# ChenyuWang-Monica/REED

Measured on AMD Instinct MI355X. Metric: SiT-XL/2 ImageNet-256 train images/sec, higher is better.
Workload: dtype bf16

## Files before the change

include/reed_hip.h:

```cpp
#ifndef REED_HIP_H
#define REED_HIP_H
#include <stdint.h>
#ifdef __cplusplus
extern "C" {
#endif

const char* reed_last_error(void);
int reed_version(void);
int reed_half_kind(void);

int reed_gemm(int layout, int epilogue, const void* P, int64_t ldp, const void* Q, int64_t ldq,
              int M, int N, int K, void* C, int64_t ldc, void* C2, int64_t ldc2, const void* R,
              int64_t ldr, const void* bias, const void* gate, int64_t ldgate, int rows_per_gate,
              float* dbias, int accumulate, int split_k, int64_t slab_stride, void* stream);

int reed_wgrad_group(int n, const void* const* dy, const void* const* x, float* const* dw, float* const* dbias,
                     const int* n_out, const int* k_in, int tokens, int accumulate, void* stream);
int reed_wgrad_group_deal(int n, const int* n_out, const int* k_in, const int* has_bias, int cus, unsigned* items);

int reed_set_cu_reserve(int n);
int reed_planning_cus(void);
int reed_set_concurrent_comm(int on);

int reed_gemm_force_tile(int tile);

int64_t reed_colsum_ws_floats(int M, int N);
int reed_colsum_bf16(const void* x, int64_t ld, float* ws, float* out, int M, int N, int accumulate,
                     void* stream);

int reed_reduce_slabs(const float* slabs, int64_t stride, int nslabs, float* out, int64_t n,
                      int accumulate, void* stream);

int reed_ln_modulate_fwd(const float* x, const void* shift, const void* scale, int64_t ldmod,
                         void* h, float* mean, float* rstd, int M, int D, int T, float eps,
                         void* stream);
int reed_ln_modulate_bwd(const void* dh, const float* x, const float* mean, const float* rstd,
                         const void* scale, int64_t ldmod, float* dx, float* part, int M, int D,
                         int T, void* stream);

int reed_ln_modulate_bwd_gate(const void* dh, const float* x, const float* mean, const float* rstd,
                              const void* scale, int64_t ldmod, float* dx, float* part, const void* y,
                              const void* gate, int64_t ldgate, void* dy, float* part_g, float* part_dy,
                              int M, int D, int T, void* stream);

int reed_gate_bwd(const float* dx, const void* y, const void* gate, int64_t ldgate, void* dy,
                  float* part, float* part_dy, int M, int D, int T, void* stream);
int reed_transpose_bf16(const void* src, void* dst, int R, int C, void* stream);
int reed_rowsum_f32(const float* part, int R, float* ws, float* out, int N, int accumulate, void* stream);

int reed_reduce_mod_parts(const float* const* parts, const int64_t* strides, const int64_t* offs,
                          int nparts, void* dmod, int64_t lddmod, int B, int D, int chunks,
                          void* stream);

int reed_attention_fwd(const void* qkv, void* o, float* lse, int B, int T, int H, int hd,
                       void* stream);
int reed_attention_bwd(const void* qkv, const void* o, const void* d_o, const float* lse,
                       void* dqkv, int B, int T, int H, int hd, void* stream);
int64_t reed_attention_bwd_ws_floats(int B, int T, int H);
int reed_attention_bwd_ws(const void* qkv, const void* o, const void* d_o, const float* lse, void* dqkv, float* ws,
                          int B, int T, int H, int hd, void* stream);
int reed_attention_bwd_dp(const void* qkv, const void* d_o, const float* lse, const float* dpart, void* dqkv, float* ws,
                          int B, int T, int H, int hd, void* stream);

int reed_qk_norm_fwd(const void* qkv, const float* qw, const float* qb, const float* kw, const float* kb,
                     void* out, float* stats, int M, int H, int hd, float eps, void* stream);
int64_t reed_qk_norm_bwd_part_floats(int M, int H, int hd);
int reed_qk_norm_bwd(const void* dn, const void* qkv, const float* stats, const float* qw, const float* kw,
                     void* dpre, float* part, int M, int H, int hd, void* stream);

int reed_patch_embed_fwd(const float* x, const void* w, const void* bias, const float* pos,
                         float* tokens, int B, int C, int HW, int P, int D, void* stream);
int reed_patchify_bf16(const float* x, void* out, int B, int C, int HW, int P, int order, void* stream);
int64_t reed_smallk_wgrad_ws_floats(int Dw, int KS);
int reed_smallk_wgrad(const void* wide, int wide_is_f32, const void* small, float* ws, float* out,
                      float* colsum_wide, float* colsum_small, int M, int Dw, int KS, int layout,
                      int accumulate, void* stream);
int reed_timestep_sinusoid(const float* t, void* out, int B, int dim, float max_period, void* stream);
int reed_label_cond(const int64_t* labels, const uint8_t* drop, int num_classes, int table_rows, const float* table,
                    const void* t_emb, int64_t* labels_out, float* c, void* silu_c, int* err_flag, int B, int D,
                    void* stream);
int reed_label_cond_bwd(const float* dsilu_c, const float* c, const int64_t* labels_eff, void* dt_emb,
                        float* dtable, int B, int D, void* stream);
int reed_final_layer_fwd(const float* x, const void* shift, const void* scale, int64_t ldmod,
                         const void* w, const void* bias, float* out, float* mean, float* rstd,
                         int B, int T, int D, int C, int P, float eps, void* stream);
int reed_final_layer_bwd_rows(const float* dout, const float* x, const float* mean, const float* rstd,
                              const void* shift, const void* scale, int64_t ldmod, const void* w,
                              void* hbuf, void* dlin, void* dh, int B, int T, int D, int C, int P,
                              void* stream);
int reed_token_mean_fwd(const float* x, void* out, int B, int T, int D, void* stream);
int reed_token_mean_bwd(const void* dmean, float* dx, int B, int T, int D, void* stream);

int reed_sample_posterior(const float* moments, const float* eps, float* out, int B, int64_t half,
                          float scale, float bias, void* stream);
int reed_interpolant(const float* x, const float* noise, const float* t, float* xt, float* target,
                     int B, int64_t per, int path_type, void* stream);
int reed_mse_fwd(const float* out, const float* target, float* loss, int B, int64_t per, void* stream);
int reed_mse_bwd(const float* out, const float* target, const float* gscale, float* dout, int B,
                 int64_t per, void* stream);
int reed_cosine_fwd(const void* zt, const float* z, float* rowdot, float* loss, int B, int T, int Z,
                    void* stream);
int reed_cosine_bwd(const void* zt, const float* z, const float* gscale, void* dzt, int B, int T,
                    int Z, void* stream);

int reed_grad_sqnorm(const float* g, int64_t n, float* partial, int nblocks, void* stream);
int reed_clip_finalize(const float* partial, int nblocks, float max_norm, float* norm_clip, void* stream);
int reed_clip_finalize_scaled(const float* partial, int nblocks, float max_norm, float* norm_clip, float* scaler_state,
                              float growth_factor, float backoff_factor, float growth_interval, void* stream);
int reed_adamw_ema(float* p, const float* g, float* m, float* v, float* ema, void* shadow,
                   int64_t n_train, int64_t n_total, const float* norm_clip, const float* scaler_state, float lr,
                   float beta1, float beta2, float eps, float weight_decay, float bc1, float bc2, float ema_decay,
                   void* stream);
int reed_cast_bf16(const float* src, void* dst, int64_t n, void* stream);

int reed_sampler_update(const double* x_cur, const float* model_out, const double* d_prev,
                        double* d_store, double* x_next, int64_t n_elems, int cfg, double cfg_scale,
                        double dt, double w0, double w1, void* stream);
int reed_sde_update(const double* x_cur, const float* model_out, const double* eps, double* x_next,
                    int64_t n_elems, int cfg, double cfg_scale, double t_cur, double dt,
                    int path_type, int last_step, void* stream);
int reed_sampler_input(const double* x, float* out, int64_t n_elems, int dup, void* stream);

int reed_comm_unique_id(void* out128);
int reed_comm_init(const void* id128, int rank, int world, void** comm_out);
int reed_comm_allreduce_avg(void* comm, float* buf, int64_t count, void* compute_stream);
int reed_comm_allreduce_avg_rsag(void* comm, float* buf, int64_t count, void* compute_stream);
int reed_comm_sync(void* comm, void* compute_stream);
int reed_comm_broadcast(void* comm, float* buf, int64_t count, int root, void* compute_stream);
int reed_comm_allgather(void* comm, const void* send, void* recv, int64_t bytes, void* compute_stream);
int reed_comm_sync_gather(void* comm, void* compute_stream);
int reed_comm_destroy(void* comm);

int reed_clip_im2col(const float* img, void* out, int B, int S, int P, int Kp, void* stream);
int reed_clip_tokens(const void* patches, const float* cls, const float* pos, void* out, int B, int T, int D,
                     void* stream);
int reed_ln_affine_bf16(const void* x, const float* w, const float* b, void* out, int M, int D, float eps,
                        void* stream);

// ... 27 lines not shown
```

reed_amd/csrc/attention.hip:

```cpp
#include <stdlib.h>

#include <type_traits>
#include <utility>

#include "../../include/reed_hip.h"
#include "common.hpp"

#ifndef REED_ATTN_LD_AUX
#define REED_ATTN_LD_AUX 0
#endif
namespace {

constexpr int ROWB = 144;
constexpr int TILE_B = 256 * ROWB;
constexpr int ROWF = 160;
constexpr int TILE_F = 256 * ROWF;
constexpr float LOG2E = 1.4426950408889634f;
constexpr float LN2 = 0.6931471805599453f;

template <int HD>
struct Cfg {
  static constexpr int KS = (HD + 31) / 32;
  static constexpr int DT = (HD + 15) / 16;
  static constexpr int NCH = HD / 8;
};

template <int HD, int RB = ROWB>
__device__ __forceinline__ void load_tile(char* lds, const bf16* src, long row_stride, int rows_valid,
                                          int tid, int nthreads) {
  constexpr int NCH = Cfg<HD>::NCH;
  constexpr int PER = (256 * NCH + 511) / 512;
  uint4 v[PER];
  const int last = rows_valid - 1;
#pragma unroll
  for (int k = 0; k < PER; ++k) {
    int idx = tid + k * 512;
    int row = idx / NCH, c = idx - row * NCH;
    int rc = min(row, last);
    if (rc < 0) rc = 0;
    int cc = idx < 256 * NCH ? c : 0;
    v[k] = *(const uint4*)(src + (long)rc * row_stride + cc * 8);
  }
#pragma unroll
  for (int k = 0; k < PER; ++k) {
    int idx = tid + k * 512;
    int row = idx / NCH, c = idx - row * NCH;
    if (idx < 256 * NCH) {
      const unsigned msk = row < rows_valid ? 0xFFFFFFFFu : 0u;
      uint4 w = v[k];
      w.x &= msk; w.y &= msk; w.z &= msk; w.w &= msk;
      *(uint4*)(lds + row * RB + c * 16) = w;
    }
  }
  if (RB > HD * 2 + 8 && tid < 256) {
#pragma unroll
    for (int c = Cfg<HD>::NCH; c < RB / 16; ++c) *(uint4*)(lds + tid * RB + c * 16) = make_uint4(0, 0, 0, 0);
  }
}

__device__ __forceinline__ bf16x8 frag_rows(const char* tile, int row0, int ks, int lane) {
  return *(const bf16x8*)(tile + (row0 + (lane & 15)) * ROWB + (ks * 32 + 8 * (lane >> 4)) * 2);
}
template <bool WRAP>
__device__ __forceinline__ bf16x8 frag_rows_f(const char* tile, int row0, int ks, int lane) {
  const int g = WRAP ? ((lane >> 4) & 1) : (lane >> 4);
  return *(const bf16x8*)(tile + (row0 + (lane & 15)) * ROWF + (ks * 32 + 8 * g) * 2);
}
__device__ __forceinline__ bf16x8 frag_trT_f(const char* tile, int rbase, int d0, int lane) {
  int i = lane & 15, g = lane >> 4, q = i >> 2, p = i & 3;
  const char* a0 = tile + (rbase + 4 * g + q) * ROWF + (d0 + 4 * p) * 2;
  bf16x4 lo = REED_DS_READ_TR16_B64((bf16x4 __attribute__((address_space(3)))*)a0);
  bf16x4 hi = REED_DS_READ_TR16_B64((bf16x4 __attribute__((address_space(3)))*)(a0 + 16 * ROWF));
  return __builtin_shufflevector(lo, hi, 0, 1, 2, 3, 4, 5, 6, 7);
}
__device__ __forceinline__ bf16x8 frag_trT(const char* tile, int rbase, int d0, int lane) {
  int i = lane & 15, g = lane >> 4, q = i >> 2, p = i & 3;
  const char* a0 = tile + (rbase + 4 * g + q) * ROWB + (d0 + 4 * p) * 2;
  bf16x4 lo = REED_DS_READ_TR16_B64((bf16x4 __attribute__((address_space(3)))*)a0);
  bf16x4 hi = REED_DS_READ_TR16_B64((bf16x4 __attribute__((address_space(3)))*)(a0 + 16 * ROWB));
  return __builtin_shufflevector(lo, hi, 0, 1, 2, 3, 4, 5, 6, 7);
}
template <int HD>
__device__ __forceinline__ bf16x8 load_frag_global(const bf16* rowptr, bool row_ok, int ks, int lane) {
  bf16x8 z;
#pragma unroll
  for (int j = 0; j < 8; ++j) z[j] = (bf16)0.f;
  int col = ks * 32 + 8 * (lane >> 4);
  if (row_ok && col < HD) z = *(const bf16x8*)(rowptr + col);
// ... 833 lines not shown
#pragma unroll
      for (int kt = 0; kt < 16; ++kt) {
#pragma unroll
        for (int r = 0; r < 4; ++r) {
          float p = __builtin_fmaf(st[qt][kt][r], sc2, -mneg);
          if (!(DBGK && (dbg & 2))) p = __builtin_amdgcn_exp2f(p);
          st[qt][kt][r] = p;
          if (!ONES) sum += p;
        }
        if (kt & 1) pb[qt][kt >> 1] = pack2(st[qt][kt - 1], st[qt][kt]);
      }
      if (!ONES) {
        sum += __shfl_xor(sum, 16, 64);
        sum += __shfl_xor(sum, 32, 64);
      }
      mrow[qt] = mneg;
      lrow[qt] = sum;
      __builtin_amdgcn_sched_barrier(0);
    }
    ATTN_STAMP(3);
    asm volatile("s_waitcnt vmcnt(12)" ::: "memory");
    __builtin_amdgcn_sched_barrier(0);
    ATTN_STAMP(4);
    if (ONES && lane < 32) *(bf16*)(Vw + lane * ROWF + HD * 2) = (bf16)1.0f;
    ATTN_BARRIER();
    ATTN_STAMP(5);
    char* const k2rows = Kb + par * TILE_F + wave * 32 * ROWF;
    const __amdgpu_buffer_rsrc_t k2rs = mk_rsrc(plus(base_of(it + 2 * G), D), win);
    constexpr bool KSPREAD = PVX && REED_ATTN_KSPREAD;
    if constexpr (!KSPREAD) {
#pragma unroll
      for (int j = 0; j < 5; ++j) issue_piece(k2rows, k2rs, j);
    }
    __builtin_amdgcn_sched_barrier(0);
    f32x4 ot[2][DT];
    {
      const unsigned vb = lds_addr(Vt + (4 * g + (i >> 2)) * ROWF + (i & 3) * 8);
      if (DBGK && (dbg & 4)) {
#pragma unroll
        for (int dt = 0; dt < DT; ++dt) ot[0][dt] = ot[1][dt] = f32x4{1.f, 1.f, 1.f, 1.f};
      } else if (FULL && !PVX) {
        pvu_all<ROWF, 8, DT>(vb, pb, ot);
      } else if (FULL) {
        pvx_all<ROWF, DT, !ONES>(vb, st, mrow, sc2, lrow, DBGK && (dbg & 2), ot, [&](auto s_c) {
          constexpr int S = decltype(s_c)::value;
          if constexpr (KSPREAD && S < 5) issue_piece(k2rows, k2rs, S);
        });
        if (!ONES) {
#pragma unroll
          for (int qt = 0; qt < 2; ++qt) {
            lrow[qt] += __shfl_xor(lrow[qt], 16, 64);
            lrow[qt] += __shfl_xor(lrow[qt], 32, 64);
          }
        }
      } else {
#pragma unroll
        for (int qt = 0; qt < 2; ++qt)
#pragma unroll
          for (int dt = 0; dt < DT; ++dt) ot[qt][dt] = zero4();
        pv_all<ROWF, DT>(Vt + (4 * g + (i >> 2)) * ROWF + (i & 3) * 8, (T + 31) >> 5, pb, ot);
      }
    }
    ATTN_STAMP(6);
    asm volatile("s_waitcnt vmcnt(22)" ::: "memory");
    __builtin_amdgcn_sched_barrier(0);
    ATTN_STAMP(7);
    ATTN_BARRIER();
    ATTN_STAMP(8);
    stage_item(ot, mrow, lrow);
    __builtin_amdgcn_sched_barrier(0);
    store_item(it);
  }
  asm volatile("s_waitcnt vmcnt(0)" ::: "memory");
  if (DBGK && (dbg & 32) && lse && lane0 == 0) {
    unsigned long long* dst = (unsigned long long*)lse + ((long)blockIdx.x * 8 + wave) * 10;
#pragma unroll
    for (int k = 0; k < 10; ++k) dst[k] = tacc[k];
  }
#undef ATTN_STAMP
}

template <int HD, bool KSP = true, bool QSP = true>
__global__ __launch_bounds__(512, 2) void attn_fwd256v_kernel(const bf16* __restrict__ qkv, bf16* __restrict__ o,
                                                             float* __restrict__ lse, int H, int nitems) {
  extern __shared__ __attribute__((aligned(16))) char smem[];
  constexpr int T = 256;
  constexpr int KS = Cfg<HD>::KS, DT = Cfg<HD>::DT, NCH = Cfg<HD>::NCH;
  constexpr bool ONES = (HD == 72);
  static_assert(HD == 64 || HD == 72, "attn_fwd256v_kernel: head_dim 64 or 72");
  const int tid = threadIdx.x;
  const int lane0 = tid & 63;
  const int wave = __builtin_amdgcn_readfirstlane(tid >> 6);
  const int D = H * HD;
  const long tok = 3l * D;
  const int tokb = (int)(tok * 2);
  char* const Kw = smem + wave * 32 * ROWF;
  char* const Vt = smem + TILE_F;
  char* const Qw = smem + 3 * TILE_F + wave * 32 * ROWF;
  const int q0 = wave * 32;
  const float sc2 = rsqrtf((float)HD) * LOG2E;
  int voff[5];
#pragma unroll
  for (int j = 0; j < 5; ++j) voff[j] = dma_voff<HD, ROWF>((wave * 5 + j) * 64 + lane0, tokb);
  const long win = tile_window<HD>(T, tokb);
  auto piece = [&](char* wave_rows, __amdgpu_buffer_rsrc_t rs, int j) {
    __builtin_amdgcn_raw_ptr_buffer_load_lds(rs, (lds_ptr_t)(wave_rows + j * 1024), 16, voff[j], 0, 0, REED_ATTN_LD_AUX);
  };
  auto issue = [&](char* wave_rows, const bf16* base) {
    const __amdgpu_buffer_rsrc_t rs = mk_rsrc(base, win);
#pragma unroll
    for (int j = 0; j < 5; ++j) piece(wave_rows, rs, j);
  };
  auto base_of = [&](int item) -> const bf16* {
    if (item >= nitems) return nullptr;
    const int b = item / H, h = item - b * H;
    return qkv + (long)b * T * tok + h * HD;
  };
  auto plus = [](const bf16* p_, long n) -> const bf16* { return p_ ? p_ + n : nullptr; };
  const int G = gridDim.x;
  constexpr int RST = ROWB;
  constexpr int NQ = 32 * NCH;
  float lsev[2] = {0.f, 0.f};
  f32x4 st[2][16];

  int it = xcd_contiguous(blockIdx.x, G);
  {
    const bf16* b0 = base_of(it);
    issue(Qw, b0);
    issue(Kw, plus(b0, D));
    issue(Vt + wave * 32 * ROWF, plus(b0, 2 * D));
    const __amdgpu_buffer_rsrc_t none = mk_rsrc(nullptr, 0);
#pragma unroll
    for (int k = 0; k < 8; ++k) __builtin_amdgcn_raw_buffer_store_b32((unsigned)(k + lane0), none, DMA_OOB - 256 * k, 0, 0);
    asm volatile("s_waitcnt vmcnt(13)" ::: "memory");
    ATTN_BARRIER();
  }
  int par = 0, pit = -1;
  for (; it < nitems; it += G, par ^= 1) {
    int lane = lane0;
    asm volatile("" : "+v"(lane));
    const int i = lane & 15, g = lane >> 4;
    char* const Vcur = Vt + par * TILE_F;
    char* const Vprev_w = Vt + (par ^ 1) * TILE_F + wave * 32 * ROWF;
    asm volatile("s_waitcnt vmcnt(17)" ::: "memory");
    __builtin_amdgcn_sched_barrier(0);
    bf16x8 qf[2][KS];
    {
      const unsigned qa = lds_addr(Qw + i * ROWF + 16 * g);
#pragma unroll
      for (int qt = 0; qt < 2; ++qt)
#pragma unroll
        for (int ks = 0; ks < KS; ++ks) {
          const bool wrap = HD % 32 != 0 && ks == KS - 1;
          const unsigned a = qa + qt * 16 * ROWF + ks * 64 - ((wrap && g >= 2) ? 32 : 0);
          qf[qt][ks] = lds_read128_asm(a);
        }
      ATTN_LDS_WAIT();
      if (HD % 32 != 0 && g >= 2) { qf[0][KS - 1] = zero_frag(); qf[1][KS - 1] = zero_frag(); }
    }
    const __amdgpu_buffer_rsrc_t rsQ = mk_rsrc(base_of(it + G), win);
    if constexpr (!QSP) {
#pragma unroll
      for (int j = 0; j < 5; ++j) piece(Qw, rsQ, j);
    }
    __builtin_amdgcn_sched_barrier(0);
    {
      const int pb_ = pit < 0 ? 0 : pit / H, ph = pit < 0 ? 0 : pit - pb_ * H;
      const __amdgpu_buffer_rsrc_t rsO = mk_rsrc(pit < 0 ? nullptr : o + (long)pb_ * T * D + ph * HD, tile_window<HD>(T, D * 2));
      const __amdgpu_buffer_rsrc_t rsL = mk_rsrc((lse && pit >= 0) ? lse + ((long)pb_ * H + ph) * T : nullptr, (long)T * 4);
      const __amdgpu_buffer_rsrc_t rsV = mk_rsrc(plus(base_of(it + G), 2 * D), win);
      u32x4 pc = {0u, 0u, 0u, 0u};
      const unsigned ka = lds_addr(smem + i * ROWF + 16 * g);
      sk_all<HD, ROWF>(ka, ka - (g >= 2 ? 32 : 0), qf, st, [&](auto kt_c) {
        constexpr int KT = decltype(kt_c)::value;
        if constexpr (KT < 10 && (KT & 1) == 0) {
          constexpr int k = KT / 2;
          const int qi = min(lane + 64 * k, NQ - 1);
          const int rr = qi / NCH, c = qi - rr * NCH;
          pc = __builtin_bit_cast(u32x4, lds_read128_asm(lds_addr(Vprev_w + rr * RST + c * 16)));
        } else if constexpr (KT < 10) {
          constexpr int k = KT / 2;
          piece(Vprev_w, rsV, k);
          const int qi = lane + 64 * k;
          const int rr = qi / NCH, c = qi - rr * NCH;
          __builtin_amdgcn_raw_buffer_store_b128(pc, rsO, qi < NQ ? (q0 + rr) * (D * 2) + c * 16 : DMA_OOB, 0, 0);
        } else if constexpr (KT < 12) {
          constexpr int qt = KT - 10;
          __builtin_amdgcn_raw_buffer_store_b32(__builtin_bit_cast(unsigned, lsev[qt]), rsL,
                                                g == 0 ? (q0 + 16 * qt + i) * 4 : DMA_OOB, 0, 0);
        }
        if constexpr (QSP && KT >= 11) piece(Qw, rsQ, KT - 11);
      });
    }
    float mrow[2], lrow[2];
#pragma unroll
    for (int qt = 0; qt < 2; ++qt) {
      float mx = -INFINITY;
#pragma unroll
      for (int kt = 0; kt < 16; ++kt)
#pragma unroll
        for (int r = 0; r < 4; ++r) mx = fmaxf(mx, st[qt][kt][r]);
      mx = fmaxf(mx, __shfl_xor(mx, 16, 64));
      mx = fmaxf(mx, __shfl_xor(mx, 32, 64));
      mrow[qt] = mx * sc2;
      lrow[qt] = 0.f;
    }
    asm volatile("s_waitcnt vmcnt(25)" ::: "memory");
    __builtin_amdgcn_sched_barrier(0);
    if (ONES && lane < 32) *(bf16*)(Vcur + (wave * 32 + lane) * ROWF + HD * 2) = (bf16)1.0f;
    ATTN_BARRIER();
    const __amdgpu_buffer_rsrc_t rsK = mk_rsrc(plus(base_of(it + G), D), win);
    if constexpr (!KSP) {
#pragma unroll
      for (int j = 0; j < 5; ++j) piece(Kw, rsK, j);
    }
    __builtin_amdgcn_sched_barrier(0);
    f32x4 ot[2][DT];
    {
      const unsigned vb = lds_addr(Vcur + (4 * g + (i >> 2)) * ROWF + (i & 3) * 8);
      pvx_all<ROWF, DT, !ONES>(vb, st, mrow, sc2, lrow, false, ot, [&](auto s_c) {
        constexpr int S = decltype(s_c)::value;
        if constexpr (KSP && S < 5) piece(Kw, rsK, S);
      });
      if (!ONES) {
#pragma unroll
        for (int qt = 0; qt < 2; ++qt) {
          lrow[qt] += __shfl_xor(lrow[qt], 16, 64);
          lrow[qt] += __shfl_xor(lrow[qt], 32, 64);
        }
      }
    }
    asm volatile("s_waitcnt vmcnt(0)" ::: "memory");
    __builtin_amdgcn_sched_barrier(0);
    ATTN_BARRIER();
    {
      char* const Vw = Vcur + wave * 32 * ROWF;
#pragma unroll
      for (int qt = 0; qt < 2; ++qt) {
        float l = lrow[qt];
        if (ONES) l = __shfl(ot[qt][DT - 1][0], 32 + i, 64);
        const float inv = __builtin_amdgcn_rcpf(l);
#pragma unroll
        for (int dt = 0; dt < DT; ++dt) {
          const int d = 16 * dt + 4 * g;
          const u32x2 v = {pk2(ot[qt][dt][0] * inv, ot[qt][dt][1] * inv), pk2(ot[qt][dt][2] * inv, ot[qt][dt][3] * inv)};
          if (16 * dt + 16 <= HD || d < HD) *(u32x2*)(Vw + (16 * qt + i) * RST + d * 2) = v;
        }
        lsev[qt] = mrow[qt] * LN2 + __logf(l);
      }
    }
    __builtin_amdgcn_sched_barrier(0);
    pit = it;
  }
  if (pit >= 0) {
    int lane = lane0;
    asm volatile("" : "+v"(lane));
    const int i = lane & 15, g = lane >> 4;
    const char* const Vw = Vt + (par ^ 1) * TILE_F + wave * 32 * ROWF;
    const int pb_ = pit / H, ph = pit - pb_ * H;
    const __amdgpu_buffer_rsrc_t rsO = mk_rsrc(o + (long)pb_ * T * D + ph * HD, tile_window<HD>(T, D * 2));
    const __amdgpu_buffer_rsrc_t rsL = mk_rsrc(lse ? lse + ((long)pb_ * H + ph) * T : nullptr, (long)T * 4);
    u32x4 pcs[5];
#pragma unroll
    for (int k = 0; k < 5; ++k) {
      const int qi = min(lane + 64 * k, NQ - 1);
      const int rr = qi / NCH, c = qi - rr * NCH;
      pcs[k] = __builtin_bit_cast(u32x4, lds_read128_asm(lds_addr(Vw + rr * RST + c * 16)));
    }
    ATTN_LDS_WAIT();
#pragma unroll
    for (int k = 0; k < 5; ++k) {
      const int qi = lane + 64 * k;
      const int rr = qi / NCH, c = qi - rr * NCH;
      __builtin_amdgcn_raw_buffer_store_b128(pcs[k], rsO, qi < NQ ? (q0 + rr) * (D * 2) + c * 16 : DMA_OOB, 0, 0);
    }
#pragma unroll
    for (int qt = 0; qt < 2; ++qt)
      __builtin_amdgcn_raw_buffer_store_b32(__builtin_bit_cast(unsigned, lsev[qt]), rsL, g == 0 ? (q0 + 16 * qt + i) * 4 : DMA_OOB, 0, 0);
  }
  asm volatile("s_waitcnt vmcnt(0)" ::: "memory");
}

template <int HD>
__global__ __launch_bounds__(512, 2) void attn_bwd_ks_kernel(const bf16* __restrict__ qkv, const bf16* __restrict__ o,
                                                             const bf16* __restrict__ d_o, const float* __restrict__ lse,
                                                             bf16* __restrict__ dqkv, int B, int T, int H) {
  extern __shared__ __attribute__((aligned(16))) char smem[];
  constexpr int KS = Cfg<HD>::KS, DT = Cfg<HD>::DT, NCH = Cfg<HD>::NCH;
  constexpr int DTA = (DT + 1) / 2;
  const int tid = threadIdx.x, lane = tid & 63;
  const int wave = __builtin_amdgcn_readfirstlane(tid >> 6);
  const int i = lane & 15, g = lane >> 4;
  const int D = H * HD;
  const int bh = xcd_contiguous(blockIdx.x, gridDim.x);
  const int b = bh / H, h = bh % H;
  const long tok = 3l * D;
  const bf16* base = qkv + (long)b * T * tok + h * HD;
  bf16* dbase = dqkv + (long)b * T * tok + h * HD;
  const bf16* gbase = d_o + (long)b * T * D + h * HD;
  char* Qt = smem;
  char* Kt = smem + TILE_B;
  char* St = smem + 2 * TILE_B;
  char* Gt = smem + 3 * TILE_B;
  float* lse2 = (float*)(smem + 4 * TILE_B + 256);
  float* dlt = lse2 + 256;
  if (tid < 16) *(uint4*)(smem + 4 * TILE_B + tid * 16) = make_uint4(0, 0, 0, 0);
  const float scale = rsqrtf((float)HD);
  const float sc2 = scale * LOG2E;
  const int r0 = wave * 32;

  auto issue_tile = [&](char* t, const bf16* s, int sb) {
    const __amdgpu_buffer_rsrc_t rs = mk_rsrc(s, tile_window<HD>(T, sb));
#pragma unroll
    for (int j = 0; j < 5; ++j) {
      const int I = wave + 8 * j;
      const int vo = dma_voff<HD, ROWB>(I * 64 + lane, sb);
      if (I < 36) __builtin_amdgcn_raw_ptr_buffer_load_lds(rs, (lds_ptr_t)(t + I * 1024), 16, vo, 0, 0, REED_ATTN_LD_AUX);
    }
  };
  issue_tile(Kt, base + D, (int)(tok * 2));
  issue_tile(Qt, base, (int)(tok * 2));
  issue_tile(Gt, gbase, D * 2);
  bf16x8 kf[2][KS], vf[2][KS];
  {
    bf16x8 gf[2][KS], of[2][KS];
    float lq[2];
#pragma unroll
    for (int t2 = 0; t2 < 2; ++t2) {
      const int row = r0 + 16 * t2 + i;
      const bool ok = row < T;
#pragma unroll
      for (int ks = 0; ks < KS; ++ks) {
        vf[t2][ks] = load_frag_global<HD>(base + 2 * D + (long)row * tok, ok, ks, lane);
        gf[t2][ks] = load_frag_global<HD>(gbase + (long)row * D, ok, ks, lane);
        of[t2][ks] = load_frag_global<HD>(o + ((long)b * T + row) * D + h * HD, ok, ks, lane);
// ... 1049 lines not shown
            bf16x8 gtf = frag_trT(Gc, qq0, 16 * dt, lane);
            bf16x8 qtf = frag_trT(Qc, qq0, 16 * dt, lane);
#pragma unroll
            for (int ct = 0; ct < 2; ++ct) {
              dv[ct][dt] = MFMA(gtf, pb[ct], dv[ct][dt]);
              dk[ct][dt] = MFMA(qtf, dsb[ct], dk[ct][dt]);
            }
          }
        }
      }
      __syncthreads();
      {
        const int qtile = wave >> 1;
        const int dt0 = (wave & 1) ? DTA : 0;
        f32x4 dq[DTA];
#pragma unroll
        for (int k = 0; k < DTA; ++k) dq[k] = zero4();
#pragma unroll 1
        for (int ks = 0; ks < nkb; ++ks) {
          const bf16x8 dsf = frag_trT(St, 32 * ks, 16 * qtile, lane);
#pragma unroll
          for (int k = 0; k < DTA; ++k) {
            if (dt0 + k < DT) {
              const bf16x8 ktf = frag_trT(Kt, 32 * ks, 16 * (dt0 + k), lane);
              dq[k] = MFMA(ktf, dsf, dq[k]);
            }
          }
        }
        const int q = ch * 64 + 16 * qtile + i;
#pragma unroll
        for (int k = 0; k < DTA; ++k) {
          const int d = 16 * (dt0 + k) + 4 * g;
          if (dt0 + k < DT && d < HD && q < T) *(f32x4*)(dqb + (long)q * D + d) = dq[k] * scale;
        }
      }
    }
#pragma unroll
    for (int ct = 0; ct < 2; ++ct) {
      const int key = k0 + r0 + 16 * ct + i;
#pragma unroll
      for (int dt = 0; dt < DT; ++dt) {
        const int d = 16 * dt + 4 * g;
        if (d < HD && kvalid[ct]) {
          bf16x4 a, c;
#pragma unroll
          for (int r = 0; r < 4; ++r) { a[r] = f2bf(dk[ct][dt][r] * scale); c[r] = f2bf(dv[ct][dt][r]); }
          *(bf16x4*)(dbase + (long)key * tok + D + d) = a;
          *(bf16x4*)(dbase + (long)key * tok + 2 * D + d) = c;
        }
      }
    }
  }
}

__global__ __launch_bounds__(256) void attn_dq_reduce_kernel(const float* __restrict__ dqp, bf16* __restrict__ dqkv, long n4, long slice,
                                                             int D, int nkt) {
  const long j = (long)blockIdx.x * 256 + threadIdx.x;
  if (j >= n4) return;
  f32x4 acc = *(const f32x4*)(dqp + 4 * j);
  for (int kt = 1; kt < nkt; ++kt) acc += *(const f32x4*)(dqp + kt * slice + 4 * j);
  const long e = 4 * j, tokn = e / D;
  const int c = (int)(e - tokn * D);
  bf16x4 v;
#pragma unroll
  for (int r = 0; r < 4; ++r) v[r] = f2bf(acc[r]);
  *(bf16x4*)(dqkv + tokn * 3 * D + c) = v;
}

template <typename K>
int set_lds(K kernel, int bytes) {
  hipError_t e = hipFuncSetAttribute((const void*)kernel, hipFuncAttributeMaxDynamicSharedMemorySize, bytes);
  if (e != hipSuccess) { reed_set_error("hipFuncSetAttribute(LDS=%d): %s", bytes, hipGetErrorString(e)); return (int)e; }
  return 0;
}

}
int reed_concurrent_comm();
int reed_num_cus();
namespace {
int num_cus() { return reed_num_cus(); }

}

extern "C" int reed_attention_fwd(const void* qkv, void* o, float* lse, int B, int T, int H, int hd,
                                  void* stream) {
  REED_CHECK_ARG(qkv && o, "attention_fwd: null pointer");
  REED_CHECK_ARG(hd == 64 || hd == 72 || hd == 80, "attention: head_dim %d unsupported (64, 72 or 80)", hd);
  REED_CHECK_ARG(hd != 80 || T <= 256, "attention: head_dim 80 (the I-JEPA ViT-H tower) is built for T <= 256 only (T=%d)", T);
  REED_CHECK_ARG(B > 0 && T > 0 && H > 0, "attention: bad dims B=%d T=%d H=%d", B, T, H);
  if (T <= 256) {
    const int lds = 4 * TILE_F, nitems = B * H;
    int ncu = num_cus();
    ncu -= ncu % 8;
    const dim3 grid(nitems < ncu ? nitems : ncu);
#ifdef REED_ATTN_DIAG
    static const int fdbg = getenv("REED_ATTN_FWD_DBG") ? atoi(getenv("REED_ATTN_FWD_DBG")) : 0;
#else
    constexpr int fdbg = 0;
#endif
    if (REED_ATTN_FWD_VDB_DEFAULT && T == 256 && (hd == 64 || hd == 72) && !fdbg) {
      if (hd == 64) {
        static int once = set_lds(attn_fwd256v_kernel<64>, lds);
        if (once) return once;
        REED_KLAUNCH((attn_fwd256v_kernel<64>), grid, dim3(512), lds, (hipStream_t)stream, (const bf16*)qkv, (bf16*)o, lse, H, nitems);
      } else {
        static int once = set_lds(attn_fwd256v_kernel<72>, lds);
        if (once) return once;
        REED_KLAUNCH((attn_fwd256v_kernel<72>), grid, dim3(512), lds, (hipStream_t)stream, (const bf16*)qkv, (bf16*)o, lse, H, nitems);
      }
      REED_LAUNCH_CHECK();
      return REED_OK;
    }
#define LAUNCH_FWD256P(HD, FULL, DBGK)                                                                                 \
    do {                                                                                                               \
      static int once = set_lds(attn_fwd256p_kernel<HD, FULL, DBGK>, lds);                                             \
      if (once) return once;                                                                                           \
      REED_KLAUNCH((attn_fwd256p_kernel<HD, FULL, DBGK>), grid, dim3(512), lds, (hipStream_t)stream,                    \
                   (const bf16*)qkv, (bf16*)o, lse, T, H, nitems, fdbg);                                               \
    } while (0)
#ifdef REED_ATTN_DIAG
    if (fdbg && hd == 72 && T == 256) LAUNCH_FWD256P(72, true, true);
    else
#endif
    if (hd == 64) { if (T == 256) LAUNCH_FWD256P(64, true, false); else LAUNCH_FWD256P(64, false, false); }
    else if (hd == 72) { if (T == 256) LAUNCH_FWD256P(72, true, false); else LAUNCH_FWD256P(72, false, false); }
    else { if (T == 256) LAUNCH_FWD256P(80, true, false); else LAUNCH_FWD256P(80, false, false); }
#undef LAUNCH_FWD256P
    REED_LAUNCH_CHECK();
    return REED_OK;
  }
  const int lds = 2 * TILE_F;
  dim3 grid(B * H, (T + 255) / 256);
  const int tail = T % 256;
  if (hd == 64 && T > 512 && T <= 4096 + 16 && tail >= 1 && tail <= 16) {
    grid.y = T / 256;
    static int once = set_lds(attn_fwd_kernel<64, true>, lds);
    if (once) return once;
    REED_KLAUNCH((attn_fwd_kernel<64, true>), grid, dim3(512), lds, (hipStream_t)stream, (const bf16*)qkv, (bf16*)o, lse, B, T, H);
    REED_LAUNCH_CHECK();
    return REED_OK;
  }
  if (hd == 64 && T > 256 && T <= 512 && tail >= 1 && tail <= 16) {
    grid.y = T / 256;
    const int nwaves = B * H * tail;
    REED_KLAUNCH(attn_fwd_rows_kernel, dim3(cdiv(nwaves, 4)), dim3(256), 0, (hipStream_t)stream, (const bf16*)qkv, (bf16*)o, lse, T, H,
                 T - tail, tail, nwaves);
    REED_LAUNCH_CHECK();
  }
  if (hd == 64) {
    static int once = set_lds(attn_fwd_kernel<64>, lds);
    if (once) return once;
    REED_KLAUNCH(attn_fwd_kernel<64>, grid, dim3(512), lds, (hipStream_t)stream, (const bf16*)qkv, (bf16*)o, lse, B, T, H);
  } else {
    static int once = set_lds(attn_fwd_kernel<72>, lds);
    if (once) return once;
    REED_KLAUNCH(attn_fwd_kernel<72>, grid, dim3(512), lds, (hipStream_t)stream, (const bf16*)qkv, (bf16*)o, lse, B, T, H);
  }
  REED_LAUNCH_CHECK();
  return REED_OK;
}

extern "C" int reed_attention_bwd(const void* qkv, const void* o, const void* d_o, const float* lse,
                                  void* dqkv, int B, int T, int H, int hd, void* stream) {
  REED_CHECK_ARG(qkv && o && d_o && lse && dqkv, "attention_bwd: null pointer");
  REED_CHECK_ARG(hd == 64 || hd == 72, "attention: head_dim %d unsupported (64 or 72)", hd);
  REED_CHECK_ARG(T > 0 && T <= 256, "attention_bwd: T=%d unsupported without a workspace (T <= 256; 256 < T <= 4096 runs through "
                 "reed_attention_bwd_ws / reed_attention_bwd_dp)", T);
  const int lds = 4 * TILE_B + 256 + 2048;
  dim3 grid(B * H);
  if (hd == 64) {
    static int once = set_lds(attn_bwd_ks_kernel<64>, lds);
    if (once) return once;
    REED_KLAUNCH((attn_bwd_ks_kernel<64>), grid, dim3(512), lds, (hipStream_t)stream, (const bf16*)qkv, (const bf16*)o,
                 (const bf16*)d_o, lse, (bf16*)dqkv, B, T, H);
  } else {
    static int once = set_lds(attn_bwd_ks_kernel<72>, lds);
    if (once) return once;
    REED_KLAUNCH((attn_bwd_ks_kernel<72>), grid, dim3(512), lds, (hipStream_t)stream, (const bf16*)qkv, (const bf16*)o,
                 (const bf16*)d_o, lse, (bf16*)dqkv, B, T, H);
  }
  REED_LAUNCH_CHECK();
  return REED_OK;
}


extern "C" int64_t reed_attention_bwd_ws_floats(int B, int T, int H) {
  const int64_t n = (int64_t)B * T * H;
  return T <= 256 ? n : n * (1 + (int64_t)((T + 255) / 256) * 72);
}

static int attention_bwd_persistent(const void* qkv, const void* o, const void* d_o, const float* lse, void* dqkv, float* ws,
                                    const float* dpart, int B, int T, int H, int hd, void* stream) {
  REED_CHECK_ARG(qkv && (o || dpart) && d_o && lse && dqkv && ws, "attention_bwd: null pointer");
  REED_CHECK_ARG(hd == 64 || hd == 72, "attention: head_dim %d unsupported (64 or 72)", hd);
  REED_CHECK_ARG(B > 0 && H > 0 && T > 0 && T <= 4096 && (T <= 256 || T % 16 == 0),
                 "attention_bwd: B=%d H=%d T=%d unsupported (T <= 256, or 256 < T <= 4096 with T a multiple of 16)", B, H, T);
  const int lds = 4 * TILE_B + 256 + 2048;
  const int nitems = B * H;
  const long nseg = (long)B * T * H;
  int ncu = num_cus();
  ncu -= ncu % 8;
  const int gmult = reed_concurrent_comm() ? 4 : 1;
  const long gwant = (long)ncu * gmult;
  const dim3 pgrid((unsigned)(nitems < gwant ? nitems : gwant));
  hipStream_t s = (hipStream_t)stream;
#ifdef REED_ATTN_DIAG
  static const int dbg = getenv("REED_ATTN_KSP_DBG") ? atoi(getenv("REED_ATTN_KSP_DBG")) : 0;
#else
  constexpr int dbg = 0;
#endif
#define REED_DELTA(HD)                                                                                                    \
  do {                                                                                                                    \
    if (dpart)                                                                                                            \
      REED_KLAUNCH(attn_delta_combine_kernel, dim3(cdiv(nseg, 256)), dim3(256), 0, s, dpart, ws, (long)B * T, T, H, (HD) == 64 ? 1 : 2); \
    else                                                                                                                  \
      REED_KLAUNCH(attn_delta_kernel<HD>, dim3(cdiv(nseg, 256)), dim3(256), 0, s, (const bf16*)o, (const bf16*)d_o, ws, nseg, T, H); \
  } while (0)
#define REED_BWD_KSP(HD)                                                                                                  \
  do {                                                                                                                    \
    static int once = set_lds(attn_bwd_ksp_kernel<HD>, lds);                                                              \
    if (once) return once;                                                                                                \
    REED_DELTA(HD);                                                                                                       \
    REED_LAUNCH_CHECK();                                                                                                  \
    REED_KLAUNCH(attn_bwd_ksp_kernel<HD>, pgrid, dim3(512), lds, s, (const bf16*)qkv, (const bf16*)d_o, lse, (const float*)ws, \
                 (bf16*)dqkv, T, H, nitems, dbg);                                                                              \
  } while (0)
  if (T > 256) {
    const int nkt = (T + 255) / 256, litems = B * H * nkt;
    const dim3 lgrid((unsigned)(litems < gwant ? litems : gwant));
    const long slice = nseg * hd;
    float* dqp = ws + nseg;
#define REED_BWD_LONG(HD)                                                                                                 \
  do {                                                                                                                    \
    static int once = set_lds(attn_bwd_long_kernel<HD>, LONG_LDS);                                                        \
    if (once) return once;                                                                                                \
    REED_DELTA(HD);                                                                                                       \
    REED_LAUNCH_CHECK();                                                                                                  \
    REED_KLAUNCH(attn_bwd_long_kernel<HD>, lgrid, dim3(512), LONG_LDS, s, (const bf16*)qkv, (const bf16*)d_o, lse,         \
                 (const float*)ws, dqp, (bf16*)dqkv, slice, T, H, nkt, litems);                                            \
  } while (0)
    if (hd == 64) REED_BWD_LONG(64);
    else REED_BWD_LONG(72);
// ... 54 lines not shown
```

reed_amd/csrc/attention_f32.hip:

```cpp
#include "../../include/reed_hip.h"
#include "common.hpp"

#ifndef REED_FP32
#error "attention_f32.hip belongs to the fp32-operand build (-DREED_FP32) only"
#endif

namespace {

constexpr int KT = 32;

template <int HD>
__device__ __forceinline__ void stage_rows(float* tile, const float* qkv, int which, long b, int h, int H, int T, int r0,
                                           int tid) {
  constexpr int NV = HD / 4;
  for (int i = tid; i < KT * NV; i += 256) {
    const int r = i / NV, c = i % NV;
    const int row = r0 + r;
    f32x4 v = {0.f, 0.f, 0.f, 0.f};
    if (row < T) v = *(const f32x4*)(qkv + (((b * T + row) * 3 + which) * H + h) * HD + 4 * c);
    *(f32x4*)(tile + r * HD + 4 * c) = v;
  }
}
template <int HD>
__device__ __forceinline__ void stage_rows_o(float* tile, const float* x, long b, int h, int H, int T, int r0, int tid) {
// ... 126 lines not shown
    __syncthreads();
    const int kn = min(KT, T - k0);
#pragma unroll 1
    for (int j = 0; j < kn; ++j) {
      const float p = expf(dot_row<HD>(qv, sk + j * HD) - ls);
      const float ds = p * (dot_row<HD>(dov, sv + j * HD) - delta);
      axpy_row<HD>(dq, ds, sk + j * HD);
    }
  }
  if (live) {
    float* gp = dqkv + (((b * T + q) * 3 + 0) * H + h) * HD;
#pragma unroll
    for (int c = 0; c < HD / 4; ++c)
      *(f32x4*)(gp + 4 * c) = f32x4{dq[4 * c] * scale, dq[4 * c + 1] * scale, dq[4 * c + 2] * scale, dq[4 * c + 3] * scale};
  }
}

template <int HD>
__global__ __launch_bounds__(256) void attn_f32_bwd_dkv_kernel(const float* __restrict__ qkv, const float* __restrict__ o,
                                                               const float* __restrict__ d_o, const float* __restrict__ lse,
                                                               float* __restrict__ dqkv, int T, int H) {
  __shared__ __attribute__((aligned(16))) float sq[KT * HD], sdo[KT * HD];
  __shared__ float sls[KT], sdl[KT];
  const int tid = threadIdx.x;
  const long b = blockIdx.x / H;
  const int h = blockIdx.x % H;
  const int kr = blockIdx.y * 256 + tid;
  const bool live = kr < T;
  const int kc = live ? kr : 0;
  const float scale = rsqrtf((float)HD);
  float kv[HD], vv[HD], dk[HD], dv[HD];
  {
    const float* kp = qkv + (((b * T + kc) * 3 + 1) * H + h) * HD;
    const float* vp = qkv + (((b * T + kc) * 3 + 2) * H + h) * HD;
#pragma unroll
    for (int c = 0; c < HD / 4; ++c) {
      const f32x4 a = *(const f32x4*)(kp + 4 * c), v = *(const f32x4*)(vp + 4 * c);
#pragma unroll
      for (int e = 0; e < 4; ++e) {
        kv[4 * c + e] = a[e] * scale;
        vv[4 * c + e] = v[e];
        dk[4 * c + e] = 0.f;
        dv[4 * c + e] = 0.f;
      }
    }
  }
  for (int q0 = 0; q0 < T; q0 += KT) {
    __syncthreads();
    stage_rows<HD>(sq, qkv, 0, b, h, H, T, q0, tid);
    stage_rows_o<HD>(sdo, d_o, b, h, H, T, q0, tid);
    if (tid < KT) {
      const int row = q0 + tid;
      float dl = 0.f, ls = INFINITY;
      if (row < T) {
        const float* op = o + ((b * T + row) * H + h) * HD;
        const float* gp = d_o + ((b * T + row) * H + h) * HD;
        for (int e = 0; e < HD; ++e) dl = fmaf(gp[e], op[e], dl);
        ls = lse[(b * H + h) * T + row];
      }
      sls[tid] = ls;
      sdl[tid] = dl;
    }
    __syncthreads();
    const int qn = min(KT, T - q0);
#pragma unroll 1
    for (int i = 0; i < qn; ++i) {
      const float p = expf(dot_row<HD>(kv, sq + i * HD) - sls[i]);
      const float ds = p * (dot_row<HD>(vv, sdo + i * HD) - sdl[i]);
      axpy_row<HD>(dv, p, sdo + i * HD);
      axpy_row<HD>(dk, ds, sq + i * HD);
    }
  }
  if (live) {
    float* gk = dqkv + (((b * T + kr) * 3 + 1) * H + h) * HD;
    float* gv = dqkv + (((b * T + kr) * 3 + 2) * H + h) * HD;
#pragma unroll
    for (int c = 0; c < HD / 4; ++c) {
      *(f32x4*)(gk + 4 * c) = f32x4{dk[4 * c] * scale, dk[4 * c + 1] * scale, dk[4 * c + 2] * scale, dk[4 * c + 3] * scale};
      *(f32x4*)(gv + 4 * c) = f32x4{dv[4 * c], dv[4 * c + 1], dv[4 * c + 2], dv[4 * c + 3]};
    }
  }
}

}

extern "C" int reed_attention_fwd(const void* qkv, void* o, float* lse, int B, int T, int H, int hd, void* stream) {
  REED_CHECK_ARG(qkv && o, "attention_fwd: null pointer");
  REED_CHECK_ARG(hd == 64 || hd == 72, "attention (fp32 build): head_dim %d unsupported (64 or 72)", hd);
  REED_CHECK_ARG(B > 0 && T > 0 && H > 0, "attention: bad dims B=%d T=%d H=%d", B, T, H);
  const dim3 grid(B * H, (T + 255) / 256);
  if (hd == 64) REED_KLAUNCH(attn_f32_fwd_kernel<64>, grid, dim3(256), 0, (hipStream_t)stream, (const float*)qkv, (float*)o, lse, T, H);
  else REED_KLAUNCH(attn_f32_fwd_kernel<72>, grid, dim3(256), 0, (hipStream_t)stream, (const float*)qkv, (float*)o, lse, T, H);
  REED_LAUNCH_CHECK();
  return REED_OK;
}

extern "C" int reed_attention_bwd(const void* qkv, const void* o, const void* d_o, const float* lse, void* dqkv, int B, int T,
                                  int H, int hd, void* stream) {
  REED_CHECK_ARG(qkv && o && d_o && lse && dqkv, "attention_bwd: null pointer");
  REED_CHECK_ARG(hd == 64 || hd == 72, "attention (fp32 build): head_dim %d unsupported (64 or 72)", hd);
  REED_CHECK_ARG(B > 0 && T > 0 && H > 0, "attention: bad dims B=%d T=%d H=%d", B, T, H);
  const dim3 grid(B * H, (T + 255) / 256);
  hipStream_t s = (hipStream_t)stream;
#define REED_BWD_F32(HD)                                                                                                 \
  do {                                                                                                                   \
    REED_KLAUNCH(attn_f32_bwd_dq_kernel<HD>, grid, dim3(256), 0, s, (const float*)qkv, (const float*)o, (const float*)d_o, \
                 lse, (float*)dqkv, T, H);                                                                               \
    REED_LAUNCH_CHECK();                                                                                                 \
    REED_KLAUNCH(attn_f32_bwd_dkv_kernel<HD>, grid, dim3(256), 0, s, (const float*)qkv, (const float*)o,                  \
                 (const float*)d_o, lse, (float*)dqkv, T, H);                                                            \
  } while (0)
  if (hd == 64) REED_BWD_F32(64);
  else REED_BWD_F32(72);
#undef REED_BWD_F32
  REED_LAUNCH_CHECK();
  return REED_OK;
}

extern "C" int64_t reed_attention_bwd_ws_floats(int, int, int) { return 0; }
extern "C" int reed_attention_bwd_ws(const void* qkv, const void* o, const void* d_o, const float* lse, void* dqkv, float*, int B,
                                     int T, int H, int hd, void* stream) {
  return reed_attention_bwd(qkv, o, d_o, lse, dqkv, B, T, H, hd, stream);
}

extern "C" int reed_attention_bwd_dp(const void*, const void*, const float*, const float*, void*, float*, int, int, int, int, void*) {
  reed_set_error("reed_attention_bwd_dp: not built for fp32 operands (use reed_attention_bwd_ws)");
  return REED_ERR_UNSUPPORTED;
}
```

reed_amd/csrc/gemm.hip:

```cpp
#include <stdlib.h>

#include "gemm_common.hpp"

int reed_gemm256_launch(int layout, int epi, GemmArgs a, int splits, hipStream_t stream);
int reed_gemm_tn_launch(int tile, GemmArgs a, int splits, hipStream_t stream);
bool reed_gemm256_preferred(int layout, int epi, const GemmArgs& a, int splits);
bool reed_gemm144_eligible(int layout, int epi, const GemmArgs& a, int splits);
bool reed_gemm144_preferred(int layout, int epi, const GemmArgs& a, int splits);
int reed_gemm144_launch(int layout, int epi, GemmArgs a, hipStream_t stream);
bool reed_gemm288_eligible(int layout, int epi, const GemmArgs& a, int splits);
bool reed_gemm288_preferred(int layout, int epi, const GemmArgs& a, int splits);
int reed_gemm288_launch(int epi, GemmArgs a, hipStream_t stream);
bool reed_gemm256w_eligible(int layout, int epi, const GemmArgs& a, int splits);
int reed_gemm256w_launch(int layout, int epi, GemmArgs a, hipStream_t stream);
int reed_num_cus();
double reed_gemm256_rate();
bool reed_gemm_skinny_eligible(int layout, int epi, const GemmArgs& a, int splits);
int reed_gemm_skinny_launch(int epi, GemmArgs a, hipStream_t stream);

namespace {
using namespace gemm_detail;

constexpr int BM = 128, BN = 128, BK = 64;
constexpr int TILE_BYTES = 16384;
// ... 105 lines not shown
    if constexpr (LAY != LAY_NT) REED_LDS_WAIT();
#pragma unroll
    for (int ks = 0; ks < 2; ++ks) {
#pragma unroll
      for (int i = 0; i < 4; ++i)
#pragma unroll
        for (int j = 0; j < 4; ++j)
          acc[i][j] = REED_MFMA_16x16x32(qf[ks][j], pf[ks][i], acc[i][j]);
      if constexpr (LAY == LAY_TN) {
        if (do_dbias) {
#pragma unroll
          for (int i = 0; i < 4; ++i)
            accb[i] = REED_MFMA_16x16x32(ones, pf[ks][i], accb[i]);
        }
      }
    }
    __syncthreads();
  }

  tile_epilogue<EPI, 4>(a, acc, m0, wm * 64, n0 + wn * 64, lane, z, smem + wave * EPI_STAGE_BYTES);
  if constexpr (LAY == LAY_TN) {
    if (do_dbias && (lane >> 4) == 0) {
#pragma unroll
      for (int i = 0; i < 4; ++i) {
        const int m = m0 + wm * 64 + i * 16 + (lane & 15);
        if (m < a.M) {
          if (gridDim.y > 1) a.dbias[(long)z * a.slab_stride + m] = accb[i][0];
          else if (a.accumulate) a.dbias[m] += accb[i][0];
          else a.dbias[m] = accb[i][0];
        }
      }
    }
  }
}

template <int LAY, int EPI>
int launch(const GemmArgs& a, int splits, hipStream_t stream) {
  static bool attr_set = false;
  if (!attr_set) {
    (void)hipFuncSetAttribute((const void*)gemm_kernel<LAY, EPI>,
                              hipFuncAttributeMaxDynamicSharedMemorySize, 2 * STAGE_BYTES);
    attr_set = true;
  }
  const int ntm = cdiv(a.M, BM), ntn = a.N / BN;
  dim3 grid(ntm * ntn, splits, 1);
  REED_KLAUNCH((gemm_kernel<LAY, EPI>), grid, dim3(256), 2 * STAGE_BYTES, stream, a);
  REED_LAUNCH_CHECK();
  return REED_OK;
}

template <int LAY>
int dispatch_epi(int epi, const GemmArgs& a, int splits, hipStream_t s) {
  switch (epi) {
    case EPI_BF16: return launch<LAY, EPI_BF16>(a, splits, s);
    case EPI_GELU: return launch<LAY, EPI_GELU>(a, splits, s);
    case EPI_SILU: return launch<LAY, EPI_SILU>(a, splits, s);
    case EPI_GATE_RES: return launch<LAY, EPI_GATE_RES>(a, splits, s);
    case EPI_DGELU: return launch<LAY, EPI_DGELU>(a, splits, s);
    case EPI_DSILU: return launch<LAY, EPI_DSILU>(a, splits, s);
    case EPI_GELU_G: return launch<LAY, EPI_GELU_G>(a, splits, s);
    case EPI_SILU_G: return launch<LAY, EPI_SILU_G>(a, splits, s);
    case EPI_MUL: return launch<LAY, EPI_MUL>(a, splits, s);
    case EPI_F32: return launch<LAY, EPI_F32>(a, splits, s);
    case EPI_ADDF32_RB: return launch<LAY, EPI_ADDF32_RB>(a, splits, s);
    case EPI_ATOMIC_F32: return launch<LAY, EPI_ATOMIC_F32>(a, splits, s);
    case EPI_QGELU: return launch<LAY, EPI_QGELU>(a, splits, s);
    case EPI_GELU_ERF: return launch<LAY, EPI_GELU_ERF>(a, splits, s);
    case EPI_RES_BF16: return launch<LAY, EPI_RES_BF16>(a, splits, s);
    case EPI_LS_RES:
      if constexpr (LAY == LAY_NT) return launch<LAY, EPI_LS_RES>(a, splits, s);
      break;
  }
  reed_set_error("reed_gemm: unknown epilogue %d", epi);
  return REED_ERR_ARG;
}

}

static const bool g_colsplit = getenv("REED_GEMM_COLSPLIT") && atoi(getenv("REED_GEMM_COLSPLIT")) != 0;
static int g_force_tile = 0;
extern "C" int reed_gemm_force_tile(int tile) { g_force_tile = tile; return 0; }
int reed_gemm_forced_tile() { return g_force_tile; }

int reed_gemm_launch(int layout, int epi, GemmArgs a, int splits, hipStream_t stream) {
  REED_CHECK_ARG(a.M > 0 && a.N > 0 && a.K > 0, "reed_gemm: empty problem M=%d N=%d K=%d", a.M, a.N, a.K);
  const int want = epi;
  if (epi == EPI_BF16_DOT) {
    REED_CHECK_ARG((layout == LAY_NN || layout == LAY_NT) && a.R && a.C2 && (a.rows_per_gate == 64 || a.rows_per_gate == 72) &&
                       a.N % a.rows_per_gate == 0 && a.N % 64 == 0 && splits <= 1,
                   "reed_gemm(epilogue 13): NN or NT, R and C2 given, rows_per_gate = head_dim 64 or 72 dividing N");
    epi = EPI_BF16;
  }
#define REED_ONLY_PLAIN()                                                                             \
  do {                                                                                                \
    if (want == EPI_BF16_DOT) {                                                                       \
      reed_set_error("reed_gemm(epilogue 13): this shape runs on a kernel without it (use epilogue 0)"); \
      return REED_ERR_UNSUPPORTED;                                                                    \
    }                                                                                                 \
  } while (0)
  const bool can144 = reed_gemm144_eligible(layout, epi, a, splits);
  REED_CHECK_ARG(a.N % BN == 0 || can144, "reed_gemm: N=%d must be a multiple of %d (or, NT / NN with a bf16-output epilogue, of 144)", a.N, BN);
  REED_CHECK_ARG(a.ldp % 8 == 0 && a.ldq % 8 == 0, "reed_gemm: leading dims must be multiples of 8 elements");
  REED_CHECK_ARG(a.ldc >= 0 && a.ldc < (1 << 20) && a.ldc2 >= 0 && a.ldc2 < (1 << 20) && a.ldr >= 0 && a.ldr < (1 << 20) &&
                     a.ldc % 8 == 0 && a.ldc2 % 8 == 0 && a.ldr % 8 == 0,
                 "reed_gemm: output/residual leading dims must be multiples of 8 below 2^20 (32-bit tile offsets)");
  REED_CHECK_ARG(((uintptr_t)a.P % 16) == 0 && ((uintptr_t)a.Q % 16) == 0 && ((uintptr_t)a.C % 16) == 0,
                 "reed_gemm: operands must be 16-byte aligned");
  const int tn_tile = layout == LAY_TN_TALL ? 1 : layout == LAY_TN_WIDE ? 2 : 0;
  if (tn_tile) {
    REED_CHECK_ARG(epi == EPI_F32, "reed_gemm(TN 256x128 / 128x256): fp32 (weight-gradient) epilogue only");
    layout = LAY_TN;
  }
  if (layout == LAY_TN) {
    REED_CHECK_ARG(a.M % BM == 0, "reed_gemm(TN): M=%d must be a multiple of %d", a.M, BM);
  } else {
    REED_CHECK_ARG(a.K % BK == 0, "reed_gemm(NT/NN): K=%d must be a multiple of %d", a.K, BK);
  }
  if (splits < 1) splits = 1;
  int ksteps = cdiv(a.K, BK);
  int per = cdiv(ksteps, splits);
  splits = cdiv(ksteps, per);
  a.ksplit_len = per * BK;
  if (splits > 1) {
    REED_CHECK_ARG(epi == EPI_ATOMIC_F32 || (epi == EPI_F32 && a.slab_stride > 0),
                   "reed_gemm: split-K needs the atomic or slab fp32 epilogue");
  }
  if (tn_tile) return reed_gemm_tn_launch(tn_tile, a, splits, stream);
  {
    const bool epi_rows_free = epi == EPI_BF16 || epi == EPI_GELU || epi == EPI_SILU || epi == EPI_QGELU || epi == EPI_GELU_ERF ||
                               epi == EPI_RES_BF16 || epi == EPI_LS_RES || epi == EPI_DGELU || epi == EPI_DSILU ||
                               epi == EPI_GELU_G || epi == EPI_SILU_G || epi == EPI_MUL;
    const int r = a.M % 256, mfull = a.M - r;
    if (g_force_tile == 0 && want != EPI_BF16_DOT && epi_rows_free && splits <= 1 && (layout == LAY_NT || layout == LAY_NN) &&
        r > 0 && r <= 128 && mfull >= 2048) {
      const int ncu = reed_num_cus(), ntn = cdiv(a.N, 256), rows = mfull / 256;
      if (cdiv((long)rows * ntn, ncu) < cdiv((long)(rows + 1) * ntn, ncu)) {
        const int cb = epi == EPI_LS_RES ? 4 : 2, rb = epi == EPI_LS_RES ? 4 : 2;
        GemmArgs m = a, t = a;
        m.M = mfull;
        t.M = r;
        t.P = a.P + (long)mfull * a.ldp;
        if (a.C) t.C = (char*)a.C + (long)mfull * a.ldc * cb;
        if (a.C2) t.C2 = (char*)a.C2 + (long)mfull * a.ldc2 * 2;
        if (a.R) t.R = (const char*)a.R + (long)mfull * a.ldr * rb;
        const int rc = reed_gemm_launch(layout, epi, m, splits, stream);
        if (rc != REED_OK) return rc;
        if (reed_gemm_skinny_eligible(layout, epi, t, splits)) return reed_gemm_skinny_launch(epi, t, stream);
        return reed_gemm_launch(layout, epi, t, splits, stream);
      }
    }
  }
  {
    const bool epi_cols_free = epi == EPI_BF16 || epi == EPI_GELU || epi == EPI_SILU || epi == EPI_QGELU || epi == EPI_GELU_ERF ||
                               epi == EPI_RES_BF16 || epi == EPI_GATE_RES || epi == EPI_DGELU || epi == EPI_DSILU ||
                               epi == EPI_GELU_G || epi == EPI_SILU_G || epi == EPI_MUL;
    if (((g_force_tile == 0 && g_colsplit) || g_force_tile == 259) && want != EPI_BF16_DOT && epi_cols_free && splits <= 1 &&
        (layout == LAY_NT || layout == LAY_NN) && a.N % 256 == 0 && a.K >= 256) {
      const int ncu = reed_num_cus();
      const long tm = cdiv(a.M, 256), tn = a.N / 256;
      const long full = tm * tn / ncu, rem = tm * tn % ncu;
      if (full >= 1 && rem > 0 && (full * ncu) % tm == 0) {
        const long tn1 = full * ncu / tm;
        GemmArgs h = a, t = a;
        h.N = (int)(tn1 * 256);
        t.N = a.N - h.N;
        if (reed_gemm256w_eligible(layout, epi, h, splits)) {
          const double r256 = 4.0 / reed_gemm256_rate();
// ... 65 lines not shown
```

reed_amd/csrc/gemm256w.hip:

```cpp
#include <math.h>
#include <stdlib.h>
#include <string.h>

#include <algorithm>
#include <vector>
#include <type_traits>

#include "gemm_common.hpp"

int reed_num_cus();
int reed_gemm_forced_tile();
int reed_concurrent_comm();

#if defined(REED_CLK_PROBE) || defined(REED_CLK_PHASE)
__device__ unsigned long long reed_clk_buf[8 * 8192];
extern "C" int reed_clk_probe_read(unsigned long long* out, int n) {
  return (int)hipMemcpyFromSymbol(out, HIP_SYMBOL(reed_clk_buf), sizeof(unsigned long long) * n);
}
#endif
#ifndef REED_EPI_PF
#define REED_EPI_PF 4
#endif
#ifndef REED_TN_RING
#define REED_TN_RING 1
#endif
#ifndef REED_TN_Q_NT
#define REED_TN_Q_NT 0
#endif
#ifndef REED_DB_DEAL
#define REED_DB_DEAL 0
#endif
namespace {
using namespace gemm_detail;

constexpr int WBM = 256, WBN = 256, WBK = 64;
constexpr int HTW = 16384;
constexpr int LDS_W = 8 * HTW + 4 * EPI_STAGE_BYTES;
constexpr int LDS_TN = 8 * HTW;
__device__ __forceinline__ constexpr int wslotA(int h, int cur) { return (h * 2 + cur) * HTW; }
__device__ __forceinline__ constexpr int wslotB(int h, int cur) { return (4 + h * 2 + cur) * HTW; }

__device__ __forceinline__ int wvoff_row(int tid, long ld) {
  const int r = tid >> 3, cp = tid & 7;
  return (int)(((long)r * ld + (cp ^ ((r >> 1) & 7)) * 8) * 2);
}
__device__ __forceinline__ int wvoff_tr(int tid, long ld) {
  const int r = tid >> 4, chp = tid & 15;
  return (int)(((long)r * ld + (chp ^ tr_sw(r)) * 8) * 2);
}

template <int OFF>
__device__ __forceinline__ bf16x8 wtr2u(unsigned a0, unsigned a1) {
  bf16x4 lo, hi;
  asm volatile("ds_read_b64_tr_b16 %0, %1 offset:%2" : "=v"(lo) : "v"(a0), "i"(OFF));
  asm volatile("ds_read_b64_tr_b16 %0, %1 offset:%2" : "=v"(hi) : "v"(a1), "i"(OFF));
  return __builtin_shufflevector(lo, hi, 0, 1, 2, 3, 4, 5, 6, 7);
}
template <int OFF>
__device__ __forceinline__ bf16x8 wtr2(const char* a0, const char* a1) {
  bf16x4 lo = ds_read_tr16_off<OFF>(a0);
  bf16x4 hi = ds_read_tr16_off<OFF>(a1);
  return __builtin_shufflevector(lo, hi, 0, 1, 2, 3, 4, 5, 6, 7);
}

typedef int w_i32x4 __attribute__((ext_vector_type(4)));
__device__ __forceinline__ void w_store_acc(const f32x4& q, w_i32x4 rs, int voff) {
  asm volatile("buffer_store_dwordx4 %0, %1, %2, 0 offen" ::"a"(q), "v"(voff), "s"(rs) : "memory");
}
template <int LAY, int EPI, int MODE, int PM = 0, int DIRECT = 0>
__device__ __forceinline__ void gemm256w_body(const GemmArgs& a, char* smem, const int tm, const int tn,
                                              const int prev_mode = -1, const int nx_mode = -1, const int nx_tm = 0,
                                              const int nx_tn = 0) {
  const bool first = prev_mode < 0;
  static_assert(MODE <= 3 || (MODE >= 6 && MODE <= 8 && LAY == LAY_TN && PM == 0), "three-unit / bias-only items: weight gradients only");
  constexpr bool RN = MODE <= 3 && (MODE & 1) != 0, RM = MODE <= 3 && (MODE & 2) != 0;
  constexpr int NA = RN ? 4 : 8;
  constexpr int NB = RM ? 4 : 8;
  constexpr int NCH = NA * NB / 4;
  constexpr int NF = NA + NB;
  constexpr int NAH = MODE == 8 ? 4 : MODE == 6 ? 3 : (MODE == 7 || RM) ? 1 : 2;
  constexpr int NBH = MODE == 7 ? 3 : MODE == 8 ? 0 : (MODE == 6 || RN) ? 1 : 2;
  constexpr int ND = 4 * (NAH + NBH);
  constexpr bool A_TR = LAY == LAY_TN, B_TR = LAY != LAY_NT;
  const int tid = threadIdx.x, lane = tid & 63;
  const int wave = __builtin_amdgcn_readfirstlane(tid >> 6);
  const bool brole = MODE == 8 || ((MODE == 6 || MODE == 7) && wave == 3);
  const int aHalf = (MODE == 6 || MODE == 8) ? wave : (MODE == 0 || MODE == 1) ? (wave >> 1) : 0;
  const int aQuart = MODE == 1 ? (wave & 1) : MODE == 3 ? (wave >> 1) : 0;
  const int bHalf = MODE == 7 ? wave : MODE == 0 ? (wave & 1) : MODE == 2 ? (wave >> 1) : 0;
  const int bQuart = (MODE == 2 || MODE == 3) ? (wave & 1) : 0;
// ... 542 lines not shown
      const bool rv = m0 + ml < a.M;
      const int ro = (ml + lr) * ldc4 + (n0 + ncol + lc) * 4;
#pragma unroll
      for (int j = 0; j < NB; ++j) {
        const bool ok = rv && n0 + ncol + 16 * j < a.N;
        w_store_acc(acc[i][j], rs, ok ? ro + 64 * j : EPI_OOB);
      }
    }
    return;
  }
  char* stage = smem + 8 * HTW + wave * EPI_STAGE_BYTES;
#pragma unroll
  for (int h = 0; h < NB / 4; ++h) {
    f32x4 part[NA][4];
#pragma unroll
    for (int i = 0; i < NA; ++i)
#pragma unroll
      for (int j = 0; j < 4; ++j) part[i][j] = acc[i][h * 4 + j];
    tile_epilogue<EPI, NA, REED_EPI_PF>(a, part, m0, mrow, n0 + ncol + h * 64, lane, 0, stage);
  }
  if constexpr (LAY == LAY_TN && !(PM == 0 && REED_TN_RING)) {
    if (do_dbias && (lane >> 4) == 0) {
#pragma unroll
      for (int i = 0; i < NA; ++i) {
        const int m = m0 + mrow + i * 16 + (lane & 15);
        if (m < a.M && (db_par < 0 || (db_par < 2 ? (i & 1) == db_par : (i >> 1) == db_par - 2))) {
          if (a.accumulate) a.dbias[m] += accb[i][0];
          else a.dbias[m] = accb[i][0];
        }
      }
    }
  }
#undef W_CI
#undef W_CJ
#undef WMMA4
#undef WPHASE
#undef WBARRIER
#undef WLGKM0
#undef WKTILE
#undef WKTILE_
#undef WSTAMP
}

template <int LAY, int EPI>
__global__ __launch_bounds__(256, 1) void gemm256w_kernel(GemmArgs a) {
  extern __shared__ __attribute__((aligned(16))) char smem[];
  const int ntm = (a.M + WBM - 1) / WBM, ntn = (a.N + WBN - 1) / WBN;
  int tm, tn;
  {
    const int nwg = ntm * ntn;
    int bid = blockIdx.x;
    {
      int xcd = bid & 7, q = nwg >> 3, r = nwg & 7;
      bid = (xcd < r ? xcd * (q + 1) : r * (q + 1) + (xcd - r) * q) + (bid >> 3);
    }
    const int GM = a.tile_gm;
    const int per_group = GM * ntn;
    const int group = bid / per_group, first_m = group * GM;
    const int gs = min(ntm - first_m, GM);
    tm = first_m + (bid % per_group) % gs;
    tn = (bid % per_group) / gs;
  }
#ifdef REED_CLK_PROBE
  const unsigned long long en0 = __builtin_amdgcn_s_memrealtime();
  __builtin_amdgcn_s_waitcnt(0xC07F);
#endif
  if (a.N - tn * WBN <= 128) gemm256w_body<LAY, EPI, 1>(a, smem, tm, tn);
  else gemm256w_body<LAY, EPI, 0>(a, smem, tm, tn);
#ifdef REED_CLK_PROBE
  {
    asm volatile("s_waitcnt vmcnt(0)" ::: "memory");
    const unsigned long long en1 = __builtin_amdgcn_s_memrealtime();
    __builtin_amdgcn_s_waitcnt(0xC07F);
    const int pidx = tm * ntn + tn;
    if (threadIdx.x == 0 && pidx < 8192) {
      const unsigned hw = __builtin_amdgcn_s_getreg((31 << 11) | 4), xcc = __builtin_amdgcn_s_getreg((31 << 11) | 20);
      reed_clk_buf[8 * pidx + 6] = en0;
      reed_clk_buf[8 * pidx + 7] = (en1 << 16) | ((xcc & 0xF) << 8) | ((hw >> 8) & 0xFF);
    }
  }
#endif
}

__device__ __forceinline__ void w_tile_of(int b, int ntm, int ntn, int GM, int& tm, int& tn) {
  const int per_group = GM * ntn;
  const int group = b / per_group, first_m = group * GM;
  const int gs = min(ntm - first_m, GM);
  tm = first_m + (b % per_group) % gs;
  tn = (b % per_group) / gs;
}
template <int LAY, int EPI>
__global__ __launch_bounds__(256, 1) void gemm256wp_kernel(GemmArgs a) {
  extern __shared__ __attribute__((aligned(16))) char smem[];
  const int ntm = (a.M + WBM - 1) / WBM, ntn = (a.N + WBN - 1) / WBN;
  const int nwg = ntm * ntn;
  const int xcd = blockIdx.x & 7, s = blockIdx.x >> 3, wpx = gridDim.x >> 3;
  const int q = nwg >> 3, r = nwg & 7;
  const int run0 = xcd < r ? xcd * (q + 1) : r * (q + 1) + (xcd - r) * q, runlen = q + (xcd < r ? 1 : 0);
  int p = s;
  if (p >= runlen) return;
  int tm, tn;
  w_tile_of(run0 + p, ntm, ntn, a.tile_gm, tm, tn);
  int pmode = -1;
  for (;;) {
    const int pn = p + wpx;
    int nmode = -1, tmn = 0, tnn = 0;
    if (pn < runlen) {
      w_tile_of(run0 + pn, ntm, ntn, a.tile_gm, tmn, tnn);
      nmode = (a.N - tnn * WBN <= 128) ? 1 : 0;
    }
#ifdef REED_CLK_PROBE
    const unsigned long long en0 = __builtin_amdgcn_s_memrealtime();
    __builtin_amdgcn_s_waitcnt(0xC07F);
#endif
    const int cmode = (a.N - tn * WBN <= 128) ? 1 : 0;
    if (cmode) gemm256w_body<LAY, EPI, 1, 1>(a, smem, tm, tn, pmode, nmode, tmn, tnn);
    else gemm256w_body<LAY, EPI, 0, 1>(a, smem, tm, tn, pmode, nmode, tmn, tnn);
#ifdef REED_CLK_PROBE
    {
      const unsigned long long en1 = __builtin_amdgcn_s_memrealtime();
      __builtin_amdgcn_s_waitcnt(0xC07F);
      const int pidx = tm * ntn + tn;
      if (threadIdx.x == 0 && pidx < 8192) {
        const unsigned hw = __builtin_amdgcn_s_getreg((31 << 11) | 4), xcc = __builtin_amdgcn_s_getreg((31 << 11) | 20);
        reed_clk_buf[8 * pidx + 6] = en0;
        reed_clk_buf[8 * pidx + 7] = (en1 << 16) | ((xcc & 0xF) << 8) | ((hw >> 8) & 0xFF);
      }
    }
#endif
    if (nmode < 0) break;
    p = pn;
    tm = tmn;
    tn = tnn;
    pmode = cmode;
  }
}

struct TnGroupW {
  GemmArgs a[4];
  int n;
  int wpx;
  unsigned item[256];
};
template <int ACC>
__global__ __launch_bounds__(256, 1) void gemm256w_tn_group_kernel(TnGroupW g) {
  extern __shared__ __attribute__((aligned(16))) char smem[];
  const unsigned it = g.item[(blockIdx.x & 7) * g.wpx + (blockIdx.x >> 3)];
  if (it == 0xFFFFFFFFu) return;
  const int p = it & 3, mode = (it >> 2) & 15, mu = (it >> 6) & 255, nu = (it >> 14) & 255;
  const int vm = ((it >> 22) & 3) + 1, vn = ((it >> 24) & 3) + 1;
  GemmArgs a = g.a[p];
  if (((it >> 26) & 1) == 0) a.dbias = nullptr;
#ifdef REED_CLK_PROBE
  a.act_variant = 2000 + (int)blockIdx.x;
#endif
  if (mode == 0) {
    gemm256w_body<LAY_TN, EPI_F32, 0, 0, 1 - ACC>(a, smem, mu >> 1, nu >> 1);
  } else if (mode == 6) {
    a.M = min(a.M, (mu + vm) * 128);
    gemm256w_body<LAY_TN, EPI_F32, 6, 0, 1 - ACC>(a, smem, mu, nu);
  } else if (mode == 7) {
    a.N = min(a.N, (nu + vn) * 128);
    gemm256w_body<LAY_TN, EPI_F32, 7, 0, 1 - ACC>(a, smem, mu, nu);
  } else {
    a.M = min(a.M, (mu + vm) * 128);
    gemm256w_body<LAY_TN, EPI_F32, 8, 0, 1 - ACC>(a, smem, mu, 0);
  }
}

int w_tile_group_rows(const GemmArgs& a) {
#ifdef REED_TILE_GM_ENV
  if (const char* e = getenv("REED_TILE_GM")) return atoi(e) > 0 ? atoi(e) : 4;
#endif
  if (cdiv(a.M, WBM) < 192) return 4;
  const int ntn = cdiv(a.N, WBN);
  return ntn <= 6 ? 2 : ntn >= 16 ? 5 : 4;
}

constexpr double RAG_COST = 0.58;
double w_static_max_load(int ntm, int ntn, bool rag, int GM, int wpx) {
  const int nwg = ntm * ntn, q = nwg >> 3, r = nwg & 7;
  double worst = 0;
  for (int xcd = 0; xcd < 8; ++xcd) {
    const int run0 = xcd < r ? xcd * (q + 1) : r * (q + 1) + (xcd - r) * q, runlen = q + (xcd < r ? 1 : 0);
    for (int s = 0; s < wpx && s < runlen; ++s) {
      double load = 0;
      for (int p = s; p < runlen; p += wpx) {
        const int b = run0 + p, per_group = GM * ntn, group = b / per_group, first_m = group * GM;
        const int gs = std::min(ntm - first_m, GM), tn = (b % per_group) / gs;
        load += (rag && tn == ntn - 1) ? RAG_COST : 1.0;
      }
      worst = std::max(worst, load);
    }
  }
  return worst;
}

template <int LAY, int EPI>
int launch256wp(const GemmArgs& a, hipStream_t stream, bool* used) {
  const int forced = reed_gemm_forced_tile();
  const int mode = forced == 257 ? 0 : forced == 258 ? 2 : reed_concurrent_comm() ? 0 : 1;
  *used = false;
  const int nt = cdiv(a.K, WBK), ntm = cdiv(a.M, WBM), ntn = cdiv(a.N, WBN);
  const int wpx = reed_num_cus() / 8;
  if (mode == 0 || (nt & 1) || nt < 4 || wpx < 1 || (a.K % WBK) != 0) return REED_OK;
  const bool rag = (a.N % WBN) != 0;
  const int GM = w_tile_group_rows(a);
  const double total = (double)ntm * ((ntn - (rag ? 1 : 0)) + (rag ? RAG_COST : 0.0));
  const double ideal = total / (8.0 * wpx);
  if (mode == 1 && ideal < 3.0) return REED_OK;
  if (mode == 1) {
    static thread_local struct { int ntm, ntn, gm, wpx, ok; } memo[8];
    static thread_local int memo_n = 0;
    int ok = -1;
    for (int i = 0; i < memo_n; ++i)
      if (memo[i].ntm == ntm && memo[i].ntn == (rag ? -ntn : ntn) && memo[i].gm == GM && memo[i].wpx == wpx) ok = memo[i].ok;
    if (ok < 0) {
      const double worst = w_static_max_load(ntm, ntn, rag, GM, wpx);
      const double greedy = ideal + (rag ? 0.45 : 0.0);
      ok = worst > greedy + 0.05 ? 0 : 1;
      memo[memo_n % 8] = {ntm, rag ? -ntn : ntn, GM, wpx, ok};
      if (memo_n < 8) ++memo_n;
    }
    if (!ok) return REED_OK;
  }
  static bool attr_set = false;
  if (!attr_set) {
    hipError_t e = hipFuncSetAttribute((const void*)gemm256wp_kernel<LAY, EPI>, hipFuncAttributeMaxDynamicSharedMemorySize,
                                       LDS_W);
    if (e != hipSuccess) { reed_set_error("gemm256wp: cannot reserve LDS: %s", hipGetErrorString(e)); return (int)e; }
    attr_set = true;
  }
  GemmArgs b = a;
  b.tile_gm = GM;
  REED_KLAUNCH((gemm256wp_kernel<LAY, EPI>), dim3(8 * wpx), dim3(256), LDS_W, stream, b);
  REED_LAUNCH_CHECK();
  *used = true;
  return REED_OK;
}

template <int LAY, int EPI>
int launch256w(const GemmArgs& a, hipStream_t stream) {
  {
    bool used = false;
    const int rc = launch256wp<LAY, EPI>(a, stream, &used);
    if (rc != REED_OK || used) return rc;
  }
  static bool attr_set = false;
  if (!attr_set) {
    hipError_t e = hipFuncSetAttribute((const void*)gemm256w_kernel<LAY, EPI>, hipFuncAttributeMaxDynamicSharedMemorySize,
                                       LDS_W);
    if (e != hipSuccess) { reed_set_error("gemm256w: cannot reserve LDS: %s", hipGetErrorString(e)); return (int)e; }
    attr_set = true;
  }
  dim3 grid(cdiv(a.M, WBM) * cdiv(a.N, WBN), 1, 1);
  GemmArgs b = a;
  b.tile_gm = w_tile_group_rows(a);
  REED_KLAUNCH((gemm256w_kernel<LAY, EPI>), grid, dim3(256), LDS_W, stream, b);
  REED_LAUNCH_CHECK();
  return REED_OK;
}

template <int LAY>
int dispatch256w(int epi, const GemmArgs& a, hipStream_t s) {
  if constexpr (LAY == LAY_NT) {
    switch (epi) {
      case EPI_BF16: return launch256w<LAY, EPI_BF16>(a, s);
      case EPI_GELU: return launch256w<LAY, EPI_GELU>(a, s);
      case EPI_SILU: return launch256w<LAY, EPI_SILU>(a, s);
      case EPI_GELU_G: return launch256w<LAY, EPI_GELU_G>(a, s);
      case EPI_SILU_G: return launch256w<LAY, EPI_SILU_G>(a, s);
      case EPI_GATE_RES: return launch256w<LAY, EPI_GATE_RES>(a, s);
      case EPI_RES_BF16: return launch256w<LAY, EPI_RES_BF16>(a, s);
      case EPI_LS_RES: return launch256w<LAY, EPI_LS_RES>(a, s);
      case EPI_QGELU: return launch256w<LAY, EPI_QGELU>(a, s);
      case EPI_GELU_ERF: return launch256w<LAY, EPI_GELU_ERF>(a, s);
      case EPI_BF16_DOT: return launch256w<LAY, EPI_BF16_DOT>(a, s);
      case EPI_DGELU: return launch256w<LAY, EPI_DGELU>(a, s);
      case EPI_MUL: return launch256w<LAY, EPI_MUL>(a, s);
    }
  } else {
    switch (epi) {
      case EPI_BF16: return launch256w<LAY, EPI_BF16>(a, s);
      case EPI_BF16_DOT: return launch256w<LAY, EPI_BF16_DOT>(a, s);
      case EPI_DGELU: return launch256w<LAY, EPI_DGELU>(a, s);
      case EPI_DSILU: return launch256w<LAY, EPI_DSILU>(a, s);
      case EPI_MUL: return launch256w<LAY, EPI_MUL>(a, s);
    }
  }
  reed_set_error("reed_gemm(256w): epilogue %d not built for this layout", epi);
  return REED_ERR_UNSUPPORTED;
}

}

bool reed_gemm256w_eligible(int layout, int epi, const GemmArgs& a, int splits) {
  const bool epi_ok = layout == LAY_NT ? (epi == EPI_BF16 || epi == EPI_GELU || epi == EPI_SILU || epi == EPI_GATE_RES ||
                                          epi == EPI_GELU_G || epi == EPI_SILU_G || epi == EPI_RES_BF16 || epi == EPI_LS_RES ||
                                          epi == EPI_BF16_DOT || epi == EPI_DGELU || epi == EPI_MUL)
                                       : (epi == EPI_BF16 || epi == EPI_BF16_DOT || epi == EPI_DGELU || epi == EPI_DSILU || epi == EPI_MUL);
  return (layout == LAY_NT || layout == LAY_NN) && splits <= 1 && a.K % WBK == 0 && a.K >= 2 * WBK && a.N % 128 == 0 && epi_ok;
}

int reed_gemm256w_launch(int layout, int epi, GemmArgs a, hipStream_t stream) {
  if (layout == LAY_NT) return dispatch256w<LAY_NT>(epi, a, stream);
  return dispatch256w<LAY_NN>(epi, a, stream);
}

int reed_gemm_forced_tile();

static int w4_deal(int n, const int* M, const int* N, const int* has_db, int ncu, unsigned* item) {
  if (n < 1 || n > 4 || ncu < 8 || (ncu & 7) != 0 || ncu > 256) return 0;
  const int wpx = ncu / 8;
  auto pack = [](int p, int mode, int mu, int nu, int vm, int vn, int db) {
    return (unsigned)(p | mode << 2 | mu << 6 | nu << 14 | (vm - 1) << 22 | (vn - 1) << 24 | db << 26);
  };
  int count = 0, bias_only = 0;
  double equiv = 0.0;
  for (int i = 0; i < n; ++i) {
    if (M[i] <= 0 || N[i] <= 0 || M[i] % 128 || N[i] % 128 || M[i] / 128 > 255 || N[i] / 128 > 255) return 0;
    const int Mu = M[i] / 128, Nu = N[i] / 128, fm = Mu / 2, fn = Nu / 2, rm = Mu & 1, rn = Nu & 1;
    count += fm * fn + (rn ? cdiv(Mu, 3) : 0) + (rm ? cdiv(2 * fn, 3) : 0);
    if (has_db[i] && !rn) bias_only += cdiv(2 * fm, 4);
    equiv += 0.25 * Mu * Nu;
  }
  constexpr double minfill = 0.7;
  if (count > ncu || equiv < minfill * ncu) return 0;
  const bool use_bias_only = count + bias_only <= ncu;
  std::vector<unsigned> seq;
  for (int i = 0; i < n; ++i) {
    const int Mu = M[i] / 128, Nu = N[i] / 128, fm = Mu / 2, fn = Nu / 2, rm = Mu & 1, rn = Nu & 1;
    const bool colmajor = fm < fn;
    const int db = has_db[i] ? 1 : 0;
    std::vector<std::pair<double, unsigned>> its;
    for (int u = 0; u < (colmajor ? fn : fm); ++u)
      for (int v = 0; v < (colmajor ? fm : fn); ++v) {
        const int tm = colmajor ? v : u, tn = colmajor ? u : v;
        its.push_back({u + 0.5, pack(i, 0, 2 * tm, 2 * tn, 2, 2, (db && !rn && !use_bias_only && tn == 0) ? 1 : 0)});
      }
    if (rn)
      for (int c = 0; 3 * c < Mu; ++c)
        its.push_back({colmajor ? fn + 0.51 : (3 * c + 1.5) / 2.0, pack(i, 6, 3 * c, 2 * fn, std::min(3, Mu - 3 * c), 1, db)});
    if (rm)
      for (int c = 0; 3 * c < 2 * fn; ++c)
        its.push_back({colmajor ? (3 * c + 1.5) / 2.0 : fm + 0.51,
                       pack(i, 7, 2 * fm, 3 * c, 1, std::min(3, 2 * fn - 3 * c), (db && !rn && c == 0) ? 1 : 0)});
    if (db && !rn && use_bias_only)
      for (int c = 0; 4 * c < 2 * fm; ++c)
        its.push_back({(colmajor ? fn : fm) + 1.0, pack(i, 8, 4 * c, 0, std::min(4, 2 * fm - 4 * c), 1, 1)});
    std::stable_sort(its.begin(), its.end(),
                     [](const std::pair<double, unsigned>& x, const std::pair<double, unsigned>& y) { return x.first < y.first; });
    for (auto& e : its) seq.push_back(e.second);
  }
  const int T = (int)seq.size();
  if (T > ncu) return 0;
  for (int q = 0; q < 256; ++q) item[q] = 0xFFFFFFFFu;
  for (int x = 0; x < 8; ++x) {
    const int b = (int)((long)x * T / 8), e = (int)((long)(x + 1) * T / 8);
    for (int q = b; q < e; ++q) item[x * wpx + (q - b)] = seq[q];
  }
  return T;
}

extern "C" int reed_wgrad_group_deal(int n, const int* n_out, const int* k_in, const int* has_bias, int cus, unsigned* items) {
  if (!n_out || !k_in || !has_bias || !items) return 0;
  return w4_deal(n, n_out, k_in, has_bias, cus, items);
}

int reed_gemm256w_tn_group_launch(int n, const GemmArgs* probs, hipStream_t stream, int* launched) {
  *launched = 0;
  static const int w4mode = getenv("REED_WGRAD_W4") ? atoi(getenv("REED_WGRAD_W4")) : -1;
  if (w4mode == 0 || reed_gemm_forced_tile() == 128) return REED_OK;
  if (reed_concurrent_comm() && w4mode != 1) return REED_OK;
  if (n < 1 || n > 4) return REED_OK;
  const int ncu = reed_num_cus();
  TnGroupW g;
  memset(&g, 0, sizeof(g));
  int M[4], N[4], db[4];
  for (int i = 0; i < n; ++i) {
    const GemmArgs& a = probs[i];
    if (a.K < 2 * WBK || a.slab_stride != 0 || a.K != probs[0].K) return REED_OK;
    M[i] = a.M; N[i] = a.N; db[i] = a.dbias != nullptr;
    g.a[i] = a;
  }
  if (w4_deal(n, M, N, db, ncu, g.item) == 0) return REED_OK;
  g.n = n;
  g.wpx = ncu / 8;
  static bool attr_set = false;
  if (!attr_set) {
    hipError_t e = hipFuncSetAttribute((const void*)gemm256w_tn_group_kernel<0>, hipFuncAttributeMaxDynamicSharedMemorySize, LDS_TN);
    if (e == hipSuccess) e = hipFuncSetAttribute((const void*)gemm256w_tn_group_kernel<1>, hipFuncAttributeMaxDynamicSharedMemorySize, LDS_TN);
    if (e != hipSuccess) { reed_set_error("gemm256w: cannot reserve LDS: %s", hipGetErrorString(e)); return (int)e; }
    attr_set = true;
// ... 10 lines not shown
```

reed_amd/csrc/gemm_f32.hip:

```cpp
#include <stdlib.h>
#include <string.h>

#include <type_traits>
#include <utility>

#include "../../include/reed_hip.h"
#include "gemm.h"

#ifndef REED_FP32
#error "gemm_f32.hip belongs to the fp32-operand build (-DREED_FP32) only"
#endif

int reed_num_cus();

namespace {

constexpr int BK = 16;
typedef __attribute__((ext_vector_type(16))) float f32x16;

template <int W>
struct Geo {
  static constexpr int BT = 64 * W, NT = 64 * W * W, LDT = BT + 32, TILE_FLOATS = BK * LDT, PP = BT * 4 / NT;
};

// ... 185 lines not shown
        if (C) C[(long)m * a.ldc + n] = v;
        C2[(long)m * a.ldc2 + n] = act_fwd(epi, a.act_variant, v);
        break;
      case EPI_GATE_RES: {
        if (C2) C2[(long)m * a.ldc2 + n] = v;
        const float g = a.gate[(long)(m / a.rows_per_gate) * a.ldgate + n];
        C[(long)m * a.ldc + n] = Rf[(long)m * a.ldr + n] + g * v;
      } break;
      case EPI_LS_RES: C[(long)m * a.ldc + n] = Rf[(long)m * a.ldr + n] + a.gate[n] * v; break;
      case EPI_GELU_G: case EPI_SILU_G: {
        float av, gv;
        if (epi == EPI_GELU_G) gelu_tanh_both(v, av, gv);
        else silu_both(v, av, gv);
        if (C) C[(long)m * a.ldc + n] = gv;
        C2[(long)m * a.ldc2 + n] = av;
      } break;
      case EPI_MUL: C[(long)m * a.ldc + n] = v * Rf[(long)m * a.ldr + n]; break;
      case EPI_DGELU: C[(long)m * a.ldc + n] = v * gelu_tanh_grad_f(Rf[(long)m * a.ldr + n]); break;
      case EPI_DSILU: C[(long)m * a.ldc + n] = v * silu_grad_f(Rf[(long)m * a.ldr + n]); break;
      case EPI_RES_BF16: C[(long)m * a.ldc + n] = v + Rf[(long)m * a.ldr + n]; break;
      case EPI_F32: {
        float* cp = C + (long)z * a.slab_stride + (long)m * a.ldc + n;
        *cp = a.accumulate ? *cp + v : v;
      } break;
      case EPI_ADDF32_RB: C[(long)m * a.ldc + n] += v; break;
      case EPI_ATOMIC_F32: atomicAdd(C + (long)m * a.ldc + n, v); break;
    }
  };
  static_for<2>([&](auto I) { static_for<2>([&](auto J) { static_for<16>([&](auto Rr) { elem(I, J, Rr); }); }); });
  if (do_dbias && tid < BM) {
    const int m = m0 + tid;
    if (m < a.M) {
      if (gridDim.y > 1) a.dbias[(long)z * a.slab_stride + m] = bsum;
      else if (a.accumulate) a.dbias[m] += bsum;
      else a.dbias[m] = bsum;
    }
  }
}

template <int LAY, int W>
int launch_w(const GemmArgs& a, int epi, int splits, hipStream_t stream, ConvGeo cg = ConvGeo{0, 0, 0, 0, 0}) {
  constexpr int lds = 2 * 2 * Geo<W>::TILE_FLOATS * (int)sizeof(float);
  static bool attr_set = false;
  if (!attr_set) {
    hipError_t e = hipFuncSetAttribute((const void*)gemm_f32_kernel<LAY, W>, hipFuncAttributeMaxDynamicSharedMemorySize, lds);
    if (e != hipSuccess) { reed_set_error("gemm_f32: cannot reserve LDS: %s", hipGetErrorString(e)); return (int)e; }
    attr_set = true;
  }
  dim3 grid(cdiv(a.M, Geo<W>::BT) * cdiv(a.N, Geo<W>::BT), splits, 1);
  REED_KLAUNCH((gemm_f32_kernel<LAY, W>), grid, dim3(Geo<W>::NT), lds, stream, a, epi, cg);
  REED_LAUNCH_CHECK();
  return REED_OK;
}

template <int LAY>
int launch(const GemmArgs& a, int epi, int splits, hipStream_t stream) {
  return launch_w<LAY, 2>(a, epi, splits, stream);
}

}

static int g_force_tile = 0, g_cu_reserve = 0, g_concurrent_comm = 0;
extern "C" int reed_gemm_force_tile(int tile) { g_force_tile = tile; return 0; }
extern "C" int reed_set_cu_reserve(int n) { g_cu_reserve = n > 0 ? n : 0; return 0; }
extern "C" int reed_set_concurrent_comm(int on) { g_concurrent_comm = on ? 1 : 0; return 0; }
int reed_num_cus() {
  static int n = 0;
  if (!n) {
    int dev = 0;
    hipDeviceProp_t p;
    if (hipGetDevice(&dev) == hipSuccess && hipGetDeviceProperties(&p, dev) == hipSuccess) n = p.multiProcessorCount;
    if (n <= 0) n = 256;
  }
  return n - g_cu_reserve > 32 ? n - g_cu_reserve : 32;
}
extern "C" int reed_planning_cus(void) { return reed_num_cus(); }

int reed_gemm_tn_group_launch(int, const GemmArgs*, hipStream_t) {
  reed_set_error("reed_wgrad_group: not built for fp32 operands (one reed_gemm(TN) per weight instead)");
  return REED_ERR_UNSUPPORTED;
}

extern "C" int reed_wgrad_group_deal(int, const int*, const int*, const int*, int, unsigned*) { return 0; }

static int conv3x3_f32(const char* what, const void* act, const void* w, const float* bias, float* out, int64_t ldc, int B, int Hi,
                       int Wi, int C, int N, int upsample, int down, int accumulate, void* stream) {
  REED_CHECK_ARG(act && w && out && B > 0 && Hi > down && Wi > down && C > 0 && N > 0, "%s: empty problem", what);
  REED_CHECK_ARG(upsample == 0 || upsample == 1, "%s: upsample must be 0 or 1 (nearest x2)", what);
  REED_CHECK_ARG(C % 4 == 0 && N % 4 == 0 && ldc >= N, "%s(fp32): C=%d and N=%d must be multiples of 4, ldc >= N", what, C, N);
  const long M = down ? (long)B * (Hi >> 1) * (Wi >> 1) : (long)B * (Hi << upsample) * (Wi << upsample);
  REED_CHECK_ARG(M < (1l << 31) - 256 && (long)B * Hi * Wi < (1l << 31), "%s: too many positions for one call", what);
  REED_CHECK_ARG(((uintptr_t)act % 16) == 0 && ((uintptr_t)w % 16) == 0 && (!bias || (uintptr_t)bias % 16 == 0),
                 "%s: operands must be 16-byte aligned", what);
  GemmArgs a;
  memset(&a, 0, sizeof(a));
  a.P = (const float*)act;
  a.Q = (const float*)w;
  a.ldp = 9 * C;
  a.ldq = 9 * C;
  a.M = (int)M;
  a.N = N;
  a.K = 9 * C;
  a.C = out;
  a.ldc = ldc;
  a.bias = bias;
  a.accumulate = accumulate;
  a.rows_per_gate = 1;
  a.ksplit_len = a.K;
  return launch_w<LAY_NT, 2>(a, EPI_F32, 1, (hipStream_t)stream, ConvGeo{C, Hi, Wi, upsample, down});
}

extern "C" int reed_conv3x3(const void* act, const void* w, const float* bias, float* out, int64_t ldc, int B, int Hi, int Wi, int C,
                            int N, int upsample, int accumulate, void* stream) {
  return conv3x3_f32("reed_conv3x3", act, w, bias, out, ldc, B, Hi, Wi, C, N, upsample, 0, accumulate, stream);
}

extern "C" int reed_conv3x3_down(const void* act, const void* w, const float* bias, float* out, int64_t ldc, int B, int Hi, int Wi,
                                 int C, int N, int accumulate, void* stream) {
  REED_CHECK_ARG(Hi > 1 && Wi > 1, "reed_conv3x3_down: Hi=%d, Wi=%d must be at least 2", Hi, Wi);
  return conv3x3_f32("reed_conv3x3_down", act, w, bias, out, ldc, B, Hi, Wi, C, N, 0, 1, accumulate, stream);
}

int reed_gemm_launch(int layout, int epi, GemmArgs a, int splits, hipStream_t stream) {
  REED_CHECK_ARG(a.M > 0 && a.N > 0 && a.K > 0, "reed_gemm: empty problem M=%d N=%d K=%d", a.M, a.N, a.K);
  REED_CHECK_ARG(a.ldp % 4 == 0 && a.ldq % 4 == 0 && a.N % 4 == 0, "reed_gemm(fp32): leading dims and N must be multiples of 4 elements");
  REED_CHECK_ARG(((uintptr_t)a.P % 16) == 0 && ((uintptr_t)a.Q % 16) == 0, "reed_gemm: operands must be 16-byte aligned");
  if (layout == LAY_TN_TALL || layout == LAY_TN_WIDE) layout = LAY_TN;
  if (layout == LAY_TN) REED_CHECK_ARG(a.M % 4 == 0, "reed_gemm(TN, fp32): M=%d must be a multiple of 4", a.M);
  else REED_CHECK_ARG(a.K % 4 == 0, "reed_gemm(NT/NN, fp32): K=%d must be a multiple of 4", a.K);
  switch (epi) {
    case EPI_BF16: case EPI_GELU: case EPI_SILU: case EPI_GATE_RES: case EPI_DGELU: case EPI_DSILU: case EPI_F32:
    case EPI_ADDF32_RB: case EPI_ATOMIC_F32: case EPI_QGELU: case EPI_RES_BF16: case EPI_LS_RES:
    case EPI_GELU_G: case EPI_SILU_G: case EPI_MUL: break;
    default: reed_set_error("reed_gemm: unknown epilogue %d", epi); return REED_ERR_ARG;
  }
  if (splits < 1) splits = 1;
  const int ksteps = cdiv(a.K, 64);
  const int per = cdiv(ksteps, splits);
  splits = cdiv(ksteps, per);
  a.ksplit_len = per * 64;
  if (splits > 1)
    REED_CHECK_ARG(epi == EPI_ATOMIC_F32 || (epi == EPI_F32 && a.slab_stride > 0),
                   "reed_gemm: split-K needs the atomic or slab fp32 epilogue");
  switch (layout) {
    case LAY_NT: return launch<LAY_NT>(a, epi, splits, stream);
    case LAY_NN: return launch<LAY_NN>(a, epi, splits, stream);
    case LAY_TN: return launch<LAY_TN>(a, epi, splits, stream);
  }
  reed_set_error("reed_gemm: unknown layout %d", layout);
  return REED_ERR_ARG;
}
```

reed_amd/csrc/norm.hip:

```cpp
#include "../../include/reed_hip.h"
#include "common.hpp"

namespace {

constexpr int MAXV = 5;

__device__ __forceinline__ f32x4 ld_bf4(const bf16* p) {
  bf16x4 v = *(const bf16x4*)p;
  return f32x4{bf2f(v[0]), bf2f(v[1]), bf2f(v[2]), bf2f(v[3])};
}
__device__ __forceinline__ void st_bf4(bf16* p, f32x4 v) {
  bf16x4 o;
#pragma unroll
  for (int j = 0; j < 4; ++j) o[j] = f2bf(v[j]);
  *(bf16x4*)p = o;
}

template <bool NT>
__global__ __launch_bounds__(256) void ln_mod_fwd_kernel(const float* __restrict__ x, const bf16* __restrict__ shift,
                                                         const bf16* __restrict__ scale, long ldmod,
                                                         bf16* __restrict__ h, float* __restrict__ mean,
                                                         float* __restrict__ rstd, int M, int D, int T, float eps) {
  const int row = blockIdx.x * 4 + (threadIdx.x >> 6);
  if (row >= M) return;
  const int lane = threadIdx.x & 63, nv = D >> 2;
  const float* xr = x + (long)row * D;
  f32x4 v[MAXV];
  float s = 0.f;
#pragma unroll
  for (int k = 0; k < MAXV; ++k) {
    int idx = lane + 64 * k;
    const bool ok = idx < nv;
    if constexpr (NT) v[k] = __builtin_nontemporal_load((const f32x4*)(xr + (ok ? idx : 0) * 4));
    else v[k] = *(const f32x4*)(xr + (ok ? idx : 0) * 4);
    const float m = ok ? 1.f : 0.f;
    v[k] *= m;
    s += v[k][0] + v[k][1] + v[k][2] + v[k][3];
  }
  bf16* hr = h + (long)row * D;
  if (scale == nullptr) {
#pragma unroll
    for (int k = 0; k < MAXV; ++k) {
      int idx = lane + 64 * k;
      if (idx < nv) st_bf4(hr + idx * 4, v[k]);
    }
    return;
  }
  const float mu = wave_sum(s) / D;
  float q = 0.f;
#pragma unroll
  for (int k = 0; k < MAXV; ++k) {
    int idx = lane + 64 * k;
    if (idx < nv) {
#pragma unroll
      for (int j = 0; j < 4; ++j) { float d = v[k][j] - mu; q += d * d; }
    }
  }
  const float r = rsqrtf(wave_sum(q) / D + eps);
  if (lane == 0 && mean) { mean[row] = mu; rstd[row] = r; }
  const bf16* sc = scale + (long)(row / T) * ldmod;
  const bf16* sh = shift + (long)(row / T) * ldmod;
  f32x4 av[MAXV], bv[MAXV];
#pragma unroll
  for (int k = 0; k < MAXV; ++k) {
    int idx = lane + 64 * k;
    int ic = idx < nv ? idx : 0;
    av[k] = ld_bf4(sc + ic * 4);
    bv[k] = ld_bf4(sh + ic * 4);
  }
#pragma unroll
  for (int k = 0; k < MAXV; ++k) {
    int idx = lane + 64 * k;
    if (idx < nv) {
      f32x4 o;
#pragma unroll
      for (int j = 0; j < 4; ++j) o[j] = (v[k][j] - mu) * r * bfround(1.f + av[k][j]) + bv[k][j];
      st_bf4(hr + idx * 4, o);
    }
  }
}

template <bool GATE>
__global__ __launch_bounds__(256) void ln_mod_bwd_kernel(const bf16* __restrict__ dh, const float* __restrict__ x,
                                                         const float* __restrict__ mean, const float* __restrict__ rstd,
                                                         const bf16* __restrict__ scale, long ldmod,
                                                         float* __restrict__ dx, float* __restrict__ part,
                                                         const bf16* __restrict__ y, const bf16* __restrict__ gate,
                                                         long ldgate, bf16* __restrict__ dy, float* __restrict__ part_g,
                                                         float* __restrict__ part_dy, int M, int D, int T) {
  extern __shared__ __attribute__((aligned(16))) float red[];
  const int wave = threadIdx.x >> 6, lane = threadIdx.x & 63, nv = D >> 2;
  const int row0 = blockIdx.x * 16 + wave * 4;
  const long smp = (blockIdx.x * 16) / T;
  const bf16* sc = scale + smp * ldmod;
  f32x4 s1[MAXV], ps[MAXV], pq[MAXV];
  f32x4 gv[GATE ? MAXV : 1], pg[GATE ? MAXV : 1], pd[GATE ? MAXV : 1];
#pragma unroll
  for (int k = 0; k < MAXV; ++k) {
    int idx = lane + 64 * k;
    ps[k] = f32x4{0, 0, 0, 0};
    pq[k] = f32x4{0, 0, 0, 0};
    if (GATE) { pg[k] = f32x4{0, 0, 0, 0}; pd[k] = f32x4{0, 0, 0, 0}; }
    if (idx < nv) {
      f32x4 a = ld_bf4(sc + idx * 4);
#pragma unroll
      for (int j = 0; j < 4; ++j) s1[k][j] = bfround(1.f + a[j]);
// ... 97 lines not shown

typedef unsigned int u32x2_t __attribute__((ext_vector_type(2)));
typedef unsigned int u32x4_t __attribute__((ext_vector_type(4)));
__device__ __forceinline__ __amdgpu_buffer_rsrc_t row_rsrc(const void* p, unsigned bytes) {
  return __builtin_amdgcn_make_buffer_rsrc(const_cast<void*>(p), 0, p ? bytes : 0u, 0x00020000);
}
template <int NF, int TS>
struct HalfRow {
  static constexpr int NE = 4 * NF + TS, NV = NF + TS;
  int vo[NV > 0 ? NV : 1];
  __device__ __forceinline__ HalfRow(int hf, int lane) {
    const int half0 = hf * 64 * NE;
#pragma unroll
    for (int k = 0; k < NF; ++k) vo[k] = half0 + (lane + 64 * k) * 4;
#pragma unroll
    for (int t = 0; t < TS; ++t) vo[NF + t] = half0 + 256 * NF + 64 * t + lane;
  }
  template <int AUX = 0>
  __device__ __forceinline__ void ld_f32(__amdgpu_buffer_rsrc_t rs, int soff, float (&v)[NE]) const {
#pragma unroll
    for (int k = 0; k < NF; ++k) {
      f32x4 t = __builtin_bit_cast(f32x4, __builtin_amdgcn_raw_buffer_load_b128(rs, vo[k] * 4, soff, AUX));
#pragma unroll
      for (int j = 0; j < 4; ++j) v[4 * k + j] = t[j];
    }
#pragma unroll
    for (int t = 0; t < TS; ++t)
      v[4 * NF + t] = __builtin_bit_cast(float, __builtin_amdgcn_raw_buffer_load_b32(rs, vo[NF + t] * 4, soff, AUX));
  }
  template <int AUX = 0>
  __device__ __forceinline__ void st_f32(__amdgpu_buffer_rsrc_t rs, int soff, const float (&v)[NE]) const {
#pragma unroll
    for (int k = 0; k < NF; ++k)
      __builtin_amdgcn_raw_buffer_store_b128(
          __builtin_bit_cast(u32x4_t, f32x4{v[4 * k], v[4 * k + 1], v[4 * k + 2], v[4 * k + 3]}), rs, vo[k] * 4, soff, AUX);
#pragma unroll
    for (int t = 0; t < TS; ++t)
      __builtin_amdgcn_raw_buffer_store_b32(__builtin_bit_cast(unsigned, v[4 * NF + t]), rs, vo[NF + t] * 4, soff, AUX);
  }
#ifdef REED_FP32
  template <int AUX = 0>
  __device__ __forceinline__ void ld_bf(__amdgpu_buffer_rsrc_t rs, int soff, float (&v)[NE]) const { ld_f32<AUX>(rs, soff, v); }
  template <int AUX = 0>
  __device__ __forceinline__ void st_bf(__amdgpu_buffer_rsrc_t rs, int soff, const float (&v)[NE]) const { st_f32<AUX>(rs, soff, v); }
#else
  template <int AUX = 0>
  __device__ __forceinline__ void ld_bf(__amdgpu_buffer_rsrc_t rs, int soff, float (&v)[NE]) const {
#pragma unroll
    for (int k = 0; k < NF; ++k) {
      const bf16x4 t = __builtin_bit_cast(bf16x4, __builtin_amdgcn_raw_buffer_load_b64(rs, vo[k] * 2, soff, AUX));
#pragma unroll
      for (int j = 0; j < 4; ++j) v[4 * k + j] = bf2f(t[j]);
    }
#pragma unroll
    for (int t = 0; t < TS; ++t)
      v[4 * NF + t] = bf2f(__builtin_bit_cast(bf16, (unsigned short)__builtin_amdgcn_raw_buffer_load_b16(rs, vo[NF + t] * 2, soff, AUX)));
  }
  template <int AUX = 0>
  __device__ __forceinline__ void st_bf(__amdgpu_buffer_rsrc_t rs, int soff, const float (&v)[NE]) const {
#pragma unroll
    for (int k = 0; k < NF; ++k) {
      bf16x4 o;
#pragma unroll
      for (int j = 0; j < 4; ++j) o[j] = f2bf(v[4 * k + j]);
      __builtin_amdgcn_raw_buffer_store_b64(__builtin_bit_cast(u32x2_t, o), rs, vo[k] * 2, soff, AUX);
    }
#pragma unroll
    for (int t = 0; t < TS; ++t)
      __builtin_amdgcn_raw_buffer_store_b16(__builtin_bit_cast(unsigned short, f2bf(v[4 * NF + t])), rs, vo[NF + t] * 2, soff, AUX);
  }
#endif
  __device__ __forceinline__ void st_lds(float* p, const float (&v)[NE]) const {
#pragma unroll
    for (int k = 0; k < NF; ++k) *(f32x4*)(p + vo[k]) = f32x4{v[4 * k], v[4 * k + 1], v[4 * k + 2], v[4 * k + 3]};
#pragma unroll
    for (int t = 0; t < TS; ++t) p[vo[NF + t]] = v[4 * NF + t];
  }
};

#ifndef REED_LNB_NT
#define REED_LNB_NT 1
#endif
constexpr int LNB_AUX = REED_LNB_NT ? 2 : 0;
template <bool GATE, int NF, int TS>
__global__ __launch_bounds__(512, 4) void ln_mod_bwd2_kernel(
    const bf16* __restrict__ dh, const float* __restrict__ x, const float* __restrict__ mean,
    const float* __restrict__ rstd, const bf16* __restrict__ scale, long ldmod, float* __restrict__ dx,
    float* __restrict__ part, const bf16* __restrict__ y, const bf16* __restrict__ gate, long ldgate,
    bf16* __restrict__ dy, float* __restrict__ part_g, float* __restrict__ part_dy, int M, int T) {
  using HR = HalfRow<NF, TS>;
  constexpr int NE = HR::NE, D = 128 * NE, HB = sizeof(bf16);
  extern __shared__ __attribute__((aligned(16))) float red[];
  const int lane = threadIdx.x & 63;
  const int wave = __builtin_amdgcn_readfirstlane(threadIdx.x >> 6);
  const int rg = wave >> 1, hf = wave & 1;
  const HR hr(hf, lane);
  float* rsum = red + 8 * D;
  const long blk0 = (long)blockIdx.x * 16;
  const long smp = blk0 / T;
  const __amdgpu_buffer_rsrc_t rsX = row_rsrc(x + blk0 * D, 16 * D * 4), rsDX = row_rsrc(dx + blk0 * D, 16 * D * 4),
                               rsDH = row_rsrc(dh + blk0 * D, 16 * D * HB),
                               rsY = row_rsrc(GATE ? y + blk0 * D : nullptr, 16 * D * HB),
                               rsDY = row_rsrc(GATE ? dy + blk0 * D : nullptr, 16 * D * HB);
  float s1[NE], gv[GATE ? NE : 1], ps[NE], pq[NE], pg[GATE ? NE : 1], pd[GATE ? NE : 1];
  hr.ld_bf(row_rsrc(scale + smp * ldmod, D * HB), 0, s1);
#pragma unroll
  for (int e = 0; e < NE; ++e) {
    s1[e] = bfround(1.f + s1[e]);
    ps[e] = 0.f;
    pq[e] = 0.f;
    if (GATE) { pg[e] = 0.f; pd[e] = 0.f; }
  }
  if constexpr (GATE) hr.ld_bf(row_rsrc(gate + smp * ldgate, D * HB), 0, gv);
#pragma unroll 1
  for (int rr = 0; rr < 4; ++rr) {
    const int lr = rg * 4 + rr;
    const float mu = mean[blk0 + lr], r = rstd[blk0 + lr];
    float xh[NE], gy[NE], o[NE], yin[GATE ? NE : 1];
    hr.template ld_f32<LNB_AUX>(rsX, lr * D * 4, xh);
    hr.ld_bf(rsDH, lr * D * HB, gy);
    hr.template ld_f32<LNB_AUX>(rsDX, lr * D * 4, o);
    if constexpr (GATE) hr.template ld_bf<LNB_AUX>(rsY, lr * D * HB, yin);
    float a1 = 0.f, a2 = 0.f;
#pragma unroll
    for (int e = 0; e < NE; ++e) {
      const float g = gy[e];
      const float xv = (xh[e] - mu) * r;
      xh[e] = xv;
      gy[e] = g * s1[e];
      a1 += gy[e];
      a2 += gy[e] * xv;
      ps[e] += g;
      pq[e] += g * xv;
    }
    a1 = wave_sum(a1);
    a2 = wave_sum(a2);
    if (lane == 0) *(float2*)(rsum + (lr * 2 + hf) * 2) = make_float2(a1, a2);
    __syncthreads();
    {
      const f32x4 t = *(const f32x4*)(rsum + lr * 4);
      a1 = (t[0] + t[2]) / D;
      a2 = (t[1] + t[3]) / D;
    }
#pragma unroll
    for (int e = 0; e < NE; ++e) o[e] += r * (gy[e] - a1 - xh[e] * a2);
    hr.template st_f32<LNB_AUX>(rsDX, lr * D * 4, o);
    if constexpr (GATE) {
#pragma unroll
      for (int e = 0; e < NE; ++e) {
        const float dg = bfround(o[e]);
        o[e] = dg * gv[e];
        pg[e] += bfround(dg * yin[e]);
        pd[e] += bfround(o[e]);
      }
      hr.st_bf(rsDY, lr * D * HB, o);
    }
  }
  hr.st_lds(red + (rg * 2 + 0) * D, ps);
  hr.st_lds(red + (rg * 2 + 1) * D, pq);
  __syncthreads();
  float* out = part + (long)blockIdx.x * 2 * D;
  for (int i = threadIdx.x; i < 2 * D; i += 512) out[i] = red[i] + red[2 * D + i] + red[4 * D + i] + red[6 * D + i];
  if constexpr (GATE) {
    __syncthreads();
    hr.st_lds(red + (rg * 2 + 0) * D, pg);
    hr.st_lds(red + (rg * 2 + 1) * D, pd);
    __syncthreads();
    float* og = part_g + (long)blockIdx.x * D;
    for (int i = threadIdx.x; i < D; i += 512) og[i] = red[i] + red[2 * D + i] + red[4 * D + i] + red[6 * D + i];
    if (part_dy) {
      float* od = part_dy + (long)blockIdx.x * D;
      for (int i = threadIdx.x; i < D; i += 512) od[i] = red[D + i] + red[3 * D + i] + red[5 * D + i] + red[7 * D + i];
    }
  }
}

template <bool GATE>
bool launch_ln_mod_bwd2(hipStream_t stream, const bf16* dh, const float* x, const float* mean, const float* rstd,
                        const bf16* scale, long ldmod, float* dx, float* part, const bf16* y, const bf16* gate,
                        long ldgate, bf16* dy, float* part_g, float* part_dy, int M, int D, int T) {
#define REED_LNB2(NF_, TS_)                                                                                          \
  if (D == 128 * (4 * NF_ + TS_)) {                                                                                   \
    REED_KLAUNCH((ln_mod_bwd2_kernel<GATE, NF_, TS_>), dim3(M / 16), dim3(512), (8 * D + 64) * sizeof(float),  \
                       stream, dh, x, mean, rstd, scale, ldmod, dx, part, y, gate, ldgate, dy, part_g, part_dy, M, T); \
    return true;                                                                                                      \
  }
  REED_LNB2(0, 1) REED_LNB2(0, 2) REED_LNB2(0, 3) REED_LNB2(1, 0) REED_LNB2(1, 2) REED_LNB2(2, 0) REED_LNB2(2, 1)
#undef REED_LNB2
  return false;
}

__global__ __launch_bounds__(256) void gate_bwd_kernel(const float* __restrict__ dx, const bf16* __restrict__ y,
                                                       const bf16* __restrict__ gate, long ldgate,
                                                       bf16* __restrict__ dy, float* __restrict__ part,
                                                       float* __restrict__ part_dy, int M, int D, int T) {
  extern __shared__ __attribute__((aligned(16))) float red[];
  const int wave = threadIdx.x >> 6, lane = threadIdx.x & 63, nv = D >> 2;
  const int row0 = blockIdx.x * 16 + wave * 4;
  const bf16* gp = gate + (long)((blockIdx.x * 16) / T) * ldgate;
  f32x4 gv[MAXV], pg[MAXV], pd[MAXV];
#pragma unroll
  for (int k = 0; k < MAXV; ++k) {
    int idx = lane + 64 * k;
    pg[k] = f32x4{0, 0, 0, 0};
    pd[k] = f32x4{0, 0, 0, 0};
    if (idx < nv) gv[k] = ld_bf4(gp + idx * 4);
  }
  for (int rr = 0; rr < 4; ++rr) {
    const int row = row0 + rr;
    if (row >= M) break;
    f32x4 din[MAXV], yin[MAXV];
#pragma unroll
    for (int k = 0; k < MAXV; ++k) {
      int idx = lane + 64 * k;
      int ic = idx < nv ? idx : 0;
      din[k] = *(const f32x4*)(dx + (long)row * D + ic * 4);
      yin[k] = ld_bf4(y + (long)row * D + ic * 4);
    }
#pragma unroll
    for (int k = 0; k < MAXV; ++k) {
      int idx = lane + 64 * k;
      if (idx < nv) {
        f32x4 d = din[k];
        f32x4 yv = yin[k], o;
#pragma unroll
        for (int j = 0; j < 4; ++j) {
          float dg = bfround(d[j]);
          o[j] = dg * gv[k][j];
          pg[k][j] += bfround(dg * yv[j]);
          pd[k][j] += bfround(o[j]);
        }
        st_bf4(dy + (long)row * D + idx * 4, o);
      }
    }
  }
#pragma unroll
  for (int k = 0; k < MAXV; ++k) {
    int idx = lane + 64 * k;
    if (idx < nv) *(f32x4*)(red + wave * D + idx * 4) = pg[k];
  }
  __syncthreads();
  float* out = part + (long)blockIdx.x * D;
  for (int i = threadIdx.x; i < D; i += 256) out[i] = red[i] + red[D + i] + red[2 * D + i] + red[3 * D + i];
  if (part_dy) {
    __syncthreads();
#pragma unroll
    for (int k = 0; k < MAXV; ++k) {
      int idx = lane + 64 * k;
      if (idx < nv) *(f32x4*)(red + wave * D + idx * 4) = pd[k];
    }
    __syncthreads();
    float* o2 = part_dy + (long)blockIdx.x * D;
    for (int i = threadIdx.x; i < D; i += 256) o2[i] = red[i] + red[D + i] + red[2 * D + i] + red[3 * D + i];
  }
}

__global__ __launch_bounds__(256) void transpose_bf16_kernel(const bf16* __restrict__ src, bf16* __restrict__ dst, int R,
                                                             int C) {
  __shared__ bf16 t[64][66];
  const int r0 = blockIdx.y * 64, c0 = blockIdx.x * 64;
  const int tx = threadIdx.x & 63, ty = threadIdx.x >> 6;
  for (int i = ty; i < 64; i += 4)
    if (r0 + i < R && c0 + tx < C) t[i][tx] = src[(long)(r0 + i) * C + c0 + tx];
  __syncthreads();
  for (int i = ty; i < 64; i += 4)
    if (c0 + i < C && r0 + tx < R) dst[(long)(c0 + i) * R + r0 + tx] = t[tx][i];
}
// ... 68 lines not shown
  for (; c < chunks; ++c) s += *(const f32x4*)(p + (long)c * st);
  bf16x4 o;
#pragma unroll
  for (int e = 0; e < 4; ++e) o[e] = f2bf(s[e]);
  *(bf16x4*)(dmod + (long)b * ld + pl.off[j] + d) = o;
}

__global__ __launch_bounds__(256) void token_mean_fwd_kernel(const float* __restrict__ x, bf16* __restrict__ out,
                                                             int T, int D) {
  const int b = blockIdx.y, d = blockIdx.x * 256 + threadIdx.x;
  if (d >= D) return;
  const float* p = x + (long)b * T * D + d;
  float s = 0.f;
  for (int t = 0; t < T; ++t) s += p[(long)t * D];
  out[(long)b * D + d] = f2bf(s / T);
}
__global__ __launch_bounds__(256) void token_mean_bwd_kernel(const bf16* __restrict__ dmean, float* __restrict__ dx,
                                                             int T, int D) {
  const int b = blockIdx.y, d = blockIdx.x * 256 + threadIdx.x;
  if (d >= D) return;
  const float g = bf2f(dmean[(long)b * D + d]) / T;
  float* p = dx + (long)b * T * D + d;
  for (int t = 0; t < T; ++t) p[(long)t * D] += g;
}

__global__ __launch_bounds__(256) void cast_bf16_kernel(const float* __restrict__ s, bf16* __restrict__ d, long n4,
                                                        long n) {
  long i = (long)blockIdx.x * 256 + threadIdx.x;
  const long stride = (long)gridDim.x * 256;
  for (; i < n4; i += stride) st_bf4(d + i * 4, *(const f32x4*)(s + i * 4));
  if (blockIdx.x == 0 && threadIdx.x < (n & 3)) {
    long k = (n4 << 2) + threadIdx.x;
    d[k] = f2bf(s[k]);
  }
}

__global__ __launch_bounds__(256) void colsum_partial_kernel(const bf16* __restrict__ x, long ld, float* __restrict__ part,
                                                             int M, int N) {
  const int col = (blockIdx.x * 256 + threadIdx.x) * 4;
  if (col >= N) return;
  const int r0 = blockIdx.y * 256;
  f32x4 s = {0, 0, 0, 0};
  const bf16* base = x + (long)r0 * ld + col;
  if (r0 + 256 <= M) {
#pragma unroll 1
    for (int rr = 0; rr < 256; rr += 8) {
      f32x4 v[8];
#pragma unroll
      for (int k = 0; k < 8; ++k) v[k] = ld_bf4(base + (long)(rr + k) * ld);
#pragma unroll
      for (int k = 0; k < 8; ++k) s += v[k];
    }
  } else {
    for (int r = r0; r < M; ++r) s += ld_bf4(x + (long)r * ld + col);
  }
  *(f32x4*)(part + (long)blockIdx.y * N + col) = s;
}
__global__ __launch_bounds__(256) void colsum_reduce_kernel(const float* __restrict__ part, int nsl, float* __restrict__ out,
                                                            int N, int accumulate) {
  __shared__ float red[4][64];
  const int col = blockIdx.x * 64 + (threadIdx.x & 63), grp = threadIdx.x >> 6;
  float s = 0.f;
  if (col < N)
    for (int z = grp; z < nsl; z += 4) s += part[(long)z * N + col];
  red[grp][threadIdx.x & 63] = s;
  __syncthreads();
  if (grp == 0 && col < N) {
    float t = (red[0][threadIdx.x] + red[1][threadIdx.x]) + (red[2][threadIdx.x] + red[3][threadIdx.x]);
    out[col] = accumulate ? out[col] + t : t;
  }
}

__global__ __launch_bounds__(256) void reduce_slabs_kernel(const float* __restrict__ slabs, long stride, int ns,
                                                           float* __restrict__ out, long n, int accumulate) {
  long i = (long)blockIdx.x * 256 + threadIdx.x;
  if (i >= n) return;
  float s = accumulate ? out[i] : 0.f;
  for (int z = 0; z < ns; ++z) s += slabs[(long)z * stride + i];
  out[i] = s;
}

}

extern "C" int reed_ln_modulate_fwd(const float* x, const void* shift, const void* scale, int64_t ldmod,
                                    void* h, float* mean, float* rstd, int M, int D, int T, float eps,
                                    void* stream) {
  REED_CHECK_ARG(x && h, "ln_modulate_fwd: null pointer");
  REED_CHECK_ARG(D % 4 == 0 && D <= 256 * MAXV, "ln_modulate: D=%d unsupported (multiple of 4, <= %d)", D, 256 * MAXV);
  REED_CHECK_ARG(M > 0 && T > 0, "ln_modulate: bad M=%d T=%d", M, T);
  REED_CHECK_ARG((scale == nullptr) == (shift == nullptr), "ln_modulate: shift and scale must both be given or both NULL");
  if ((long)M * D * 4 >= (256l << 20))
    REED_KLAUNCH(ln_mod_fwd_kernel<true>, dim3(cdiv(M, 4)), dim3(256), 0, (hipStream_t)stream, x, (const bf16*)shift,
                 (const bf16*)scale, (long)ldmod, (bf16*)h, mean, rstd, M, D, T, eps);
  else
    REED_KLAUNCH(ln_mod_fwd_kernel<false>, dim3(cdiv(M, 4)), dim3(256), 0, (hipStream_t)stream, x, (const bf16*)shift,
                 (const bf16*)scale, (long)ldmod, (bf16*)h, mean, rstd, M, D, T, eps);
  REED_LAUNCH_CHECK();
  return REED_OK;
}

extern "C" int reed_ln_modulate_bwd(const void* dh, const float* x, const float* mean, const float* rstd,
                                    const void* scale, int64_t ldmod, float* dx, float* part, int M, int D,
                                    int T, void* stream) {
  REED_CHECK_ARG(dh && x && mean && rstd && scale && dx && part, "ln_modulate_bwd: null pointer");
  REED_CHECK_ARG(D % 4 == 0 && D <= 256 * MAXV, "ln_modulate: D=%d unsupported", D);
  REED_CHECK_ARG(T % 16 == 0 && M % 16 == 0, "ln_modulate_bwd: T=%d, M=%d must be multiples of 16", T, M);
  if (launch_ln_mod_bwd2<false>((hipStream_t)stream, (const bf16*)dh, x, mean, rstd, (const bf16*)scale, (long)ldmod, dx,
                                part, nullptr, nullptr, 0l, nullptr, nullptr, nullptr, M, D, T)) {
    REED_LAUNCH_CHECK();
    return REED_OK;
  }
    REED_KLAUNCH(ln_mod_bwd_kernel<false>, dim3(M / 16), dim3(256), 8 * D * sizeof(float), (hipStream_t)stream,
                 (const bf16*)dh, x, mean, rstd, (const bf16*)scale, (long)ldmod, dx, part, (const bf16*)nullptr,
                 (const bf16*)nullptr, 0l, (bf16*)nullptr, (float*)nullptr, (float*)nullptr, M, D, T);
  REED_LAUNCH_CHECK();
  return REED_OK;
}

extern "C" int reed_ln_modulate_bwd_gate(const void* dh, const float* x, const float* mean, const float* rstd,
                                         const void* scale, int64_t ldmod, float* dx, float* part, const void* y,
                                         const void* gate, int64_t ldgate, void* dy, float* part_g, float* part_dy,
                                         int M, int D, int T, void* stream) {
  REED_CHECK_ARG(dh && x && mean && rstd && scale && dx && part, "ln_modulate_bwd_gate: null pointer");
  REED_CHECK_ARG(y && gate && dy && part_g, "ln_modulate_bwd_gate: null gate operand");
  REED_CHECK_ARG(D % 4 == 0 && D <= 256 * MAXV, "ln_modulate: D=%d unsupported", D);
  REED_CHECK_ARG(T % 16 == 0 && M % 16 == 0, "ln_modulate_bwd_gate: T=%d, M=%d must be multiples of 16", T, M);
  if (launch_ln_mod_bwd2<true>((hipStream_t)stream, (const bf16*)dh, x, mean, rstd, (const bf16*)scale, (long)ldmod, dx,
                               part, (const bf16*)y, (const bf16*)gate, (long)ldgate, (bf16*)dy, part_g, part_dy, M, D, T)) {
    REED_LAUNCH_CHECK();
    return REED_OK;
  }
    REED_KLAUNCH(ln_mod_bwd_kernel<true>, dim3(M / 16), dim3(256), 8 * D * sizeof(float), (hipStream_t)stream,
                 (const bf16*)dh, x, mean, rstd, (const bf16*)scale, (long)ldmod, dx, part, (const bf16*)y,
                 (const bf16*)gate, (long)ldgate, (bf16*)dy, part_g, part_dy, M, D, T);
  REED_LAUNCH_CHECK();
  return REED_OK;
}

extern "C" int reed_transpose_bf16(const void* src, void* dst, int R, int C, void* stream) {
  REED_CHECK_ARG(src && dst && R > 0 && C > 0, "transpose_bf16: bad args");
  if (R % 64 == 0 && C % 64 == 0 && ((uintptr_t)src % 8) == 0 && ((uintptr_t)dst % 8) == 0)
    REED_KLAUNCH(transpose_bf16_v4_kernel, dim3(C / 64, R / 64), dim3(256), 0, (hipStream_t)stream, (const bf16*)src, (bf16*)dst, R, C);
  else
    REED_KLAUNCH(transpose_bf16_kernel, dim3(cdiv(C, 64), cdiv(R, 64)), dim3(256), 0, (hipStream_t)stream,
                 (const bf16*)src, (bf16*)dst, R, C);
  REED_LAUNCH_CHECK();
  return REED_OK;
}

__global__ __launch_bounds__(256) void rowsum_stage1_kernel(const float* __restrict__ part, int R, float* __restrict__ part2,
                                                            int N) {
  const int col = blockIdx.x * 256 + threadIdx.x;
  if (col >= N) return;
  const int r0 = blockIdx.y * 64, r1 = min(R, r0 + 64);
  float s = 0.f;
  int r = r0;
  for (; r + 8 <= r1; r += 8) {
    float v[8];
#pragma unroll
    for (int k = 0; k < 8; ++k) v[k] = part[(long)(r + k) * N + col];
#pragma unroll
    for (int k = 0; k < 8; ++k) s += v[k];
  }
  for (; r < r1; ++r) s += part[(long)r * N + col];
  part2[(long)blockIdx.y * N + col] = s;
}

extern "C" int reed_rowsum_f32(const float* part, int R, float* ws, float* out, int N, int accumulate, void* stream) {
  REED_CHECK_ARG(part && out && R > 0 && N > 0, "rowsum_f32: bad args");
  if (R > 256 && ws) {
    const int R2 = cdiv(R, 64);
    REED_KLAUNCH(rowsum_stage1_kernel, dim3(cdiv(N, 256), R2), dim3(256), 0, (hipStream_t)stream, part, R, ws, N);
    REED_KLAUNCH(rowsum_f32_kernel, dim3(cdiv(N, 64)), dim3(256), 0, (hipStream_t)stream, ws, R2, out, N, accumulate);
  } else {
    REED_KLAUNCH(rowsum_f32_kernel, dim3(cdiv(N, 64)), dim3(256), 0, (hipStream_t)stream, part, R, out, N, accumulate);
  }
  REED_LAUNCH_CHECK();
  return REED_OK;
}

extern "C" int reed_gate_bwd(const float* dx, const void* y, const void* gate, int64_t ldgate, void* dy,
                             float* part, float* part_dy, int M, int D, int T, void* stream) {
  REED_CHECK_ARG(dx && y && gate && dy && part, "gate_bwd: null pointer");
  REED_CHECK_ARG(D % 4 == 0 && D <= 256 * MAXV, "gate_bwd: D=%d unsupported", D);
  REED_CHECK_ARG(T % 16 == 0 && M % 16 == 0, "gate_bwd: T=%d, M=%d must be multiples of 16", T, M);
  REED_KLAUNCH(gate_bwd_kernel, dim3(M / 16), dim3(256), 4 * D * sizeof(float), (hipStream_t)stream, dx,
                     (const bf16*)y, (const bf16*)gate, (long)ldgate, (bf16*)dy, part, part_dy, M, D, T);
  REED_LAUNCH_CHECK();
  return REED_OK;
}

extern "C" int reed_reduce_mod_parts(const float* const* parts, const int64_t* strides, const int64_t* offs,
                                     int nparts, void* dmod, int64_t lddmod, int B, int D, int chunks,
                                     void* stream) {
  REED_CHECK_ARG(nparts >= 1 && nparts <= 8, "reduce_mod_parts: nparts=%d out of range", nparts);
  PartList pl;
  pl.n = nparts;
  for (int i = 0; i < nparts; ++i) { pl.ptr[i] = parts[i]; pl.stride[i] = strides[i]; pl.off[i] = offs[i]; }
  bool four = (D % 4) == 0 && (lddmod % 4) == 0 && ((uintptr_t)dmod % 8) == 0;
  for (int i = 0; i < nparts; ++i) four = four && (strides[i] % 4) == 0 && (offs[i] % 4) == 0 && ((uintptr_t)parts[i] % 16) == 0;
  if (four)
    REED_KLAUNCH(reduce_mod_parts4_kernel, dim3(cdiv(D, 256), B, nparts), dim3(64), 0, (hipStream_t)stream, pl,
                 (bf16*)dmod, (long)lddmod, D, chunks);
  else
    REED_KLAUNCH(reduce_mod_parts_kernel, dim3(cdiv(D, 256), B, nparts), dim3(256), 0, (hipStream_t)stream, pl,
                 (bf16*)dmod, (long)lddmod, D, chunks);
  REED_LAUNCH_CHECK();
  return REED_OK;
}

extern "C" int reed_token_mean_fwd(const float* x, void* out, int B, int T, int D, void* stream) {
  REED_KLAUNCH(token_mean_fwd_kernel, dim3(cdiv(D, 256), B), dim3(256), 0, (hipStream_t)stream, x, (bf16*)out, T, D);
  REED_LAUNCH_CHECK();
  return REED_OK;
}
extern "C" int reed_token_mean_bwd(const void* dmean, float* dx, int B, int T, int D, void* stream) {
  REED_KLAUNCH(token_mean_bwd_kernel, dim3(cdiv(D, 256), B), dim3(256), 0, (hipStream_t)stream,
                     (const bf16*)dmean, dx, T, D);
  REED_LAUNCH_CHECK();
// ... 36 lines not shown
```

reed_amd/engine.py:

```python
import contextlib
import os
import types

import torch

from . import ops
from .ops import (NT, NN, TN, EPI_BF16, EPI_GELU, EPI_SILU, EPI_GATE_RES, EPI_DGELU, EPI_DSILU, EPI_F32, EPI_ADDF32_RB,
                  EPI_GELU_G, EPI_SILU_G, EPI_MUL)


class Engine:
    DGRAD_NT_MIN_TOKENS = 12289
    SAVE_ACT_GRAD_MIN_TOKENS = 12288
    WGRAD_STREAM_MAX_TOKENS = 0

    def __init__(self, model):
        self.m = model
        self.L = model._layout
        self.A = model._arena
        if self.A.master.device.type != "cuda":
            raise RuntimeError("reed_amd.SiT: parameters are on %s; move the model to an AMD GPU (model.cuda()). "
                               "The hot path has no CPU fallback." % self.A.master.device)
        self.D = model.hidden_size
        self.H = model.num_heads
        self.hd = self.D // self.H
        self.Hm = int(self.D * model.mlp_ratio)
        self.T = model.num_patches
        self.P = model.patch_size
        self.C = model.in_channels
        self.depth = model.depth
        self.NO = self.P * self.P * self.C
        self._dims_ok = set()
        split = model.encoder_depth_text is not None and model.encoder_depth_text != model.encoder_depth
        self.split = split
        self.tap_depth = [model.encoder_depth if (zt == "i" or not split) else model.encoder_depth_text
                          for zt in model.z_types]
        self.reducer = None
        self._dot_delta = {}
        self._ws = None
        self._named = None
        self._sentinel = None
        self._ws_side = None
        self._shadow_t = None
        self.dgrad_nt = None
        self.split_ada_wgrad = None
        self._side = None
        self.wgrad_stream = {"0": False, "1": True}.get(os.environ.get("REED_WGRAD_STREAM", "auto"))
        self.wgrad_stream_max_tokens = self.WGRAD_STREAM_MAX_TOKENS
        self.grad_live = False
        self.table_rows = model.num_classes + (1 if model.class_dropout_prob > 0 else 0)
        self._hb = 2
        self.save_act_grad = None
        self.fused_delta = True
        self._err = None

    def _check_dims(self, prec):
        if prec in self._dims_ok:
            return
        q = 4 if prec == "fp32" else 128
        what = "4 (fp32 operands)" if prec == "fp32" else "128 for the MFMA GEMM tiles"
        for n, v in (("hidden_size", self.D), ("mlp hidden", self.Hm), ("projector_dim", self.m.projector_dim)):
            if v % q:
                raise ValueError(f"{n}={v} must be a multiple of {what}")
        for z in self.m.z_dims:
            if z % q:
                raise ValueError(f"z_dim={z} must be a multiple of {what}")
        self._dims_ok.add(prec)

    def check_errors(self):
        if self._err is not None and int(self._err.item()) != 0:
            self._err.zero_()
            raise IndexError(f"reed_amd.SiT: a class label outside [0, {self.table_rows}) was passed to the model "
                             f"(num_classes={self.m.num_classes}, class_dropout_prob={self.m.class_dropout_prob}); "
                             "the affected forwards used row 0 instead")

    def W(self, name):
        return self._shadow.data_ptr() + self._hb * self.L.off(name)

    def Wf(self, name):
        return self.A.master.data_ptr() + 4 * self.L.off(name)

    def G(self, name):
        return self.A.grad.data_ptr() + 4 * self.L.off(name)

    def ws(self, nfloats, dev):
        if self._ws is None or self._ws.numel() < nfloats:
            self._ws = torch.empty(int(nfloats), dtype=torch.float32, device=dev)
        return self._ws

    def ws_side(self, nfloats, dev):
        if self._ws_side is None or self._ws_side.numel() < nfloats:
            self._ws_side = torch.empty(int(nfloats), dtype=torch.float32, device=dev)
        return self._ws_side

    def forward(self, x, t, y, inference, need_grad, drop):
        prec = getattr(self.m, "precision", "bf16")
        prev = ops.use(prec)
        try:
            return self._forward(x, t, y, inference, need_grad, drop, prec)
        finally:
            ops.use(prev)

    def _forward(self, x, t, y, inference, need_grad, drop, prec):
        m, L = self.m, self.L
        ops.require_cuda(x, "x")
        dev = x.device
        B, C, HW = x.shape[0], x.shape[1], x.shape[-1]
        D, H, hd, Hm, T, P = self.D, self.H, self.hd, self.Hm, self.T, self.P
        if C != self.C or HW != m.input_size or x.shape[-2] != HW:
            raise ValueError(f"input {tuple(x.shape)} does not match (N,{self.C},{m.input_size},{m.input_size})")
        M = B * T
        self._check_dims(prec)
        self._shadow = self.A.ensure_shadow(prec)
        hdt = ops.half_dtype(prec)
        hb = self._hb = hdt.itemsize
        pend = self.A.pending
        if "all" in pend:
            self.A.wait_all()
        elif pend:
            self.A.wait("embed")
        x = x.contiguous().float()
        t = t.contiguous().float()
        y = y.contiguous().long()

        def bf(*s):
            return torch.empty(s, dtype=hdt, device=dev)

        def f32(*s):
            return torch.empty(s, dtype=torch.float32, device=dev)

        sag = self.save_act_grad if self.save_act_grad is not None else M > self.SAVE_ACT_GRAD_MIN_TOKENS
        self._sag = sag
        tp = types.SimpleNamespace(B=B, blocks=[], proj={}, x=x, prec=prec, act_grad=sag) if need_grad else None
        epi_silu = EPI_SILU_G if need_grad and sag else EPI_SILU
        epi_gelu = EPI_GELU_G if need_grad and sag else EPI_GELU
        tok = f32(M, D)
        ops.patch_embed_fwd(x, self.W("x_embedder.proj.weight"), self.W("x_embedder.proj.bias"), self.Wf("pos_embed"),
                            tok, B, C, HW, P, D)
        sin = bf(B, 256)
        ops.timestep_sinusoid(t, sin, B)
        t1p = bf(B, D) if need_grad else None
        t1 = bf(B, D)
        ops.gemm(NT, epi_silu, sin, self.W("t_embedder.mlp.0.weight"), B, D, 256, t1p, 256, 256, D, C2=t1, ldc2=D,
                 bias=self.W("t_embedder.mlp.0.bias"))
        temb = bf(B, D)
        ops.gemm(NT, EPI_BF16, t1, self.W("t_embedder.mlp.2.weight"), B, D, D, temb, D, D, D,
                 bias=self.W("t_embedder.mlp.2.bias"))
        drop_u8 = None
        if drop is not None:
            drop_u8 = drop.to(device=dev, dtype=torch.uint8).contiguous()
        labels_eff = torch.empty(B, dtype=torch.int64, device=dev)
        c = f32(B, D)
        silu_c = bf(B, D)
        if self._err is None:
            self._err = torch.zeros(1, dtype=torch.int32, device=dev)
        ops.label_cond(y, drop_u8, m.num_classes, self.Wf("y_embedder.embedding_table.weight"), temb, labels_eff, c,
                       silu_c, B, D, table_rows=self.table_rows, err=self._err)
        Nall = L.ada_rows
        mod = bf(B, Nall)
        sp = self._shadow.data_ptr()
        mp = mod.data_ptr()
        kh = min(L.ADA_HEAD_BLOCKS, self.depth) if "ada_tail" in pend else 0
        n_head = kh * 6 * D if kh else Nall
        if pend:
            self.A.wait("ada_head")
        ops.gemm(NT, EPI_BF16, silu_c, sp + hb * L.ada_w_off, B, n_head, D, mod, D, D, Nall, bias=sp + hb * L.ada_b_off)
        if need_grad:
            tp.sin, tp.t1p, tp.t1, tp.labels_eff, tp.c, tp.silu_c, tp.mod = sin, t1p, t1, labels_eff, c, silu_c, mod

        if not need_grad:
            xa, xb = tok, f32(M, D)
            h, qkv, o, u = bf(M, D), bf(M, 3 * D), bf(M, D), bf(M, Hm)
        xcur = tok
        zs_by_proj = {}
        for i in range(self.depth):
            b = f"blocks.{i}."
            mb = mp + hb * (i * 6 * D)
            if kh and i == kh:
                self.A.wait("ada_tail")
                ops.gemm(NT, EPI_BF16, silu_c, sp + hb * (L.ada_w_off + n_head * D), B, Nall - n_head, D, mp + hb * n_head,
                         D, D, Nall, bias=sp + hb * (L.ada_b_off + n_head))
                kh = 0
            if pend:
                self.A.wait(f"block{i}")
            if need_grad:
                h, qkv, o, u = bf(M, D), bf(M, 3 * D), bf(M, D), bf(M, Hm)
                h2, a1, y1, y2 = bf(M, D), bf(M, Hm), bf(M, D), bf(M, D)
                mean1, rstd1, mean2, rstd2 = f32(M), f32(M), f32(M), f32(M)
                lse = f32(B, H, T)
                xmid, xout = f32(M, D), f32(M, D)
            else:
                h2, a1, y1, y2 = h, None, None, None
                mean1 = rstd1 = mean2 = rstd2 = lse = None
                xmid = xb if xcur is xa else xa
                xout = xcur
            ops.ln_modulate_fwd(xcur, mb, mb + hb * D, Nall, h, mean1, rstd1, M, D, T)
            ops.gemm(NT, EPI_BF16, h, self.W(b + "attn.qkv.weight"), M, 3 * D, D, qkv, D, D, 3 * D,
                     bias=self.W(b + "attn.qkv.bias"))
            qkv_a, qstats = qkv, None
            if m.qk_norm:
                qkv_a = bf(M, 3 * D)
                qstats = f32(M, 2, H, 2) if need_grad else None
                ops.qk_norm_fwd(qkv, self.Wf(b + "attn.q_norm.weight"), self.Wf(b + "attn.q_norm.bias"),
                                self.Wf(b + "attn.k_norm.weight"), self.Wf(b + "attn.k_norm.bias"), qkv_a, qstats, M, H, hd)
            ops.attention_fwd(qkv_a, o, lse, B, T, H, hd)
            ops.gemm(NT, EPI_GATE_RES, o, self.W(b + "attn.proj.weight"), M, D, D, xmid, D, D, D, C2=y1, ldc2=D,
                     R=xcur, ldr=D, bias=self.W(b + "attn.proj.bias"), gate=mb + 2 * hb * D, ldgate=Nall, rows_per_gate=T)
            ops.ln_modulate_fwd(xmid, mb + 3 * hb * D, mb + 4 * hb * D, Nall, h2, mean2, rstd2, M, D, T)
            ops.gemm(NT, epi_gelu, h2, self.W(b + "mlp.fc1.weight"), M, Hm, D, a1, D, D, Hm, C2=u, ldc2=Hm,
                     bias=self.W(b + "mlp.fc1.bias"))
            ops.gemm(NT, EPI_GATE_RES, u, self.W(b + "mlp.fc2.weight"), M, D, Hm, xout, Hm, Hm, D, C2=y2, ldc2=D,
                     R=xmid, ldr=D, bias=self.W(b + "mlp.fc2.bias"), gate=mb + 5 * hb * D, ldgate=Nall, rows_per_gate=T)
            if need_grad:
                tp.blocks.append(types.SimpleNamespace(x=xcur, mean1=mean1, rstd1=rstd1, h=h, qkv=qkv, qkv_a=qkv_a,
                                                       qstats=qstats, o=o, lse=lse,
                                                       y1=y1, xmid=xmid, mean2=mean2, rstd2=rstd2, h2=h2, a1=a1, u=u,
                                                       y2=y2))
            xcur = xout
            if not inference:
                for j, dj in enumerate(self.tap_depth):
                    if dj == i + 1:
                        zs_by_proj[j] = self._projector_fwd(j, xcur, B, need_grad, tp)
        if kh:
            self.A.wait("ada_tail")
            ops.gemm(NT, EPI_BF16, silu_c, sp + hb * (L.ada_w_off + n_head * D), B, Nall - n_head, D, mp + hb * n_head,
                     D, D, Nall, bias=sp + hb * (L.ada_b_off + n_head))
        if pend:
            self.A.wait_all()
        out = f32(B, C, HW, HW)
        meanF = f32(M) if need_grad else None
        rstdF = f32(M) if need_grad else None
        mf = mp + hb * (self.depth * 6 * D)
        ops.final_layer_fwd(xcur, mf, mf + hb * D, Nall, self.W("final_layer.linear.weight"),
                            self.W("final_layer.linear.bias"), out, meanF, rstdF, B, T, D, C, P)
        if need_grad:
            tp.x_last, tp.meanF, tp.rstdF = xcur, meanF, rstdF
        zs = None
        if not inference:
            if self.split:
                ji, jt = m.z_types.index("i"), m.z_types.index("t")
                zs = [zs_by_proj[ji], zs_by_proj[jt]]
                if need_grad:
                    tp.zs_order = [ji, jt]
            else:
                zs = [zs_by_proj[j] for j in range(len(m.z_dims))]
                if need_grad:
                    tp.zs_order = list(range(len(m.z_dims)))
        return out, zs, tp

    def _projector_fwd(self, j, x, B, need_grad, tp):
        m, D, T = self.m, self.D, self.T
        Pd, Z = m.projector_dim, m.z_dims[j]
        dev = x.device
        img = m.z_types[j] == "i"
        self.A.wait("projectors")
        R = B * T if img else B
        hdt = ops.half_dtype()
        bf = lambda *s: torch.empty(s, dtype=hdt, device=dev)
        xin = bf(R, D)
        if img:
            ops.ln_modulate_fwd(x, None, None, 0, xin, None, None, R, D, T)
        else:
            ops.token_mean_fwd(x, xin, B, T, D)
        pre = f"projectors.{j}."
        epi_silu = EPI_SILU_G if need_grad and self._sag else EPI_SILU
        p1p, p1 = (bf(R, Pd) if need_grad else None), bf(R, Pd)
        ops.gemm(NT, epi_silu, xin, self.W(pre + "0.weight"), R, Pd, D, p1p, D, D, Pd, C2=p1, ldc2=Pd,
                 bias=self.W(pre + "0.bias"))
        p2p, p2 = (bf(R, Pd) if need_grad else None), bf(R, Pd)
        ops.gemm(NT, epi_silu, p1, self.W(pre + "2.weight"), R, Pd, Pd, p2p, Pd, Pd, Pd, C2=p2, ldc2=Pd,
                 bias=self.W(pre + "2.bias"))
        zt = bf(R, Z)
        ops.gemm(NT, EPI_BF16, p2, self.W(pre + "4.weight"), R, Z, Pd, zt, Pd, Pd, Z, bias=self.W(pre + "4.bias"))
        if need_grad:
            tp.proj[j] = types.SimpleNamespace(xin=xin, p1p=p1p, p1=p1, p2p=p2p, p2=p2, R=R)
        return zt.view(B, T, Z) if img else zt

    def _wgrad_block(self, probs, Mtok, acc, dev, side):
        args = [(dy, x, self.G(w), self.G(w.replace("weight", "bias")), N, K) for dy, x, w, N, K in probs]
        if side is not None:
            side.wait_stream(torch.cuda.current_stream())
        with torch.cuda.stream(side) if side is not None else contextlib.nullcontext():
            done = ops.wgrad_group(args, Mtok, accumulate=acc)
        if not done:
            for dy, x, w, N, K in probs:
                self._wgrad(dy, x, w, Mtok, N, K, acc, dev, side=side)
            return
        if side is not None:
            for dy, x, _, _, _ in probs:
                dy.record_stream(side)
                x.record_stream(side)

    def _wgrad(self, dy, x, wname, Mtok, N, K, acc, dev, bias_done=False, side=None):
        bname = wname.replace("weight", "bias")
        lay, split = ops.plan_wgrad(Mtok, N, K)
        if side is None:
            ws = self.ws(split * (N * K + N), dev) if split > 1 else None
            ops.linear_wgrad(dy, x, self.G(wname), dbias=None if bias_done else self.G(bname), accumulate=acc,
                             split_k=split, Mtok=Mtok, N=N, K=K, ws=ws, lay=lay)
            return
        side.wait_stream(torch.cuda.current_stream())
        with torch.cuda.stream(side):
            ws = self.ws_side(split * (N * K + N), dev) if split > 1 else None
            ops.linear_wgrad(dy, x, self.G(wname), dbias=None if bias_done else self.G(bname), accumulate=acc,
                             split_k=split, Mtok=Mtok, N=N, K=K, ws=ws, lay=lay)
        dy.record_stream(side)
        x.record_stream(side)

    def WT(self, name):
        if self._shadow_t is None:
            return None
        seg = self.A.t_seg.get(name)
        return None if seg is None else self._shadow_t.data_ptr() + self._hb * seg[0]

    def _dgrad(self, epi, dy, wname, Mtok, N, K, out, **kw):
        wt = self.WT(wname)
        if wt is not None:
            ops.gemm(NT, epi, dy, wt, Mtok, K, N, out, N, N, K, **kw)
        else:
            ops.gemm(NN, epi, dy, self.W(wname), Mtok, K, N, out, N, K, K, **kw)

    def backward(self, tp, dout, dzs):
        prec = getattr(self.m, "precision", "bf16")
        if getattr(tp, "prec", prec) != prec:
            raise RuntimeError("reed_amd.SiT: model.precision changed between forward and backward")
        prev = ops.use(prec)
        comm = self.reducer is not None and self.reducer.active()
        if comm:
            ops.set_concurrent_comm(True)
        try:
            return self._backward(tp, dout, dzs, ops.half_dtype(prec))
        finally:
            if comm:
                ops.set_concurrent_comm(False)
            ops.use(prev)

    def _backward(self, tp, dout, dzs, hdt):
        m, L = self.m, self.L
        D, H, hd, Hm, T, P, C = self.D, self.H, self.hd, self.Hm, self.T, self.P, self.C
        B = tp.B
        M = B * T
        dev = dout.device
        Nall = L.ada_rows
        hb = self._hb = hdt.itemsize
        self.A.ensure_grad()
        use_t = self.dgrad_nt if self.dgrad_nt is not None else (self.DGRAD_NT_MIN_TOKENS is not None and M >= self.DGRAD_NT_MIN_TOKENS)
        self._shadow_t = self.A.ensure_shadow_t(tp.prec) if (use_t and hb == 2) else None
        acc = self.grad_live
        mp = tp.mod.data_ptr()
        ch = T // 16

        def bf(*s):
            return torch.empty(s, dtype=hdt, device=dev)

        def f32(*s):
            return torch.empty(s, dtype=torch.float32, device=dev)

        group_wgrad = ops.wgrad_group_fits([(D, Hm), (Hm, D), (D, D), (3 * D, D)])
        nws = ops.attention_bwd_ws_floats(B, T, H)
        attn_ws = f32(nws) if nws else None
        dkey = (M, str(hdt), self.reducer is not None and self.reducer.active(), ops.gemm_forced_tile(), ops.cu_reserve(),
                ops.comm_forms())
        dot_delta = self._dot_delta if self.fused_delta and hdt != torch.float32 else {dkey: False}
        side = None
        if self.wgrad_stream or (self.wgrad_stream is None and M <= self.wgrad_stream_max_tokens):
            if self._side is None:
                self._side = torch.cuda.Stream(device=dev)
            side = self._side
        dout = dout.contiguous().float()
        mf = mp + hb * (self.depth * 6 * D)
        hbuf, dlin, dh = bf(M, D), bf(M, self.NO), bf(M, D)
        ops.final_layer_bwd_rows(dout, tp.x_last, tp.meanF, tp.rstdF, mf, mf + hb * D, Nall,
                                 self.W("final_layer.linear.weight"), hbuf, dlin, dh, B, T, D, C, P)
        dx = torch.zeros(M, D, dtype=torch.float32, device=dev)
        partF = f32(M // 16, 2, D)
        pending = {j: d for j, d in enumerate(self.tap_depth)}

        def tap_fires(depth_idx):
            return any(dj == depth_idx and j in tp.proj for j, dj in pending.items())

        def ln_bwd(dh_, x_, mean_, rstd_, scale_ptr, part_, nxt):
            if nxt is None or nxt < 0 or tap_fires(nxt + 1):
                ops.ln_modulate_bwd(dh_, x_, mean_, rstd_, scale_ptr, Nall, dx, part_, M, D, T)
                return None
            nb_ = tp.blocks[nxt]
            dy_, pg_ = bf(M, D), f32(M // 16, D)
            ops.ln_modulate_bwd_gate(dh_, x_, mean_, rstd_, scale_ptr, Nall, dx, part_, nb_.y2,
                                     mp + hb * (nxt * 6 * D + 5 * D), Nall, dy_, pg_, None, M, D, T)
            return dy_, pg_

        pre = ln_bwd(dh, tp.x_last, tp.meanF, tp.rstdF, mf + hb * D, partF, self.depth - 1)
        wsf = self.ws(ops.smallk_ws_floats(D, max(self.NO, C * P * P)), dev)
        ops.smallk_wgrad(hbuf, False, dlin, wsf, self.G("final_layer.linear.weight"), None,
                         self.G("final_layer.linear.bias"), M, D, self.NO, 1, acc)
        dmod = bf(B, Nall)
        offF = self.depth * 6 * D
        ops.reduce_mod_parts([(partF.data_ptr(), 2 * D, offF), (partF.data_ptr() + 4 * D, 2 * D, offF + D)], dmod, Nall,
                             B, D, ch)
        del hbuf, dlin, dh
        split_ada = self.reducer is not None if self.split_ada_wgrad is None else self.split_ada_wgrad
        gp = self.A.grad.data_ptr()
        dmp = dmod.data_ptr()
        red = self.reducer
        fg = (red is not None and red.ada_gather and red.active() and not acc and self.split_ada_wgrad is None)
        if fg:
            split_ada = False
            W = red.world
            g_send, g_recv = red.gather_buffers("dmod", B * Nall, hdt, dev)
            s_send, s_all = red.gather_buffers("silu", B * D, hdt, dev)
            s_send.view(B, D).copy_(tp.silu_c)
            red.gather(s_send, s_all)

        def ada_rows(i):
            return i * 6 * D, (6 * D if i < self.depth else 2 * D)

        def ada_wgrad(i):
            c0, rows = ada_rows(i)
            ops.gemm(TN, EPI_F32, dmp + hb * c0, tp.silu_c, rows, D, B, gp + 4 * (L.ada_w_off + c0 * D), Nall, D, D,
                     dbias=gp + 4 * (L.ada_b_off + c0), accumulate=acc)

        def ada_gather(i):
            c0, rows = ada_rows(i)
            snd = g_send[B * c0:B * (c0 + rows)]
            torch.mul(dmod[:, c0:c0 + rows], 1.0 / W, out=snd.view(B, rows))
            red.gather(snd, g_recv[W * B * c0:W * B * (c0 + rows)])

        def ada_after(i):
            if fg:
                ada_gather(i)
            elif split_ada:
                ada_wgrad(i)

        ada_after(self.depth)
        if self.reducer is not None:
            self.reducer.ready("final")
            if split_ada:
                self.reducer.ready(f"ada{self.depth}")
        proj_left = len([j for j in pending if j in tp.proj])
        dz_by_proj = {}
        if dzs is not None:
            for k, j in enumerate(tp.zs_order):
                dz_by_proj[j] = dzs[k]
        for i in reversed(range(self.depth)):
            for j, dj in pending.items():
                if dj == i + 1 and j in tp.proj:
                    self._projector_bwd(j, tp, dz_by_proj.get(j), dx, B, acc, dev)
                    proj_left -= 1
                    if proj_left == 0 and self.reducer is not None:
                        self.reducer.ready("projectors")
            bk = tp.blocks[i]
            b = f"blocks.{i}."
            mb = mp + hb * (i * 6 * D)
            if pre is not None:
                dy2, pg2 = pre
            else:
                pg2, dy2 = f32(M // 16, D), bf(M, D)
                ops.gate_bwd(dx, bk.y2, mb + 5 * hb * D, Nall, dy2, pg2, M, D, T)
            wg = [] if group_wgrad else None
            if wg is not None:
                wg.append((dy2, bk.u, b + "mlp.fc2.weight", D, Hm))
            else:
                self._wgrad(dy2, bk.u, b + "mlp.fc2.weight", M, D, Hm, acc, dev, side=side)
            da1 = bf(M, Hm)
            self._dgrad(EPI_MUL if tp.act_grad else EPI_DGELU, dy2, b + "mlp.fc2.weight", M, D, Hm, da1, R=bk.a1, ldr=Hm)
            if wg is not None:
                wg.append((da1, bk.h2, b + "mlp.fc1.weight", Hm, D))
            else:
                self._wgrad(da1, bk.h2, b + "mlp.fc1.weight", M, Hm, D, acc, dev, side=side)
            dh2 = dy2 if side is None and wg is None else bf(M, D)
            self._dgrad(EPI_BF16, da1, b + "mlp.fc1.weight", M, Hm, D, dh2)
            pl2 = f32(M // 16, 2, D)
            pg1, dy1 = f32(M // 16, D), bf(M, D)
            ops.ln_modulate_bwd_gate(dh2, bk.xmid, bk.mean2, bk.rstd2, mb + 4 * hb * D, Nall, dx, pl2, bk.y1, mb + 2 * hb * D, Nall,
                                     dy1, pg1, None, M, D, T)
            if wg is not None:
                wg.append((dy1, bk.o, b + "attn.proj.weight", D, D))
            else:
                self._wgrad(dy1, bk.o, b + "attn.proj.weight", M, D, D, acc, dev, side=side)
            do = bf(M, D)
            dqkv = bf(M, 3 * D)
            fused = False
            if dot_delta.get(dkey, True) and attn_ws is not None:
                dpart = f32(M * H * (1 if hd == 64 else 2))
                fused = dot_delta[dkey] = ops.dgrad_with_head_dots(dy1, self.W(b + "attn.proj.weight"), do, bk.o, dpart, M, D, D, hd,
                                                                   wt=self.WT(b + "attn.proj.weight"))
            if fused:
                ops.attention_bwd_dp(bk.qkv_a, do, bk.lse, dpart, dqkv, attn_ws, B, T, H, hd)
            else:
                self._dgrad(EPI_BF16, dy1, b + "attn.proj.weight", M, D, D, do)
                ops.attention_bwd(bk.qkv_a, bk.o, do, bk.lse, dqkv, B, T, H, hd, ws=attn_ws)
            if m.qk_norm:
                nb = (M * 3 * H + 255) // 256
                part = f32(nb, 4 * hd)
                dpre = bf(M, 3 * D)
                ops.qk_norm_bwd(dqkv, bk.qkv, bk.qstats, self.Wf(b + "attn.q_norm.weight"),
                                self.Wf(b + "attn.k_norm.weight"), dpre, part, M, H, hd)
                ops.rowsum_f32(part, nb, self.G(b + "attn.q_norm.weight"), 4 * hd, acc,
                               ws=self.ws((nb + 63) // 64 * 4 * hd, dev))
                dqkv = dpre
            if wg is not None:
                wg.append((dqkv, bk.h, b + "attn.qkv.weight", 3 * D, D))
                self._wgrad_block(wg, M, acc, dev, side)
            else:
                self._wgrad(dqkv, bk.h, b + "attn.qkv.weight", M, 3 * D, D, acc, dev, side=side)
            dh1 = do
            self._dgrad(EPI_BF16, dqkv, b + "attn.qkv.weight", M, 3 * D, D, dh1)
            pl1 = f32(M // 16, 2, D)
            pre = ln_bwd(dh1, bk.x, bk.mean1, bk.rstd1, mb + hb * D, pl1, i - 1)
            o6 = i * 6 * D
            p1, p2 = pl1.data_ptr(), pl2.data_ptr()
            ops.reduce_mod_parts([(p1, 2 * D, o6), (p1 + 4 * D, 2 * D, o6 + D), (pg1.data_ptr(), D, o6 + 2 * D),
                                  (p2, 2 * D, o6 + 3 * D), (p2 + 4 * D, 2 * D, o6 + 4 * D),
                                  (pg2.data_ptr(), D, o6 + 5 * D)], dmod, Nall, B, D, ch)
            tp.blocks[i] = None
            ada_after(i)
            if self.reducer is not None:
                if side is None:
                    self.reducer.ready(f"block{i}")
                    if split_ada:
                        self.reducer.ready(f"ada{i}")
                else:
                    side.wait_stream(torch.cuda.current_stream())
                    with torch.cuda.stream(side):
                        self.reducer.ready(f"block{i}")
                        if split_ada:
                            self.reducer.ready(f"ada{i}")
        if proj_left > 0 and m.z_dims and self.reducer is not None:
            self.reducer.ready("projectors")
        sp = self._shadow.data_ptr()
        if fg:
            red.gather_sync()
            for i in reversed(range(self.depth + 1)):
                c0, rows = ada_rows(i)
                ops.gemm(TN, EPI_F32, g_recv.data_ptr() + hb * W * B * c0, s_all, rows, D, W * B,
                         gp + 4 * (L.ada_w_off + c0 * D), rows, D, D, dbias=gp + 4 * (L.ada_b_off + c0), accumulate=False)
        elif not split_ada:
            ops.gemm(TN, EPI_F32, dmod, tp.silu_c, Nall, D, B, gp + 4 * L.ada_w_off, Nall, D, D,
                     dbias=gp + 4 * L.ada_b_off, accumulate=acc)
        ksteps = Nall // 64
        split = min(64, max(1, ksteps // 8))
        slab = B * D
        wsd = self.ws(split * slab, dev)
        ops.gemm(NN, EPI_F32, dmod, sp + hb * L.ada_w_off, B, D, Nall, wsd, Nall, D, D, split_k=split, slab_stride=slab)
        per = (ksteps + split - 1) // split
        eff = (ksteps + per - 1) // per
        dsilu = f32(B, D)
        ops.reduce_slabs(wsd, slab, eff, dsilu, slab, False)
        dtemb = bf(B, D)
        gt = self.A.view(self.A.grad, "y_embedder.embedding_table.weight")
        if not acc:
            gt.zero_()
        ops.label_cond_bwd(dsilu, tp.c, tp.labels_eff, dtemb, gt, B, D)
        ops.linear_wgrad(dtemb, tp.t1, self.G("t_embedder.mlp.2.weight"), dbias=self.G("t_embedder.mlp.2.bias"),
                         accumulate=acc, Mtok=B, N=D, K=D)
        dt1 = bf(B, D)
        ops.gemm(NN, EPI_MUL if tp.act_grad else EPI_DSILU, dtemb, self.W("t_embedder.mlp.2.weight"), B, D, D, dt1, D, D, D, R=tp.t1p, ldr=D)
        ops.linear_wgrad(dt1, tp.sin, self.G("t_embedder.mlp.0.weight"), dbias=self.G("t_embedder.mlp.0.bias"),
                         accumulate=acc, Mtok=B, N=D, K=256)
        K = C * P * P
        xb = bf(M, K)
        ops.patchify_bf16(tp.x, xb, B, C, tp.x.shape[-1], P, 0)
        wsf = self.ws(ops.smallk_ws_floats(D, max(self.NO, K)), dev)
        ops.smallk_wgrad(dx, True, xb, wsf, self.G("x_embedder.proj.weight"), self.G("x_embedder.proj.bias"), None, M, D,
                         K, 0, acc)
        if self.reducer is not None:
            if fg:
                eb, ee = self.reducer.buckets["embed"]
                self.reducer.ready_range(L.ada_b_off + Nall, ee)
            else:
                if not split_ada:
                    for i in reversed(range(self.depth + 1)):
                        self.reducer.ready(f"ada{i}")
                self.reducer.ready("embed")
        if side is not None:
            torch.cuda.current_stream().wait_stream(side)
        self.grad_live = True
        self._attach_grads()

    def _projector_bwd(self, j, tp, dz, dx, B, acc, dev):
        m, D, T = self.m, self.D, self.T
        Pd, Z = m.projector_dim, m.z_dims[j]
        pj = tp.proj[j]
        R = pj.R
        pre = f"projectors.{j}."
        if dz is None:
            if not acc:
                b, e = self.L.range_of(pre)
                self.A.grad[b:e].zero_()
            return
        dz = dz.reshape(R, Z)
        hdt = ops.half_dtype()
# ... 81 lines not shown
```

reed_amd/ops.py:

```python
import ctypes

import math

import torch

from . import _lib

NT, NN, TN = 0, 1, 2
TN_TALL, TN_WIDE = 3, 4
(EPI_BF16, EPI_GELU, EPI_SILU, EPI_GATE_RES, EPI_DGELU, EPI_DSILU, EPI_F32, EPI_ADDF32_RB, EPI_ATOMIC_F32, EPI_QGELU,
 EPI_RES_BF16, EPI_GELU_ERF, EPI_LS_RES, EPI_BF16_DOT, EPI_GELU_G, EPI_SILU_G, EPI_MUL) = range(17)


def _p(t):
    if t is None:
        return None
    if isinstance(t, int):
        return t
    return t.data_ptr()


def _stream():
    return torch._C._cuda_getCurrentRawStream(torch._C._cuda_getDevice())

# ... 184 lines not shown
    slots = wgrad_slots()
    return n is not None and len(shapes) <= 4 and min_fill * slots <= n <= slots


def wgrad_group_deal(shapes, cus=256, precision="bf16"):
    n = len(shapes)
    ip = ctypes.c_int * n
    items = (ctypes.c_uint * 256)()
    L = _lib.load(precision)
    T = L.reed_wgrad_group_deal(n, ctypes.cast(ip(*[int(q[0]) for q in shapes]), ctypes.c_void_p),
                                ctypes.cast(ip(*[int(q[1]) for q in shapes]), ctypes.c_void_p),
                                ctypes.cast(ip(*[int(bool(q[2])) for q in shapes]), ctypes.c_void_p), int(cus),
                                ctypes.cast(items, ctypes.c_void_p))
    if T <= 0:
        return None
    wpx, out = cus // 8, []
    for x in range(8):
        run = []
        for j in range(wpx):
            it = items[x * wpx + j]
            if it == 0xFFFFFFFF:
                continue
            mode, mu, nu = (it >> 2) & 15, (it >> 6) & 255, (it >> 14) & 255
            vm, vn = ((it >> 22) & 3) + 1, ((it >> 24) & 3) + 1
            rows = {0: 256, 6: 128 * vm, 7: 128, 8: 128 * vm}[mode]
            cols = {0: 256, 6: 128, 7: 128 * vn, 8: 0}[mode]
            run.append(dict(p=it & 3, mode=mode, row=128 * mu, col=128 * nu, rows=rows, cols=cols, bias=(it >> 26) & 1))
        out.append(run)
    assert sum(len(r) for r in out) == T
    return out


def wgrad_group(problems, tokens, accumulate=False):
    n = len(problems)
    vp, ip = ctypes.c_void_p * n, ctypes.c_int * n
    dy = vp(*[_p(q[0]) for q in problems])
    x = vp(*[_p(q[1]) for q in problems])
    dw = vp(*[_p(q[2]) for q in problems])
    db = vp(*[_p(q[3]) for q in problems])
    no = ip(*[int(q[4]) for q in problems])
    ki = ip(*[int(q[5]) for q in problems])
    cast = lambda a: ctypes.cast(a, ctypes.c_void_p)
    L = _lib.load(_PRECISION)
    key = wgrad_group_probe(tokens, [(int(q[4]), int(q[5])) for q in problems]) if wgrad_group_probe is not None else None
    if key is not None:
        e0, e1 = torch.cuda.Event(enable_timing=True), torch.cuda.Event(enable_timing=True)
        e0.record()
    rc = L.reed_wgrad_group(n, cast(dy), cast(x), cast(dw), cast(db), cast(no), cast(ki), int(tokens), int(accumulate),
                            _stream())
    if rc == 1002:
        return False
    _lib.check(rc, "reed_wgrad_group", L)
    if key is not None:
        e1.record()
        gemm_probe_log.append((key, e0, e1))
    return True


def plan_wgrad(Mtok, N, K):
    ktiles = (Mtok + 63) // 64
    slots = wgrad_slots()
    best, best_key = (TN, 1), None
    for lay, bm, bn, rate in WGRAD_TILES:
        if K % bn or N % 128:
            continue
        tiles = ((N + bm - 1) // bm) * (K // bn)
        fill = (N * K) / (tiles * bm * bn)
        for s in range(1, WGRAD_SPLIT_MAX + 1):
            if s > 1 and ktiles // s < 32:
                break
            blocks = tiles * s
            eff = blocks / (((blocks + slots - 1) // slots) * slots)
            dist = abs(math.log((ktiles / s) / 256.0))
            key = (-round(rate * fill * eff / 0.03), dist)
            if best_key is None or key < best_key:
                best, best_key = (lay, s), key
    return best


def reduce_slabs(slabs, stride, n, out, count, accumulate=False):
    _call("reed_reduce_slabs", _p(slabs), stride, n, _p(out), count, int(accumulate), _stream())


def ln_modulate_fwd(x, shift, scale, ldmod, h, mean, rstd, M, D, T, eps=1e-6):
    _call("reed_ln_modulate_fwd", _p(x), _p(shift), _p(scale), ldmod, _p(h), _p(mean), _p(rstd), M, D, T, eps, _stream())


def ln_modulate_bwd(dh, x, mean, rstd, scale, ldmod, dx, part, M, D, T):
    _call("reed_ln_modulate_bwd", _p(dh), _p(x), _p(mean), _p(rstd), _p(scale), ldmod, _p(dx), _p(part), M, D, T, _stream())


def ln_modulate_bwd_gate(dh, x, mean, rstd, scale, ldmod, dx, part, y, gate, ldgate, dy, part_g, part_dy, M, D, T):
    _call("reed_ln_modulate_bwd_gate", _p(dh), _p(x), _p(mean), _p(rstd), _p(scale), ldmod, _p(dx), _p(part), _p(y),
          _p(gate), ldgate, _p(dy), _p(part_g), _p(part_dy), M, D, T, _stream())


def gate_bwd(dx, y, gate, ldgate, dy, part, M, D, T, part_dy=None):
    _call("reed_gate_bwd", _p(dx), _p(y), _p(gate), ldgate, _p(dy), _p(part), _p(part_dy), M, D, T, _stream())


def transpose_bf16(src, dst, R, C):
    _call("reed_transpose_bf16", _p(src), _p(dst), R, C, _stream())


def rowsum_f32(part, R, out, N, accumulate=False, ws=None):
    _call("reed_rowsum_f32", _p(part), R, _p(ws), _p(out), N, int(accumulate), _stream())


def reduce_mod_parts(parts, dmod, lddmod, B, D, chunks):
    n = len(parts)
    ptrs = (ctypes.c_void_p * n)(*[_p(p[0]) for p in parts])
    strides = (ctypes.c_int64 * n)(*[p[1] for p in parts])
    offs = (ctypes.c_int64 * n)(*[p[2] for p in parts])
    _call("reed_reduce_mod_parts", ptrs, strides, offs, n, _p(dmod), lddmod, B, D, chunks, _stream())


def token_mean_fwd(x, out, B, T, D):
    _call("reed_token_mean_fwd", _p(x), _p(out), B, T, D, _stream())


def token_mean_bwd(dmean, dx, B, T, D):
    _call("reed_token_mean_bwd", _p(dmean), _p(dx), B, T, D, _stream())


def cast_bf16(src, dst, n):
    _call("reed_cast_bf16", _p(src), _p(dst), n, _stream())


def attention_fwd(qkv, o, lse, B, T, H, hd):
    _call("reed_attention_fwd", _p(qkv), _p(o), _p(lse), B, T, H, hd, _stream())


def attention_bwd(qkv, o, do, lse, dqkv, B, T, H, hd, ws=None):
    if ws is None:
        _call("reed_attention_bwd", _p(qkv), _p(o), _p(do), _p(lse), _p(dqkv), B, T, H, hd, _stream())
    else:
        _call("reed_attention_bwd_ws", _p(qkv), _p(o), _p(do), _p(lse), _p(dqkv), _p(ws), B, T, H, hd, _stream())


def attention_bwd_dp(qkv, do, lse, dpart, dqkv, ws, B, T, H, hd):
    _call("reed_attention_bwd_dp", _p(qkv), _p(do), _p(lse), _p(dpart), _p(dqkv), _p(ws), B, T, H, hd, _stream())


def dgrad_with_head_dots(dy, w, dx, o, dpart, M, N, K, hd, wt=None):
    L = _lib.load(_PRECISION)
    if wt is not None:
        rc = L.reed_gemm(NT, EPI_BF16_DOT, _p(dy), N, _p(wt), N, M, K, N, _p(dx), K, _p(dpart), 0, _p(o), K, None, None, 0, hd, None, 0,
                         1, 0, _stream())
    else:
        rc = L.reed_gemm(NN, EPI_BF16_DOT, _p(dy), N, _p(w), K, M, K, N, _p(dx), K, _p(dpart), 0, _p(o), K, None, None, 0, hd, None, 0,
                         1, 0, _stream())
    if rc == 1002:
        return False
    _lib.check(rc, "reed_gemm", L)
    return True


def attention_bwd_ws_floats(B, T, H):
    return int(_lib.load(_PRECISION).reed_attention_bwd_ws_floats(B, T, H))


def qk_norm_fwd(qkv, qw, qb, kw, kb, out, stats, M, H, hd, eps=1e-5):
    _call("reed_qk_norm_fwd", _p(qkv), _p(qw), _p(qb), _p(kw), _p(kb), _p(out), _p(stats), M, H, hd, eps, _stream())


def qk_norm_part_floats(M, H, hd):
    return int(_lib.load().reed_qk_norm_bwd_part_floats(M, H, hd))


def qk_norm_bwd(dn, qkv, stats, qw, kw, dpre, part, M, H, hd):
    _call("reed_qk_norm_bwd", _p(dn), _p(qkv), _p(stats), _p(qw), _p(kw), _p(dpre), _p(part), M, H, hd, _stream())


def patch_embed_fwd(x, w, bias, pos, tokens, B, C, HW, P, D):
    _call("reed_patch_embed_fwd", _p(x), _p(w), _p(bias), _p(pos), _p(tokens), B, C, HW, P, D, _stream())


def patchify_bf16(x, out, B, C, HW, P, order):
    _call("reed_patchify_bf16", _p(x), _p(out), B, C, HW, P, order, _stream())


def smallk_ws_floats(Dw, KS):
    return int(_lib.load().reed_smallk_wgrad_ws_floats(Dw, KS))


def smallk_wgrad(wide, wide_is_f32, small, ws, out, colsum_wide, colsum_small, M, Dw, KS, layout, accumulate):
    _call("reed_smallk_wgrad", _p(wide), int(wide_is_f32), _p(small), _p(ws), _p(out), _p(colsum_wide),
          _p(colsum_small), M, Dw, KS, layout, int(accumulate), _stream())


def timestep_sinusoid(t, out, B, dim=256, max_period=10000.0):
    _call("reed_timestep_sinusoid", _p(t), _p(out), B, dim, max_period, _stream())


def label_cond(labels, drop, num_classes, table, t_emb, labels_out, c, silu_c, B, D, table_rows=None, err=None):
    if table_rows is None:
        table_rows = num_classes + 1
    _call("reed_label_cond", _p(labels), _p(drop), num_classes, table_rows, _p(table), _p(t_emb), _p(labels_out), _p(c),
          _p(silu_c), _p(err), B, D, _stream())


def label_cond_bwd(dsilu_c, c, labels_eff, dt_emb, dtable, B, D):
    _call("reed_label_cond_bwd", _p(dsilu_c), _p(c), _p(labels_eff), _p(dt_emb), _p(dtable), B, D, _stream())


def final_layer_fwd(x, shift, scale, ldmod, w, bias, out, mean, rstd, B, T, D, C, P, eps=1e-6):
    _call("reed_final_layer_fwd", _p(x), _p(shift), _p(scale), ldmod, _p(w), _p(bias), _p(out), _p(mean), _p(rstd),
          B, T, D, C, P, eps, _stream())


def final_layer_bwd_rows(dout, x, mean, rstd, shift, scale, ldmod, w, hbuf, dlin, dh, B, T, D, C, P):
    _call("reed_final_layer_bwd_rows", _p(dout), _p(x), _p(mean), _p(rstd), _p(shift), _p(scale), ldmod, _p(w),
          _p(hbuf), _p(dlin), _p(dh), B, T, D, C, P, _stream())
# ... 121 lines not shown
```

Measured before the change: 1336.

## Order consumer kernels to follow the producing GEMM's tile completion order

Adds an 'age order' mapping so LayerNorm-modulate forward/backward and attention forward process row strips in the order the preceding GEMM's XCD-partitioned tile deal produced them. Each strip is handled on the same XCD run as its producer and in reverse completion age. The aim is to hit data still resident in the per-XCD L2 / MALL instead of refetching from HBM. It costs extra index arithmetic per block (including a binary search for uneven runs), plus host-side plumbing to record the last GEMM deal.

```diff
diff --git a/include/reed_hip.h b/include/reed_hip.h
--- a/include/reed_hip.h
+++ b/include/reed_hip.h
@@ -17,6 +17,10 @@
 int reed_wgrad_group(int n, const void* const* dy, const void* const* x, float* const* dw, float* const* dbias,
                      const int* n_out, const int* k_in, int tokens, int accumulate, void* stream);
 int reed_wgrad_group_deal(int n, const int* n_out, const int* k_in, const int* has_bias, int cus, unsigned* items);
+
+int reed_gemm_last_deal(int* m_ntn_gm);
+int reed_gemm_deal_for(int M, int N, int* ntn_gm);
+int reed_age_order(int M, int ntn, int gm, int* strips, int* runs);
 
 int reed_set_cu_reserve(int n);
 int reed_planning_cus(void);
@@ -43,6 +47,17 @@
                               const void* gate, int64_t ldgate, void* dy, float* part_g, float* part_dy,
                               int M, int D, int T, void* stream);
 
+int reed_ln_modulate_fwd_ordered(const float* x, const void* shift, const void* scale, int64_t ldmod,
+                                 void* h, float* mean, float* rstd, int M, int D, int T, float eps,
+                                 int order_ntn, int order_gm, void* stream);
+int reed_ln_modulate_bwd_ordered(const void* dh, const float* x, const float* mean, const float* rstd,
+                                 const void* scale, int64_t ldmod, float* dx, float* part, int M, int D,
+                                 int T, int order_ntn, int order_gm, void* stream);
+int reed_ln_modulate_bwd_gate_ordered(const void* dh, const float* x, const float* mean, const float* rstd,
+                                      const void* scale, int64_t ldmod, float* dx, float* part, const void* y,
+                                      const void* gate, int64_t ldgate, void* dy, float* part_g, float* part_dy,
+                                      int M, int D, int T, int order_ntn, int order_gm, void* stream);
+
 int reed_gate_bwd(const float* dx, const void* y, const void* gate, int64_t ldgate, void* dy,
                   float* part, float* part_dy, int M, int D, int T, void* stream);
 int reed_transpose_bf16(const void* src, void* dst, int R, int C, void* stream);
@@ -54,6 +69,8 @@
 
 int reed_attention_fwd(const void* qkv, void* o, float* lse, int B, int T, int H, int hd,
                        void* stream);
+int reed_attention_fwd_ordered(const void* qkv, void* o, float* lse, int B, int T, int H, int hd,
+                               int order_ntn, int order_gm, void* stream);
 int reed_attention_bwd(const void* qkv, const void* o, const void* d_o, const float* lse,
                        void* dqkv, int B, int T, int H, int hd, void* stream);
 int64_t reed_attention_bwd_ws_floats(int B, int T, int H);
diff --git a/reed_amd/csrc/age_order.hpp b/reed_amd/csrc/age_order.hpp
--- /dev/null
+++ b/reed_amd/csrc/age_order.hpp
@@ -0,0 +1,87 @@
+#pragma once
+#include <hip/hip_runtime.h>
+
+__host__ __device__ __forceinline__ void w_run_of(int xcd, int nwg, int& run0, int& runlen) {
+  const int q = nwg >> 3, r = nwg & 7;
+  run0 = xcd < r ? xcd * (q + 1) : r * (q + 1) + (xcd - r) * q;
+  runlen = q + (xcd < r ? 1 : 0);
+}
+__host__ __device__ __forceinline__ void w_tile_of(int b, int ntm, int ntn, int GM, int& tm, int& tn) {
+  const int per_group = GM * ntn;
+  const int group = b / per_group, first_m = group * GM;
+  const int gs = ntm - first_m < GM ? ntm - first_m : GM;
+  tm = first_m + (b % per_group) % gs;
+  tn = (b % per_group) / gs;
+}
+
+struct AgeOrder {
+  int ntn, gm;
+};
+
+__host__ __device__ __forceinline__ int age_rows_before(int P, int ntm, int ntn, int GM) {
+  const int per_group = GM * ntn, group = P / per_group, first_m = group * GM;
+  if (first_m >= ntm) return ntm;
+  const int gs = ntm - first_m < GM ? ntm - first_m : GM;
+  const int k = P - group * per_group - (ntn - 1) * gs;
+  return first_m + (k < 0 ? 0 : k > gs ? gs : k);
+}
+
+struct AgeRuns {
+  int n, even;
+  int end[8];
+};
+__host__ __device__ __forceinline__ AgeRuns age_runs(int M, AgeOrder od) {
+  AgeRuns r;
+  r.n = r.even = 0;
+#pragma unroll
+  for (int x = 0; x < 8; ++x) r.end[x] = 0;
+  if (M <= 0 || od.ntn <= 0 || od.gm <= 0) return r;
+  const int ntm = (M + 255) / 256, nwg = ntm * od.ntn;
+  r.n = ntm;
+  bool even = true;
+#pragma unroll
+  for (int x = 0; x < 8; ++x) {
+    int run0, runlen;
+    w_run_of(x, nwg, run0, runlen);
+    r.end[x] = age_rows_before(run0 + runlen, ntm, od.ntn, od.gm);
+    even = even && r.end[x] == (x + 1) * r.end[0];
+  }
+  r.even = even ? r.end[0] : 0;
+  return r;
+}
+
+__host__ __device__ __forceinline__ int age_order_strip(int v, const AgeRuns& r, int* run_out = nullptr) {
+  if (r.even > 0) {
+    const int run = v & 7;
+    if (run_out) *run_out = run;
+    return (run + 1) * r.even - 1 - (v >> 3);
+  }
+  int cnt[8], maxc = 0, prev = 0;
+#pragma unroll
+  for (int x = 0; x < 8; ++x) {
+    cnt[x] = r.end[x] - prev;
+    prev = r.end[x];
+    maxc = cnt[x] > maxc ? cnt[x] : maxc;
+  }
+  int lo = 0, hi = maxc - 1, before = 0;
+  while (lo < hi) {
+    const int mid = (lo + hi + 1) >> 1;
+    int s = 0;
+#pragma unroll
+    for (int x = 0; x < 8; ++x) s += cnt[x] < mid ? cnt[x] : mid;
+    if (s <= v) lo = mid;
+    else hi = mid - 1;
+  }
+#pragma unroll
+  for (int x = 0; x < 8; ++x) before += cnt[x] < lo ? cnt[x] : lo;
+  int k = v - before, strip = 0, run = 0;
+#pragma unroll
+  for (int x = 0; x < 8; ++x) {
+    if (cnt[x] > lo) {
+      if (k == 0) { strip = r.end[x] - 1 - lo; run = x; }
+      --k;
+    }
+  }
+  if (run_out) *run_out = run;
+  return strip;
+}
diff --git a/reed_amd/csrc/attention.hip b/reed_amd/csrc/attention.hip
--- a/reed_amd/csrc/attention.hip
+++ b/reed_amd/csrc/attention.hip
@@ -4,6 +4,7 @@
 #include <utility>
 
 #include "../../include/reed_hip.h"
+#include "age_order.hpp"
 #include "common.hpp"
 
 #ifndef REED_ATTN_LD_AUX
@@ -1003,7 +1004,7 @@
 
 template <int HD, bool KSP = true, bool QSP = true>
 __global__ __launch_bounds__(512, 2) void attn_fwd256v_kernel(const bf16* __restrict__ qkv, bf16* __restrict__ o,
-                                                             float* __restrict__ lse, int H, int nitems) {
+                                                             float* __restrict__ lse, int H, int nitems, AgeRuns ord) {
   extern __shared__ __attribute__((aligned(16))) char smem[];
   constexpr int T = 256;
   constexpr int KS = Cfg<HD>::KS, DT = Cfg<HD>::DT, NCH = Cfg<HD>::NCH;
@@ -1032,8 +1033,14 @@
 #pragma unroll
     for (int j = 0; j < 5; ++j) piece(wave_rows, rs, j);
   };
-  auto base_of = [&](int item) -> const bf16* {
-    if (item >= nitems) return nullptr;
+  auto item_of = [&](int w) -> int {
+    if (ord.n <= 0) return w;
+    const int sw = w / H;
+    return age_order_strip(sw, ord) * H + (w - sw * H);
+  };
+  auto base_of = [&](int w) -> const bf16* {
+    if (w >= nitems) return nullptr;
+    const int item = item_of(w);
     const int b = item / H, h = item - b * H;
     return qkv + (long)b * T * tok + h * HD;
   };
@@ -1171,7 +1178,7 @@
       }
     }
     __builtin_amdgcn_sched_barrier(0);
-    pit = it;
+    pit = item_of(it);
   }
   if (pit >= 0) {
     int lane = lane0;
@@ -2387,9 +2394,10 @@
 
 }
 
-extern "C" int reed_attention_fwd(const void* qkv, void* o, float* lse, int B, int T, int H, int hd,
-                                  void* stream) {
+static int attention_fwd(const void* qkv, void* o, float* lse, int B, int T, int H, int hd, AgeOrder od, void* stream) {
   REED_CHECK_ARG(qkv && o, "attention_fwd: null pointer");
+  REED_CHECK_ARG(od.ntn >= 0 && (od.ntn == 0 || od.gm > 0), "attention_fwd: bad order (%d, %d)", od.ntn, od.gm);
+  const AgeRuns ord = age_runs(T == 256 ? B * T : 0, od);
   REED_CHECK_ARG(hd == 64 || hd == 72 || hd == 80, "attention: head_dim %d unsupported (64, 72 or 80)", hd);
   REED_CHECK_ARG(hd != 80 || T <= 256, "attention: head_dim 80 (the I-JEPA ViT-H tower) is built for T <= 256 only (T=%d)", T);
   REED_CHECK_ARG(B > 0 && T > 0 && H > 0, "attention: bad dims B=%d T=%d H=%d", B, T, H);
@@ -2407,11 +2415,11 @@
       if (hd == 64) {
         static int once = set_lds(attn_fwd256v_kernel<64>, lds);
         if (once) return once;
-        REED_KLAUNCH((attn_fwd256v_kernel<64>), grid, dim3(512), lds, (hipStream_t)stream, (const bf16*)qkv, (bf16*)o, lse, H, nitems);
+        REED_KLAUNCH((attn_fwd256v_kernel<64>), grid, dim3(512), lds, (hipStream_t)stream, (const bf16*)qkv, (bf16*)o, lse, H, nitems, ord);
       } else {
         static int once = set_lds(attn_fwd256v_kernel<72>, lds);
         if (once) return once;
-        REED_KLAUNCH((attn_fwd256v_kernel<72>), grid, dim3(512), lds, (hipStream_t)stream, (const bf16*)qkv, (bf16*)o, lse, H, nitems);
+        REED_KLAUNCH((attn_fwd256v_kernel<72>), grid, dim3(512), lds, (hipStream_t)stream, (const bf16*)qkv, (bf16*)o, lse, H, nitems, ord);
       }
       REED_LAUNCH_CHECK();
       return REED_OK;
@@ -2463,6 +2471,16 @@
   }
   REED_LAUNCH_CHECK();
   return REED_OK;
+}
+
+extern "C" int reed_attention_fwd(const void* qkv, void* o, float* lse, int B, int T, int H, int hd,
+                                  void* stream) {
+  return attention_fwd(qkv, o, lse, B, T, H, hd, AgeOrder{0, 0}, stream);
+}
+
+extern "C" int reed_attention_fwd_ordered(const void* qkv, void* o, float* lse, int B, int T, int H, int hd,
+                                          int order_ntn, int order_gm, void* stream) {
+  return attention_fwd(qkv, o, lse, B, T, H, hd, AgeOrder{order_ntn, order_gm}, stream);
 }
 
 extern "C" int reed_attention_bwd(const void* qkv, const void* o, const void* d_o, const float* lse,
diff --git a/reed_amd/csrc/attention_f32.hip b/reed_amd/csrc/attention_f32.hip
--- a/reed_amd/csrc/attention_f32.hip
+++ b/reed_amd/csrc/attention_f32.hip
@@ -232,6 +232,12 @@
   }
 }
 
+}
+
+extern "C" int reed_attention_fwd(const void* qkv, void* o, float* lse, int B, int T, int H, int hd, void* stream);
+extern "C" int reed_attention_fwd_ordered(const void* qkv, void* o, float* lse, int B, int T, int H, int hd, int, int,
+                                          void* stream) {
+  return reed_attention_fwd(qkv, o, lse, B, T, H, hd, stream);
 }
 
 extern "C" int reed_attention_fwd(const void* qkv, void* o, float* lse, int B, int T, int H, int hd, void* stream) {
diff --git a/reed_amd/csrc/gemm.hip b/reed_amd/csrc/gemm.hip
--- a/reed_amd/csrc/gemm.hip
+++ b/reed_amd/csrc/gemm.hip
@@ -211,7 +211,10 @@
 extern "C" int reed_gemm_force_tile(int tile) { g_force_tile = tile; return 0; }
 int reed_gemm_forced_tile() { return g_force_tile; }
 
+void reed_gemm_clear_last_deal();
+
 int reed_gemm_launch(int layout, int epi, GemmArgs a, int splits, hipStream_t stream) {
+  reed_gemm_clear_last_deal();
   REED_CHECK_ARG(a.M > 0 && a.N > 0 && a.K > 0, "reed_gemm: empty problem M=%d N=%d K=%d", a.M, a.N, a.K);
   const int want = epi;
   if (epi == EPI_BF16_DOT) {
diff --git a/reed_amd/csrc/gemm256w.hip b/reed_amd/csrc/gemm256w.hip
--- a/reed_amd/csrc/gemm256w.hip
+++ b/reed_amd/csrc/gemm256w.hip
@@ -6,6 +6,7 @@
 #include <vector>
 #include <type_traits>
 
+#include "age_order.hpp"
 #include "gemm_common.hpp"
 
 int reed_num_cus();
@@ -714,21 +715,14 @@
 #endif
 }
 
-__device__ __forceinline__ void w_tile_of(int b, int ntm, int ntn, int GM, int& tm, int& tn) {
-  const int per_group = GM * ntn;
-  const int group = b / per_group, first_m = group * GM;
-  const int gs = min(ntm - first_m, GM);
-  tm = first_m + (b % per_group) % gs;
-  tn = (b % per_group) / gs;
-}
 template <int LAY, int EPI>
 __global__ __launch_bounds__(256, 1) void gemm256wp_kernel(GemmArgs a) {
   extern __shared__ __attribute__((aligned(16))) char smem[];
   const int ntm = (a.M + WBM - 1) / WBM, ntn = (a.N + WBN - 1) / WBN;
   const int nwg = ntm * ntn;
   const int xcd = blockIdx.x & 7, s = blockIdx.x >> 3, wpx = gridDim.x >> 3;
-  const int q = nwg >> 3, r = nwg & 7;
-  const int run0 = xcd < r ? xcd * (q + 1) : r * (q + 1) + (xcd - r) * q, runlen = q + (xcd < r ? 1 : 0);
+  int run0, runlen;
+  w_run_of(xcd, nwg, run0, runlen);
   int p = s;
   if (p >= runlen) return;
   int tm, tn;
@@ -828,6 +822,7 @@
   return worst;
 }
 
+thread_local struct { int M, ntn, gm; } g_last_deal = {0, 0, 0};
 template <int LAY, int EPI>
 int launch256wp(const GemmArgs& a, hipStream_t stream, bool* used) {
   const int forced = reed_gemm_forced_tile();
@@ -867,6 +862,7 @@
   b.tile_gm = GM;
   REED_KLAUNCH((gemm256wp_kernel<LAY, EPI>), dim3(8 * wpx), dim3(256), LDS_W, stream, b);
   REED_LAUNCH_CHECK();
+  g_last_deal = {a.M, ntn, GM};
   *used = true;
   return REED_OK;
 }
@@ -941,6 +937,27 @@
 
 int reed_gemm_forced_tile();
 
+void reed_gemm_clear_last_deal() { g_last_deal = {0, 0, 0}; }
+#ifndef REED_AGE_ORDER_DEFAULT
+#define REED_AGE_ORDER_DEFAULT 1
+#endif
+extern "C" int reed_gemm_last_deal(int* m_ntn_gm) {
+  if (!m_ntn_gm || g_last_deal.M <= 0 || !REED_AGE_ORDER_DEFAULT) return 0;
+  m_ntn_gm[0] = g_last_deal.M;
+  m_ntn_gm[1] = g_last_deal.ntn;
+  m_ntn_gm[2] = g_last_deal.gm;
+  return 1;
+}
+extern "C" int reed_gemm_deal_for(int M, int N, int* ntn_gm) {
+  if (!ntn_gm || M <= 0 || N <= 0) return 0;
+  GemmArgs a{};
+  a.M = M;
+  a.N = N;
+  ntn_gm[0] = cdiv(N, WBN);
+  ntn_gm[1] = w_tile_group_rows(a);
+  return 1;
+}
+
 static int w4_deal(int n, const int* M, const int* N, const int* has_db, int ncu, unsigned* item) {
   if (n < 1 || n > 4 || ncu < 8 || (ncu & 7) != 0 || ncu > 256) return 0;
   const int wpx = ncu / 8;
diff --git a/reed_amd/csrc/gemm_f32.hip b/reed_amd/csrc/gemm_f32.hip
--- a/reed_amd/csrc/gemm_f32.hip
+++ b/reed_amd/csrc/gemm_f32.hip
@@ -291,6 +291,8 @@
 }
 
 extern "C" int reed_wgrad_group_deal(int, const int*, const int*, const int*, int, unsigned*) { return 0; }
+extern "C" int reed_gemm_last_deal(int*) { return 0; }
+extern "C" int reed_gemm_deal_for(int, int, int*) { return 0; }
 
 static int conv3x3_f32(const char* what, const void* act, const void* w, const float* bias, float* out, int64_t ldc, int B, int Hi,
                        int Wi, int C, int N, int upsample, int down, int accumulate, void* stream) {
diff --git a/reed_amd/csrc/norm.hip b/reed_amd/csrc/norm.hip
--- a/reed_amd/csrc/norm.hip
+++ b/reed_amd/csrc/norm.hip
@@ -1,4 +1,5 @@
 #include "../../include/reed_hip.h"
+#include "age_order.hpp"
 #include "common.hpp"
 
 namespace {
@@ -16,12 +17,14 @@
   *(bf16x4*)p = o;
 }
 
-template <bool NT>
+template <bool NT, bool ORD>
 __global__ __launch_bounds__(256) void ln_mod_fwd_kernel(const float* __restrict__ x, const bf16* __restrict__ shift,
                                                          const bf16* __restrict__ scale, long ldmod,
                                                          bf16* __restrict__ h, float* __restrict__ mean,
-                                                         float* __restrict__ rstd, int M, int D, int T, float eps) {
-  const int row = blockIdx.x * 4 + (threadIdx.x >> 6);
+                                                         float* __restrict__ rstd, int M, int D, int T, float eps, AgeRuns ord) {
+  int blk = blockIdx.x;
+  if constexpr (ORD) blk = age_order_strip(blockIdx.x >> 6, ord) * 64 + (blockIdx.x & 63);
+  const int row = blk * 4 + (threadIdx.x >> 6);
   if (row >= M) return;
   const int lane = threadIdx.x & 63, nv = D >> 2;
   const float* xr = x + (long)row * D;
@@ -285,12 +288,17 @@
 #define REED_LNB_NT 1
 #endif
 constexpr int LNB_AUX = REED_LNB_NT ? 2 : 0;
-template <bool GATE, int NF, int TS>
+template <bool GATE, int NF, int TS, bool ORD>
 __global__ __launch_bounds__(512, 4) void ln_mod_bwd2_kernel(
     const bf16* __restrict__ dh, const float* __restrict__ x, const float* __restrict__ mean,
     const float* __restrict__ rstd, const bf16* __restrict__ scale, long ldmod, float* __restrict__ dx,
     float* __restrict__ part, const bf16* __restrict__ y, const bf16* __restrict__ gate, long ldgate,
-    bf16* __restrict__ dy, float* __restrict__ part_g, float* __restrict__ part_dy, int M, int T) {
+    bf16* __restrict__ dy, float* __restrict__ part_g, float* __restrict__ part_dy, int M, int T, AgeRuns ord) {
+  int blk = blockIdx.x;
+  if constexpr (ORD) {
+    blk = age_order_strip(blockIdx.x >> 4, ord) * 16 + (blockIdx.x & 15);
+    if (blk * 16 >= M) return;
+  }
   using HR = HalfRow<NF, TS>;
   constexpr int NE = HR::NE, D = 128 * NE, HB = sizeof(bf16);
   extern __shared__ __attribute__((aligned(16))) float red[];
@@ -299,7 +307,7 @@
   const int rg = wave >> 1, hf = wave & 1;
   const HR hr(hf, lane);
   float* rsum = red + 8 * D;
-  const long blk0 = (long)blockIdx.x * 16;
+  const long blk0 = (long)blk * 16;
   const long smp = blk0 / T;
   const __amdgpu_buffer_rsrc_t rsX = row_rsrc(x + blk0 * D, 16 * D * 4), rsDX = row_rsrc(dx + blk0 * D, 16 * D * 4),
                                rsDH = row_rsrc(dh + blk0 * D, 16 * D * HB),
@@ -362,17 +370,17 @@
   hr.st_lds(red + (rg * 2 + 0) * D, ps);
   hr.st_lds(red + (rg * 2 + 1) * D, pq);
   __syncthreads();
-  float* out = part + (long)blockIdx.x * 2 * D;
+  float* out = part + (long)blk * 2 * D;
   for (int i = threadIdx.x; i < 2 * D; i += 512) out[i] = red[i] + red[2 * D + i] + red[4 * D + i] + red[6 * D + i];
   if constexpr (GATE) {
     __syncthreads();
     hr.st_lds(red + (rg * 2 + 0) * D, pg);
     hr.st_lds(red + (rg * 2 + 1) * D, pd);
     __syncthreads();
-    float* og = part_g + (long)blockIdx.x * D;
+    float* og = part_g + (long)blk * D;
     for (int i = threadIdx.x; i < D; i += 512) og[i] = red[i] + red[2 * D + i] + red[4 * D + i] + red[6 * D + i];
     if (part_dy) {
-      float* od = part_dy + (long)blockIdx.x * D;
+      float* od = part_dy + (long)blk * D;
       for (int i = threadIdx.x; i < D; i += 512) od[i] = red[D + i] + red[3 * D + i] + red[5 * D + i] + red[7 * D + i];
     }
   }
@@ -381,11 +389,17 @@
 template <bool GATE>
 bool launch_ln_mod_bwd2(hipStream_t stream, const bf16* dh, const float* x, const float* mean, const float* rstd,
                         const bf16* scale, long ldmod, float* dx, float* part, const bf16* y, const bf16* gate,
-                        long ldgate, bf16* dy, float* part_g, float* part_dy, int M, int D, int T) {
+                        long ldgate, bf16* dy, float* part_g, float* part_dy, int M, int D, int T, AgeOrder od) {
+  const AgeRuns ord = age_runs(M, od);
 #define REED_LNB2(NF_, TS_)                                                                                          \
   if (D == 128 * (4 * NF_ + TS_)) {                                                                                   \
-    REED_KLAUNCH((ln_mod_bwd2_kernel<GATE, NF_, TS_>), dim3(M / 16), dim3(512), (8 * D + 64) * sizeof(float),  \
-                       stream, dh, x, mean, rstd, scale, ldmod, dx, part, y, gate, ldgate, dy, part_g, part_dy, M, T); \
+    if (ord.n > 0)                                                                                                    \
+      REED_KLAUNCH((ln_mod_bwd2_kernel<GATE, NF_, TS_, true>), dim3(cdiv(M, 256) * 16), dim3(512),                    \
+                   (8 * D + 64) * sizeof(float), stream, dh, x, mean, rstd, scale, ldmod, dx, part, y, gate, ldgate,  \
+                   dy, part_g, part_dy, M, T, ord);                                                                   \
+    else                                                                                                              \
+      REED_KLAUNCH((ln_mod_bwd2_kernel<GATE, NF_, TS_, false>), dim3(M / 16), dim3(512), (8 * D + 64) * sizeof(float), \
+                   stream, dh, x, mean, rstd, scale, ldmod, dx, part, y, gate, ldgate, dy, part_g, part_dy, M, T, ord); \
     return true;                                                                                                      \
   }
   REED_LNB2(0, 1) REED_LNB2(0, 2) REED_LNB2(0, 3) REED_LNB2(1, 0) REED_LNB2(1, 2) REED_LNB2(2, 0) REED_LNB2(2, 1)
@@ -620,19 +634,56 @@
 
 }
 
-extern "C" int reed_ln_modulate_fwd(const float* x, const void* shift, const void* scale, int64_t ldmod,
-                                    void* h, float* mean, float* rstd, int M, int D, int T, float eps,
-                                    void* stream) {
+static int ln_modulate_fwd(const float* x, const void* shift, const void* scale, int64_t ldmod, void* h, float* mean,
+                           float* rstd, int M, int D, int T, float eps, AgeOrder ord, void* stream) {
   REED_CHECK_ARG(x && h, "ln_modulate_fwd: null pointer");
   REED_CHECK_ARG(D % 4 == 0 && D <= 256 * MAXV, "ln_modulate: D=%d unsupported (multiple of 4, <= %d)", D, 256 * MAXV);
   REED_CHECK_ARG(M > 0 && T > 0, "ln_modulate: bad M=%d T=%d", M, T);
   REED_CHECK_ARG((scale == nullptr) == (shift == nullptr), "ln_modulate: shift and scale must both be given or both NULL");
-  if ((long)M * D * 4 >= (256l << 20))
-    REED_KLAUNCH(ln_mod_fwd_kernel<true>, dim3(cdiv(M, 4)), dim3(256), 0, (hipStream_t)stream, x, (const bf16*)shift,
-                 (const bf16*)scale, (long)ldmod, (bf16*)h, mean, rstd, M, D, T, eps);
-  else
-    REED_KLAUNCH(ln_mod_fwd_kernel<false>, dim3(cdiv(M, 4)), dim3(256), 0, (hipStream_t)stream, x, (const bf16*)shift,
-                 (const bf16*)scale, (long)ldmod, (bf16*)h, mean, rstd, M, D, T, eps);
+  REED_CHECK_ARG(ord.ntn >= 0 && (ord.ntn == 0 || ord.gm > 0), "ln_modulate: bad order (%d, %d)", ord.ntn, ord.gm);
+  const AgeRuns runs = age_runs(M, ord);
+  const bool nt = (long)M * D * 4 >= (256l << 20);
+#define REED_LNF(NT_, ORD_, GRID_)                                                                                      \
+  REED_KLAUNCH((ln_mod_fwd_kernel<NT_, ORD_>), dim3(GRID_), dim3(256), 0, (hipStream_t)stream, x, (const bf16*)shift, \
+               (const bf16*)scale, (long)ldmod, (bf16*)h, mean, rstd, M, D, T, eps, runs)
+  if (runs.n > 0) {
+    if (nt) REED_LNF(true, true, cdiv(M, 256) * 64);
+    else REED_LNF(false, true, cdiv(M, 256) * 64);
+  } else {
+    if (nt) REED_LNF(true, false, cdiv(M, 4));
+    else REED_LNF(false, false, cdiv(M, 4));
+  }
+#undef REED_LNF
+  REED_LAUNCH_CHECK();
+  return REED_OK;
+}
+
+extern "C" int reed_ln_modulate_fwd(const float* x, const void* shift, const void* scale, int64_t ldmod,
+                                    void* h, float* mean, float* rstd, int M, int D, int T, float eps,
+                                    void* stream) {
+  return ln_modulate_fwd(x, shift, scale, ldmod, h, mean, rstd, M, D, T, eps, AgeOrder{0, 0}, stream);
+}
+
+extern "C" int reed_ln_modulate_fwd_ordered(const float* x, const void* shift, const void* scale, int64_t ldmod,
+                                            void* h, float* mean, float* rstd, int M, int D, int T, float eps,
+                                            int order_ntn, int order_gm, void* stream) {
+  return ln_modulate_fwd(x, shift, scale, ldmod, h, mean, rstd, M, D, T, eps, AgeOrder{order_ntn, order_gm}, stream);
+}
+
+static int ln_modulate_bwd(const void* dh, const float* x, const float* mean, const float* rstd, const void* scale,
+                           int64_t ldmod, float* dx, float* part, int M, int D, int T, AgeOrder ord, void* stream) {
+  REED_CHECK_ARG(dh && x && mean && rstd && scale && dx && part, "ln_modulate_bwd: null pointer");
+  REED_CHECK_ARG(D % 4 == 0 && D <= 256 * MAXV, "ln_modulate: D=%d unsupported", D);
+  REED_CHECK_ARG(T % 16 == 0 && M % 16 == 0, "ln_modulate_bwd: T=%d, M=%d must be multiples of 16", T, M);
+  REED_CHECK_ARG(ord.ntn >= 0 && (ord.ntn == 0 || ord.gm > 0), "ln_modulate_bwd: bad order (%d, %d)", ord.ntn, ord.gm);
+  if (launch_ln_mod_bwd2<false>((hipStream_t)stream, (const bf16*)dh, x, mean, rstd, (const bf16*)scale, (long)ldmod, dx,
+                                part, nullptr, nullptr, 0l, nullptr, nullptr, nullptr, M, D, T, ord)) {
+    REED_LAUNCH_CHECK();
+    return REED_OK;
+  }
+    REED_KLAUNCH(ln_mod_bwd_kernel<false>, dim3(M / 16), dim3(256), 8 * D * sizeof(float), (hipStream_t)stream,
+                 (const bf16*)dh, x, mean, rstd, (const bf16*)scale, (long)ldmod, dx, part, (const bf16*)nullptr,
+                 (const bf16*)nullptr, 0l, (bf16*)nullptr, (float*)nullptr, (float*)nullptr, M, D, T);
   REED_LAUNCH_CHECK();
   return REED_OK;
 }
@@ -640,17 +691,31 @@
 extern "C" int reed_ln_modulate_bwd(const void* dh, const float* x, const float* mean, const float* rstd,
                                     const void* scale, int64_t ldmod, float* dx, float* part, int M, int D,
                                     int T, void* stream) {
-  REED_CHECK_ARG(dh && x && mean && rstd && scale && dx && part, "ln_modulate_bwd: null pointer");
+  return ln_modulate_bwd(dh, x, mean, rstd, scale, ldmod, dx, part, M, D, T, AgeOrder{0, 0}, stream);
+}
+
+extern "C" int reed_ln_modulate_bwd_ordered(const void* dh, const float* x, const float* mean, const float* rstd,
+                                            const void* scale, int64_t ldmod, float* dx, float* part, int M, int D,
+                                            int T, int order_ntn, int order_gm, void* stream) {
+  return ln_modulate_bwd(dh, x, mean, rstd, scale, ldmod, dx, part, M, D, T, AgeOrder{order_ntn, order_gm}, stream);
+}
+
+static int ln_modulate_bwd_gate(const void* dh, const float* x, const float* mean, const float* rstd, const void* scale,
+                                int64_t ldmod, float* dx, float* part, const void* y, const void* gate, int64_t ldgate,
+                                void* dy, float* part_g, float* part_dy, int M, int D, int T, AgeOrder ord, void* stream) {
+  REED_CHECK_ARG(dh && x && mean && rstd && scale && dx && part, "ln_modulate_bwd_gate: null pointer");
+  REED_CHECK_ARG(y && gate && dy && part_g, "ln_modulate_bwd_gate: null gate operand");
   REED_CHECK_ARG(D % 4 == 0 && D <= 256 * MAXV, "ln_modulate: D=%d unsupported", D);
-  REED_CHECK_ARG(T % 16 == 0 && M % 16 == 0, "ln_modulate_bwd: T=%d, M=%d must be multiples of 16", T, M);
-  if (launch_ln_mod_bwd2<false>((hipStream_t)stream, (const bf16*)dh, x, mean, rstd, (const bf16*)scale, (long)ldmod, dx,
-                                part, nullptr, nullptr, 0l, nullptr, nullptr, nullptr, M, D, T)) {
+  REED_CHECK_ARG(T % 16 == 0 && M % 16 == 0, "ln_modulate_bwd_gate: T=%d, M=%d must be multiples of 16", T, M);
+  REED_CHECK_ARG(ord.ntn >= 0 && (ord.ntn == 0 || ord.gm > 0), "ln_modulate_bwd_gate: bad order (%d, %d)", ord.ntn, ord.gm);
+  if (launch_ln_mod_bwd2<true>((hipStream_t)stream, (const bf16*)dh, x, mean, rstd, (const bf16*)scale, (long)ldmod, dx,
+                               part, (const bf16*)y, (const bf16*)gate, (long)ldgate, (bf16*)dy, part_g, part_dy, M, D, T, ord)) {
     REED_LAUNCH_CHECK();
     return REED_OK;
   }
-    REED_KLAUNCH(ln_mod_bwd_kernel<false>, dim3(M / 16), dim3(256), 8 * D * sizeof(float), (hipStream_t)stream,
-                 (const bf16*)dh, x, mean, rstd, (const bf16*)scale, (long)ldmod, dx, part, (const bf16*)nullptr,
-                 (const bf16*)nullptr, 0l, (bf16*)nullptr, (float*)nullptr, (float*)nullptr, M, D, T);
+    REED_KLAUNCH(ln_mod_bwd_kernel<true>, dim3(M / 16), dim3(256), 8 * D * sizeof(float), (hipStream_t)stream,
+                 (const bf16*)dh, x, mean, rstd, (const bf16*)scale, (long)ldmod, dx, part, (const bf16*)y,
+                 (const bf16*)gate, (long)ldgate, (bf16*)dy, part_g, part_dy, M, D, T);
   REED_LAUNCH_CHECK();
   return REED_OK;
 }
@@ -659,20 +724,28 @@
                                          const void* scale, int64_t ldmod, float* dx, float* part, const void* y,
                                          const void* gate, int64_t ldgate, void* dy, float* part_g, float* part_dy,
                                          int M, int D, int T, void* stream) {
-  REED_CHECK_ARG(dh && x && mean && rstd && scale && dx && part, "ln_modulate_bwd_gate: null pointer");
-  REED_CHECK_ARG(y && gate && dy && part_g, "ln_modulate_bwd_gate: null gate operand");
-  REED_CHECK_ARG(D % 4 == 0 && D <= 256 * MAXV, "ln_modulate: D=%d unsupported", D);
-  REED_CHECK_ARG(T % 16 == 0 && M % 16 == 0, "ln_modulate_bwd_gate: T=%d, M=%d must be multiples of 16", T, M);
-  if (launch_ln_mod_bwd2<true>((hipStream_t)stream, (const bf16*)dh, x, mean, rstd, (const bf16*)scale, (long)ldmod, dx,
-                               part, (const bf16*)y, (const bf16*)gate, (long)ldgate, (bf16*)dy, part_g, part_dy, M, D, T)) {
-    REED_LAUNCH_CHECK();
-    return REED_OK;
-  }
-    REED_KLAUNCH(ln_mod_bwd_kernel<true>, dim3(M / 16), dim3(256), 8 * D * sizeof(float), (hipStream_t)stream,
-                 (const bf16*)dh, x, mean, rstd, (const bf16*)scale, (long)ldmod, dx, part, (const bf16*)y,
-                 (const bf16*)gate, (long)ldgate, (bf16*)dy, part_g, part_dy, M, D, T);
-  REED_LAUNCH_CHECK();
-  return REED_OK;
+  return ln_modulate_bwd_gate(dh, x, mean, rstd, scale, ldmod, dx, part, y, gate, ldgate, dy, part_g, part_dy, M, D, T,
+                              AgeOrder{0, 0}, stream);
+}
+
+extern "C" int reed_ln_modulate_bwd_gate_ordered(const void* dh, const float* x, const float* mean, const float* rstd,
+                                                 const void* scale, int64_t ldmod, float* dx, float* part, const void* y,
+                                                 const void* gate, int64_t ldgate, void* dy, float* part_g, float* part_dy,
+                                                 int M, int D, int T, int order_ntn, int order_gm, void* stream) {
+  return ln_modulate_bwd_gate(dh, x, mean, rstd, scale, ldmod, dx, part, y, gate, ldgate, dy, part_g, part_dy, M, D, T,
+                              AgeOrder{order_ntn, order_gm}, stream);
+}
+
+extern "C" int reed_age_order(int M, int ntn, int gm, int* strips, int* runs) {
+  if (M <= 0 || ntn <= 0 || gm <= 0 || !strips) return 0;
+  const AgeRuns r = age_runs(M, AgeOrder{ntn, gm});
+  const int ns = r.n;
+  for (int v = 0; v < ns; ++v) {
+    int run = 0;
+    strips[v] = age_order_strip(v, r, &run);
+    if (runs) runs[v] = run;
+  }
+  return ns;
 }
 
 extern "C" int reed_transpose_bf16(const void* src, void* dst, int R, int C, void* stream) {
diff --git a/reed_amd/engine.py b/reed_amd/engine.py
--- a/reed_amd/engine.py
+++ b/reed_amd/engine.py
@@ -52,6 +52,7 @@
         self._hb = 2
         self.save_act_grad = None
         self.fused_delta = True
+        self.age_order = False
         self._err = None
 
     def _check_dims(self, prec):
@@ -82,6 +83,16 @@
 
     def G(self, name):
         return self.A.grad.data_ptr() + 4 * self.L.off(name)
+
+    def _order(self, M, N):
+        if self.age_order is False:
+            return None
+        deal = ops.gemm_last_deal()
+        if deal is not None and deal[0] != M:
+            deal = None
+        if self.age_order is None:
+            return deal if M * self.D * 4 >= (256 << 20) else None
+        return deal if deal is not None else ops.gemm_deal_for(M, N)
 
     def ws(self, nfloats, dev):
         if self._ws is None or self._ws.numel() < nfloats:
@@ -172,6 +183,7 @@
             xa, xb = tok, f32(M, D)
             h, qkv, o, u = bf(M, D), bf(M, 3 * D), bf(M, D), bf(M, Hm)
         xcur = tok
+        ord_x = None
         zs_by_proj = {}
         for i in range(self.depth):
             b = f"blocks.{i}."
@@ -194,23 +206,26 @@
                 mean1 = rstd1 = mean2 = rstd2 = lse = None
                 xmid = xb if xcur is xa else xa
                 xout = xcur
-            ops.ln_modulate_fwd(xcur, mb, mb + hb * D, Nall, h, mean1, rstd1, M, D, T)
+            ops.ln_modulate_fwd(xcur, mb, mb + hb * D, Nall, h, mean1, rstd1, M, D, T, order=ord_x)
             ops.gemm(NT, EPI_BF16, h, self.W(b + "attn.qkv.weight"), M, 3 * D, D, qkv, D, D, 3 * D,
                      bias=self.W(b + "attn.qkv.bias"))
+            ord_qkv = self._order(M, 3 * D)
             qkv_a, qstats = qkv, None
             if m.qk_norm:
+                ord_qkv = None
                 qkv_a = bf(M, 3 * D)
                 qstats = f32(M, 2, H, 2) if need_grad else None
                 ops.qk_norm_fwd(qkv, self.Wf(b + "attn.q_norm.weight"), self.Wf(b + "attn.q_norm.bias"),
                                 self.Wf(b + "attn.k_norm.weight"), self.Wf(b + "attn.k_norm.bias"), qkv_a, qstats, M, H, hd)
-            ops.attention_fwd(qkv_a, o, lse, B, T, H, hd)
+            ops.attention_fwd(qkv_a, o, lse, B, T, H, hd, order=ord_qkv)
             ops.gemm(NT, EPI_GATE_RES, o, self.W(b + "attn.proj.weight"), M, D, D, xmid, D, D, D, C2=y1, ldc2=D,
                      R=xcur, ldr=D, bias=self.W(b + "attn.proj.bias"), gate=mb + 2 * hb * D, ldgate=Nall, rows_per_gate=T)
-            ops.ln_modulate_fwd(xmid, mb + 3 * hb * D, mb + 4 * hb * D, Nall, h2, mean2, rstd2, M, D, T)
+            ops.ln_modulate_fwd(xmid, mb + 3 * hb * D, mb + 4 * hb * D, Nall, h2, mean2, rstd2, M, D, T, order=self._order(M, D))
             ops.gemm(NT, epi_gelu, h2, self.W(b + "mlp.fc1.weight"), M, Hm, D, a1, D, D, Hm, C2=u, ldc2=Hm,
                      bias=self.W(b + "mlp.fc1.bias"))
             ops.gemm(NT, EPI_GATE_RES, u, self.W(b + "mlp.fc2.weight"), M, D, Hm, xout, Hm, Hm, D, C2=y2, ldc2=D,
                      R=xmid, ldr=D, bias=self.W(b + "mlp.fc2.bias"), gate=mb + 5 * hb * D, ldgate=Nall, rows_per_gate=T)
+            ord_x = self._order(M, D)
             if need_grad:
                 tp.blocks.append(types.SimpleNamespace(x=xcur, mean1=mean1, rstd1=rstd1, h=h, qkv=qkv, qkv_a=qkv_a,
                                                        qstats=qstats, o=o, lse=lse,
@@ -220,7 +235,8 @@
             if not inference:
                 for j, dj in enumerate(self.tap_depth):
                     if dj == i + 1:
-                        zs_by_proj[j] = self._projector_fwd(j, xcur, B, need_grad, tp)
+                        zs_by_proj[j] = self._projector_fwd(j, xcur, B, need_grad, tp, ord_x)
+                        ord_x = None
         if kh:
             self.A.wait("ada_tail")
             ops.gemm(NT, EPI_BF16, silu_c, sp + hb * (L.ada_w_off + n_head * D), B, Nall - n_head, D, mp + hb * n_head,
@@ -248,7 +264,7 @@
                     tp.zs_order = list(range(len(m.z_dims)))
         return out, zs, tp
 
-    def _projector_fwd(self, j, x, B, need_grad, tp):
+    def _projector_fwd(self, j, x, B, need_grad, tp, ord_x=None):
         m, D, T = self.m, self.D, self.T
         Pd, Z = m.projector_dim, m.z_dims[j]
         dev = x.device
@@ -259,7 +275,7 @@
         bf = lambda *s: torch.empty(s, dtype=hdt, device=dev)
         xin = bf(R, D)
         if img:
-            ops.ln_modulate_fwd(x, None, None, 0, xin, None, None, R, D, T)
+            ops.ln_modulate_fwd(x, None, None, 0, xin, None, None, R, D, T, order=ord_x)
         else:
             ops.token_mean_fwd(x, xin, B, T, D)
         pre = f"projectors.{j}."
@@ -379,14 +395,14 @@
         def tap_fires(depth_idx):
             return any(dj == depth_idx and j in tp.proj for j, dj in pending.items())
 
-        def ln_bwd(dh_, x_, mean_, rstd_, scale_ptr, part_, nxt):
+        def ln_bwd(dh_, x_, mean_, rstd_, scale_ptr, part_, nxt, order=None):
             if nxt is None or nxt < 0 or tap_fires(nxt + 1):
-                ops.ln_modulate_bwd(dh_, x_, mean_, rstd_, scale_ptr, Nall, dx, part_, M, D, T)
+                ops.ln_modulate_bwd(dh_, x_, mean_, rstd_, scale_ptr, Nall, dx, part_, M, D, T, order=order)
                 return None
             nb_ = tp.blocks[nxt]
             dy_, pg_ = bf(M, D), f32(M // 16, D)
             ops.ln_modulate_bwd_gate(dh_, x_, mean_, rstd_, scale_ptr, Nall, dx, part_, nb_.y2,
-                                     mp + hb * (nxt * 6 * D + 5 * D), Nall, dy_, pg_, None, M, D, T)
+                                     mp + hb * (nxt * 6 * D + 5 * D), Nall, dy_, pg_, None, M, D, T, order=order)
             return dy_, pg_
 
         pre = ln_bwd(dh, tp.x_last, tp.meanF, tp.rstdF, mf + hb * D, partF, self.depth - 1)
@@ -472,7 +488,7 @@
             pl2 = f32(M // 16, 2, D)
             pg1, dy1 = f32(M // 16, D), bf(M, D)
             ops.ln_modulate_bwd_gate(dh2, bk.xmid, bk.mean2, bk.rstd2, mb + 4 * hb * D, Nall, dx, pl2, bk.y1, mb + 2 * hb * D, Nall,
-                                     dy1, pg1, None, M, D, T)
+                                     dy1, pg1, None, M, D, T, order=self._order(M, D))
             if wg is not None:
                 wg.append((dy1, bk.o, b + "attn.proj.weight", D, D))
             else:
@@ -505,8 +521,9 @@
                 self._wgrad(dqkv, bk.h, b + "attn.qkv.weight", M, 3 * D, D, acc, dev, side=side)
             dh1 = do
             self._dgrad(EPI_BF16, dqkv, b + "attn.qkv.weight", M, 3 * D, D, dh1)
+            ord_dh1 = self._order(M, D)
             pl1 = f32(M // 16, 2, D)
-            pre = ln_bwd(dh1, bk.x, bk.mean1, bk.rstd1, mb + hb * D, pl1, i - 1)
+            pre = ln_bwd(dh1, bk.x, bk.mean1, bk.rstd1, mb + hb * D, pl1, i - 1, order=ord_dh1)
             o6 = i * 6 * D
             p1, p2 = pl1.data_ptr(), pl2.data_ptr()
             ops.reduce_mod_parts([(p1, 2 * D, o6), (p1 + 4 * D, 2 * D, o6 + D), (pg1.data_ptr(), D, o6 + 2 * D),
diff --git a/reed_amd/ops.py b/reed_amd/ops.py
--- a/reed_amd/ops.py
+++ b/reed_amd/ops.py
@@ -290,17 +290,64 @@
     _call("reed_reduce_slabs", _p(slabs), stride, n, _p(out), count, int(accumulate), _stream())
 
 
-def ln_modulate_fwd(x, shift, scale, ldmod, h, mean, rstd, M, D, T, eps=1e-6):
-    _call("reed_ln_modulate_fwd", _p(x), _p(shift), _p(scale), ldmod, _p(h), _p(mean), _p(rstd), M, D, T, eps, _stream())
-
-
-def ln_modulate_bwd(dh, x, mean, rstd, scale, ldmod, dx, part, M, D, T):
-    _call("reed_ln_modulate_bwd", _p(dh), _p(x), _p(mean), _p(rstd), _p(scale), ldmod, _p(dx), _p(part), M, D, T, _stream())
-
-
-def ln_modulate_bwd_gate(dh, x, mean, rstd, scale, ldmod, dx, part, y, gate, ldgate, dy, part_g, part_dy, M, D, T):
-    _call("reed_ln_modulate_bwd_gate", _p(dh), _p(x), _p(mean), _p(rstd), _p(scale), ldmod, _p(dx), _p(part), _p(y),
-          _p(gate), ldgate, _p(dy), _p(part_g), _p(part_dy), M, D, T, _stream())
+def gemm_last_deal():
+    out = (ctypes.c_int * 3)()
+    if _lib.load(_PRECISION).reed_gemm_last_deal(ctypes.cast(out, ctypes.c_void_p)) != 1:
+        return None
+    return out[0], out[1], out[2]
+
+
+def gemm_deal_for(M, N):
+    out = (ctypes.c_int * 2)()
+    if _lib.load(_PRECISION).reed_gemm_deal_for(int(M), int(N), ctypes.cast(out, ctypes.c_void_p)) != 1:
+        return None
+    return int(M), out[0], out[1]
+
+
+def age_order(M, ntn, gm, precision="bf16"):
+    ns = (M + 255) // 256
+    strips, runs = (ctypes.c_int * ns)(), (ctypes.c_int * ns)()
+    n = _lib.load(precision).reed_age_order(int(M), int(ntn), int(gm), ctypes.cast(strips, ctypes.c_void_p),
+                                            ctypes.cast(runs, ctypes.c_void_p))
+    if n != ns or n <= 0:
+        raise ValueError(f"reed_age_order({M}, {ntn}, {gm}) returned {n}")
+    return list(strips), list(runs)
+
+
+def _order_args(order, M):
+    if order is None:
+        return None
+    if order[0] != M:
+        raise ValueError(f"order {order} was dealt for {order[0]} rows, not {M}")
+    return int(order[1]), int(order[2])
+
+
+def ln_modulate_fwd(x, shift, scale, ldmod, h, mean, rstd, M, D, T, eps=1e-6, order=None):
+    od = _order_args(order, M)
+    if od is None:
+        _call("reed_ln_modulate_fwd", _p(x), _p(shift), _p(scale), ldmod, _p(h), _p(mean), _p(rstd), M, D, T, eps, _stream())
+    else:
+        _call("reed_ln_modulate_fwd_ordered", _p(x), _p(shift), _p(scale), ldmod, _p(h), _p(mean), _p(rstd), M, D, T, eps,
+              od[0], od[1], _stream())
+
+
+def ln_modulate_bwd(dh, x, mean, rstd, scale, ldmod, dx, part, M, D, T, order=None):
+    od = _order_args(order, M)
+    if od is None:
+        _call("reed_ln_modulate_bwd", _p(dh), _p(x), _p(mean), _p(rstd), _p(scale), ldmod, _p(dx), _p(part), M, D, T, _stream())
+    else:
+        _call("reed_ln_modulate_bwd_ordered", _p(dh), _p(x), _p(mean), _p(rstd), _p(scale), ldmod, _p(dx), _p(part), M, D, T,
+              od[0], od[1], _stream())
+
+
+def ln_modulate_bwd_gate(dh, x, mean, rstd, scale, ldmod, dx, part, y, gate, ldgate, dy, part_g, part_dy, M, D, T, order=None):
+    od = _order_args(order, M)
+    if od is None:
+        _call("reed_ln_modulate_bwd_gate", _p(dh), _p(x), _p(mean), _p(rstd), _p(scale), ldmod, _p(dx), _p(part), _p(y),
+              _p(gate), ldgate, _p(dy), _p(part_g), _p(part_dy), M, D, T, _stream())
+    else:
+        _call("reed_ln_modulate_bwd_gate_ordered", _p(dh), _p(x), _p(mean), _p(rstd), _p(scale), ldmod, _p(dx), _p(part), _p(y),
+              _p(gate), ldgate, _p(dy), _p(part_g), _p(part_dy), M, D, T, od[0], od[1], _stream())
 
 
 def gate_bwd(dx, y, gate, ldgate, dy, part, M, D, T, part_dy=None):
@@ -335,8 +382,12 @@
     _call("reed_cast_bf16", _p(src), _p(dst), n, _stream())
 
 
-def attention_fwd(qkv, o, lse, B, T, H, hd):
-    _call("reed_attention_fwd", _p(qkv), _p(o), _p(lse), B, T, H, hd, _stream())
+def attention_fwd(qkv, o, lse, B, T, H, hd, order=None):
+    od = _order_args(order, B * T)
+    if od is None:
+        _call("reed_attention_fwd", _p(qkv), _p(o), _p(lse), B, T, H, hd, _stream())
+    else:
+        _call("reed_attention_fwd_ordered", _p(qkv), _p(o), _p(lse), B, T, H, hd, od[0], od[1], _stream())
 
 
 def attention_bwd(qkv, o, do, lse, dqkv, B, T, H, hd, ws=None):
```

After: 1334. No clear change (-0.1%).
